# PAMRec/PAMRec

Measured on NVIDIA B200. Metric: train samples/sec, higher is better.
Workload: dtype f32

## Files before the change

pamrec_b200/csrc/api.cu:

```cuda
#include <cmath>
#include <cstdarg>
#include <cstdio>
#include <cstdlib>
#include <string>
#include <vector>

#include "comm.h"
#include "head2.h"
#include "kernels.h"
#include "layout.h"

using namespace pamrec;

struct Xchg {
  std::vector<int64_t> soff, scnt, roff, rcnt;
  int64_t n_send = 0, n_recv = 0;
};

struct PamrecHandle_ {
  PamrecConfig cfg;
  Layout L;
  PamrecBuffers buf;
  bool bound = false;
  int debug = 0;
// ... 301 lines not shown
  size_t have = (size_t)h->L.ws[h->L.ws_index["cub_temp"]].numel;
  if (need > have) return fail(h, "cub temp storage: need %zu have %zu", need, have);
  cudaMemsetAsync(h->buf.workspace, 0, h->L.ws_bytes, st);
  if (h->sharded() || h->sibling()) {
    cudaMemsetAsync(h->wi("sp.item.slot"), 0xFF, (size_t)h->L.rows_of(h->cfg.n_items) * 4, st);
    cudaMemsetAsync(h->wi("sp.cate.slot"), 0xFF, (size_t)h->L.rows_of(h->cfg.n_cates) * 4, st);
    if (h->cfg.model_kind != PAMREC_MODEL_SASREC)
      cudaMemsetAsync(h->wi("sp.user.slot"), 0xFF, (size_t)h->L.rows_of(h->cfg.n_users) * 4, st);
  } else {
    cudaMemsetAsync(h->wi("sp2.slot"), 0xFF, ((size_t)h->cfg.n_items + h->cfg.n_cates + h->cfg.n_users) * 4, st);
  }
  if (h->sharded() && !h->h_counts &&
      cudaMallocHost(&h->h_counts, sizeof(int) * (8 * (size_t)h->cfg.world_size + 4)) != cudaSuccess)
    return fail(h, "cudaMallocHost for the exchange counts failed");
  cudaMemcpyAsync(h->wi("seg_id"), h->h_seg_id.data(), h->h_seg_id.size() * 4, cudaMemcpyHostToDevice, st);
  cudaMemcpyAsync(h->wi("seg_tab"), h->h_seg_tab.data(), h->h_seg_tab.size() * 4, cudaMemcpyHostToDevice, st);
  if (h->sibling()) h->head2_grid = 0;
  else if (int rc = build_head(h, st)) return rc;
  cudaStreamSynchronize(st);
  h->bound = true;
  return check_cuda(h, "bind");
}

static int check_batch(PamrecHandle h, const PamrecBatch* b, bool training) {
  if (!h) return -1;
  if (!h->bound) return fail(h, "pamrec_bind has not been called");
  if (!b) return fail(h, "null batch");
  if (b->batch == 0 && (h->sharded() || h->cfg.world_size > 1)) return 0;
  if (b->batch < 1 || b->batch > h->cfg.max_batch) return fail(h, "batch %d outside [1, %d]", b->batch, h->cfg.max_batch);
  if (h->sibling()) {
    if (!b->satisfied_item_history || !b->satisfied_cate_history || !b->satisfied_mask || !b->item_history || !b->item_cate_history ||
        !b->mask || !b->items || !b->cates)
      return fail(h, "null batch field (the sibling models also read satisfied_item_history / satisfied_cate_history / satisfied_mask)");
    const bool sas = h->cfg.model_kind == PAMREC_MODEL_SASREC;
    if (training && (!b->labels_satisfied || (!sas && (!b->users || !b->labels_play)))) return fail(h, "null label field");
    return 0;
  }
  if (training && b->batch % PAMREC_GROUP != 0)
    return fail(h, "training batch %d is not a multiple of %d (pamrec.py:73-75)", b->batch, PAMREC_GROUP);
  if (training && h->cfg.loss_kind == PAMREC_LOSS_SOFTMAX && b->batch % h->cfg.softmax_group != 0)
    return fail(h, "training batch %d is not a multiple of the softmax group %d (base_model.py:224-225)", b->batch, h->cfg.softmax_group);
  if (!b->item_history || !b->item_cate_history || !b->item_loop_times_history || !b->mask || !b->items || !b->cates)
    return fail(h, "null batch field");
  if (training && (!b->users || !b->labels_satisfied || !b->labels_play || !b->plays)) return fail(h, "null label field");
  return 0;
}

static Sp2 make_sp2(PamrecHandle h, const PamrecBatch* b) {
  Sp2 s;
  memset(&s, 0, sizeof s);
  const PamrecConfig& c = h->cfg;
  s.item_hist = b->item_history; s.cate_hist = b->item_cate_history; s.items = b->items; s.cates = b->cates; s.users = b->users;
  s.B = b->batch; s.N = (int64_t)b->batch * c.max_seq_len;
  s.n_items = c.n_items; s.n_cates = c.n_cates; s.n_users = c.n_users;
  s.keys = h->wi("sp2.keys"); s.idx = h->wi("sp2.idx"); s.skeys = h->wi("sp2.skeys"); s.sidx = h->wi("sp2.sidx"); s.uidx = h->wi("sp2.uidx");
  s.ukeys[0] = h->wi("sp.item.ukeys"); s.ukeys[1] = h->wi("sp.cate.ukeys"); s.ukeys[2] = h->wi("sp.user.ukeys");
  s.nuniq = h->wi("sp.nuniq"); s.meta = h->wi("sp2.meta");
  s.accum[0] = h->wf("sp.item.accum"); s.accum[1] = h->wf("sp.cate.accum");
  s.dflag[0] = h->wi("sp2.dflag"); s.dflag[1] = s.dflag[0] + h->L.cub_keys_table;
  s.l2sq = h->wd("sp2.l2sq"); s.undedup = h->wd("sp_normsq");
  s.w[0] = h->buf.item_w; s.m[0] = h->buf.item_m; s.v[0] = h->buf.item_v;
  s.w[1] = h->buf.cate_w; s.m[1] = h->buf.cate_m; s.v[1] = h->buf.cate_v;
  s.w[2] = h->buf.ulong_w; s.m[2] = h->buf.ulong_m; s.v[2] = h->buf.ulong_v;
  s.w[3] = h->buf.ushort_w; s.m[3] = h->buf.ushort_m; s.v[3] = h->buf.ushort_v;
  s.dX0 = h->wf("g_a"); s.dT = h->wf("d_tgt_total");
  if (h->replicated()) { s.mode = SP2_DENSE; s.rep_grad = h->rep_grad_in(); }
  else if (c.sparse_adam_mode == PAMREC_ADAM_LAZY) s.mode = SP2_FUSED;
  else { s.mode = SP2_COMPACT; s.slot = h->wi("sp2.slot"); }
  return s;
}
static AdamP make_adam(PamrecHandle h, float lr_t) {
  const PamrecConfig& c = h->cfg;
  AdamP a;
  a.lr = lr_t; a.b1 = c.beta1; a.b2 = c.beta2; a.eps = c.epsilon; a.l2 = c.embed_l2; a.clip = c.max_grad_norm; a.is_clip = c.is_clip_norm;
  a.lr_dev = nullptr;
  return a;
}

static const char* const kShardName[3] = {"item", "cate", "user"};
static const ShardDim& shard_dim(PamrecHandle h, int t) { return t == 0 ? h->L.sh_item : (t == 1 ? h->L.sh_cate : h->L.sh_user); }

static SparseTable req_table(PamrecHandle h, int t) {
  SparseTable s;
  memset(&s, 0, sizeof s);
  const ShardDim& d = shard_dim(h, t);
  std::string p = std::string("sp.") + kShardName[t] + ".";
  s.keys = h->wi(p + "keys"); s.idx = h->wi(p + "idx"); s.skeys = h->wi(p + "skeys"); s.sidx = h->wi(p + "sidx");
  s.uidx = h->wi(p + "uidx"); s.ukeys = h->wi(p + "ukeys");
  s.width = d.width; s.n_rows = d.rps * h->cfg.world_size;
  s.accum = d.width ? h->wf(p + "accum") : nullptr;
  s.nuniq = h->wi("sp.nuniq") + t;
  s.normsq = h->wd("sp_normsq") + t;
  return s;
}
static SparseTable own_table(PamrecHandle h, int t, bool user_short = false) {
  SparseTable s;
  memset(&s, 0, sizeof s);
  const ShardDim& d = shard_dim(h, t);
  std::string q = std::string("so.") + kShardName[t] + ".";
  s.keys = h->wi(q + "keys"); s.idx = h->wi(q + "idx"); s.skeys = h->wi(q + "skeys"); s.sidx = h->wi(q + "sidx");
  s.uidx = h->wi(q + "uidx"); s.ukeys = h->wi(q + "ukeys");
  s.slot = h->wi(std::string("sp.") + kShardName[t] + ".slot");
  s.n_rows = d.rps;
  s.nuniq = h->wi("sp.nuniq") + 4 + t;
  double* ns = h->wd("sp_normsq");
  if (t == 0) { s.width = kI; s.w = h->buf.item_w; s.m = h->buf.item_m; s.v = h->buf.item_v; s.accum = h->wf(q + "accum"); s.normsq = ns; }
  else if (t == 1) { s.width = kC; s.w = h->buf.cate_w; s.m = h->buf.cate_m; s.v = h->buf.cate_v; s.accum = h->wf(q + "accum"); s.normsq = ns + 1; }
  else if (!user_short) { s.width = PAMREC_USER_DIM; s.w = h->buf.ulong_w; s.m = h->buf.ulong_m; s.v = h->buf.ulong_v; s.normsq = ns + 2; }
  else { s.width = PAMREC_USER_DIM; s.w = h->buf.ushort_w; s.m = h->buf.ushort_m; s.v = h->buf.ushort_v; s.normsq = ns + 3; }
  return s;
}

static int shard_exchange_fwd(PamrecHandle h, const PamrecBatch* b, bool training, cudaStream_t st) {
  const int W = h->cfg.world_size, B = b->batch, T = h->cfg.max_seq_len;
  const int64_t N = (int64_t)B * T;
  void* tmp = h->ws<char>("cub_temp");
  const size_t tmp_bytes = (size_t)h->L.ws[h->L.ws_index.at("cub_temp")].numel;
  int* cs = h->wi("sh.counts_send");
  int* cr = h->wi("sh.counts_recv");
  cudaMemsetAsync(cs, 0, sizeof(int) * 4 * W, st);
  const int nt = training ? 3 : 2;
  h->xc_users = training;
  for (int t = 0; t < nt; ++t) {
    const ShardDim& d = shard_dim(h, t);
    SparseTable req = req_table(h, t);
    const int* hist = t == 0 ? b->item_history : (t == 1 ? b->item_cate_history : b->users);
    const int* tgt = t == 0 ? b->items : (t == 1 ? b->cates : nullptr);
    const int64_t n_hist = t < 2 ? N : B, n_tgt = t < 2 ? B : 0;
    if (launch_sparse_plan(req, hist, tgt, n_hist, n_tgt, W, d.rps, d.rps * W, false, tmp, tmp_bytes, st))
      return fail(h, "cub sort failed");
    std::string p = std::string("sh.") + kShardName[t] + ".";
    launch_shard_route(req, n_hist + n_tgt, W, d.rps, h->wi(p + "off"), cs, t, h->wi(p + "send_ids"), h->wi(p + "inv"), st);
  }
  {
    PAMREC_PROF("xchg_counts", 1, st);
    if (h->comm.all_to_all(cs, cr, 4, COMM_I32, st)) return fail(h, "nccl: %s", h->comm.err.c_str());
    cudaMemcpyAsync(h->h_counts, cs, sizeof(int) * 4 * W, cudaMemcpyDeviceToHost, st);
    cudaMemcpyAsync(h->h_counts + 4 * W, cr, sizeof(int) * 4 * W, cudaMemcpyDeviceToHost, st);
    h->h_counts[8 * W] = 0;
    if (h->mbox_open) cudaMemcpyAsync(h->h_counts + 8 * W, h->mbox_err(), sizeof(int), cudaMemcpyDeviceToHost, st);
    if (cudaStreamSynchronize(st) != cudaSuccess) return check_cuda(h, "exchange counts");
    if (h->h_counts[8 * W]) return fail(h, "peer mailbox all-reduce timed out at sync point %d (a rank left the step?)", h->h_counts[8 * W] - 1);
  }
  for (int t = 0; t < 3; ++t) {
    Xchg& x = h->xc[t];
    x.soff.assign(W, 0); x.scnt.assign(W, 0); x.roff.assign(W, 0); x.rcnt.assign(W, 0);
    int64_t so = 0, ro = 0;
    for (int p = 0; p < W; ++p) {
      x.scnt[p] = t < nt ? h->h_counts[4 * p + t] : 0;
      x.rcnt[p] = t < nt ? h->h_counts[4 * W + 4 * p + t] : 0;
      x.soff[p] = so; so += x.scnt[p];
      x.roff[p] = ro; ro += x.rcnt[p];
    }
    x.n_send = so; x.n_recv = ro;
    if (ro > shard_dim(h, t).cap_recv) return fail(h, "exchange overflow on table %s: %lld rows", kShardName[t], (long long)ro);
  }
  {
    PAMREC_PROF("xchg_ids", 1, st);
    int xrc = h->comm.group_start();
    for (int t = 0; t < nt && !xrc; ++t) {
      const Xchg& x = h->xc[t];
      std::string p = std::string("sh.") + kShardName[t] + ".";
      xrc |= h->comm.all_to_all_v(h->wi(p + "send_ids"), x.soff.data(), x.scnt.data(), h->wi(p + "recv_ids"), x.roff.data(),
                                  x.rcnt.data(), 1, COMM_I32, st);
    }
    xrc |= h->comm.group_end();
    if (xrc) return fail(h, "nccl: %s", h->comm.err.c_str());
  }
  if (training) {
    int prc = 0;
    h->fork(st, [&](cudaStream_t s2) {
      for (int t = 0; t < 3; ++t) {
        SparseTable own = own_table(h, t);
        std::string p = std::string("sh.") + kShardName[t] + ".";
        prc |= launch_sparse_plan(own, h->wi(p + "recv_ids"), nullptr, h->xc[t].n_recv, 0, 1, 0, own.n_rows, true, tmp, tmp_bytes, s2);
      }
      cudaEventRecord(h->ev_plan, s2);
    });
    if (prc) return fail(h, "cub sort failed");
  }
  launch_serve_rows(h->buf.item_w, h->wi("sh.item.recv_ids"), h->xc[0].n_recv, kI, h->wf("sh.item.xrows"), st);
  launch_serve_rows(h->buf.cate_w, h->wi("sh.cate.recv_ids"), h->xc[1].n_recv, kC, h->wf("sh.cate.xrows"), st);
  {
    PAMREC_PROF("xchg_rows", 1, st);
    int xrc = h->comm.group_start();
    for (int t = 0; t < 2 && !xrc; ++t) {
      const Xchg& x = h->xc[t];
      std::string p = std::string("sh.") + kShardName[t] + ".";
      xrc |= h->comm.all_to_all_v(h->wf(p + "xrows"), x.roff.data(), x.rcnt.data(), h->wf(p + "rows"), x.soff.data(),
                                  x.scnt.data(), shard_dim(h, t).width, COMM_F32, st);
    }
    xrc |= h->comm.group_end();
    if (xrc) return fail(h, "nccl: %s", h->comm.err.c_str());
  }
  return 0;
}

static int embed_forward(PamrecHandle h, const PamrecBatch* b, bool training, float* x0, cudaStream_t st) {
  const int B = b->batch, T = h->cfg.max_seq_len;
  if (!h->sharded()) {
    launch_embed_fwd(b->item_history, b->item_cate_history, b->items, b->cates, h->buf.item_w, h->buf.cate_w, h->P(h->L.pos), x0,
                     h->wf("tgt"), B, T, st);
    return 0;
  }
  if (int rc = shard_exchange_fwd(h, b, training, st)) return rc;
  const int64_t N = (int64_t)B * T;
  const int* ii = h->wi("sh.item.inv");
  const int* ci = h->wi("sh.cate.inv");
  launch_embed_fwd(ii, ci, ii + N, ci + N, h->wf("sh.item.rows"), h->wf("sh.cate.rows"), h->P(h->L.pos), x0, h->wf("tgt"), B, T, st);
  return 0;
}

int pamrec_gather_fwd(PamrecHandle h, const PamrecBatch* b, float* x0_out, void* stream) {
  if (int rc = check_batch(h, b, false)) return rc;
  if (h->sibling()) return fail(h, "pamrec_gather_fwd is PAMRec's fused gather; the sibling models gather inside pamrec_forward");
  ProfBind _pb(h);
  cudaStream_t st = (cudaStream_t)stream;
  if (int rc = embed_forward(h, b, false, x0_out ? x0_out : h->wf("x0"), st)) return rc;
  return check_cuda(h, "gather_fwd");
}

static DenseP dense_p(const float* X, int ldx, int M, int groups, int K, int N, const float* W, int ws, const float* bias,
                      int bs, float* Z, int ldz) {
  DenseP p;
  memset(&p, 0, sizeof p);
  p.X = X; p.ldx = ldx; p.M = M; p.n_groups = groups; p.K = K; p.N = N;
  p.W = W; p.w_stride = ws; p.bias = bias; p.b_stride = bs; p.Z = Z; p.ldz = ldz;
  return p;
}
static void set_in_bn(DenseP& p, const BnSet& s) { p.in_stat = s.stat; p.in_gamma = s.gamma; p.in_beta = s.beta; }
static void set_in_bn_dw(DenseDwP& p, const BnSet& s) { p.in_stat = s.stat; p.in_gamma = s.gamma; p.in_beta = s.beta; }

static int sib_forward(PamrecHandle h, const PamrecBatch* b, int training, float* pred_out, cudaStream_t st);
static int sib_backward(PamrecHandle h, const PamrecBatch* b, cudaStream_t st);
static int sib_apply(PamrecHandle h, const PamrecBatch* b, int64_t step, cudaStream_t st);
static int sas_forward(PamrecHandle h, const PamrecBatch* b, int training, float* pred_out, cudaStream_t st);
static int sas_backward(PamrecHandle h, const PamrecBatch* b, cudaStream_t st);

int pamrec_forward(PamrecHandle h, const PamrecBatch* b, int training, float* pred_out, void* stream) {
  if (int rc = check_batch(h, b, training != 0)) return rc;
  ProfBind _pb(h);
  cudaStream_t st = (cudaStream_t)stream;
  if (h->cfg.model_kind == PAMREC_MODEL_SASREC) return sas_forward(h, b, training, pred_out, st);
  if (h->sibling()) return sib_forward(h, b, training, pred_out, st);
  const Layout& L = h->L;
  const int B = b->batch, T = h->cfg.max_seq_len, N = B * T;
  const int W = h->cfg.world_size;
  const int Bg = b->global_batch > 0 ? b->global_batch : B * W;
  const double cntN = (double)Bg * T, cntB = (double)Bg;
  int64_t nl = 0;
  int crc = 0;
  int p2p_slot = 0;
  auto sync_finalize = [&](std::initializer_list<int> ids, double cnt, bool with_scalars) {
    if (!training) return;
    if (W > 1 && h->mbox_open) {
      P2PArgs a;
      memset(&a, 0, sizeof a);
      for (int id : ids) { a.buf[a.nbuf] = h->bn[id].sums; a.n[a.nbuf++] = 2 * h->bn[id].C; a.bn[a.nbn] = h->bn[id]; a.count[a.nbn++] = cnt; }
      if (with_scalars) { a.buf[a.nbuf] = h->wd("dp.scalars"); a.n[a.nbuf++] = 8; }
      for (int p = 0; p < W; ++p) { a.peer_slots[p] = h->mbox_slots(p); a.peer_flags[p] = h->mbox_flags(p); }
      a.world = W; a.rank = h->cfg.rank; a.slot = p2p_slot; a.epoch = ++h->mbox_epoch[p2p_slot]; a.err = h->mbox_err();
      ++p2p_slot;
      launch_p2p_allreduce(a, st); nl += 1;
      return;
    }
    if (W > 1 && !crc) {
      PAMREC_PROF("allreduce_bn_fwd", 1, st);
      crc |= h->comm.group_start();
      for (int id : ids) crc |= h->comm.all_reduce(h->bn[id].sums, 2 * (int64_t)h->bn[id].C, COMM_F64, st);
      if (with_scalars) crc |= h->comm.all_reduce(h->wd("dp.scalars"), 8, COMM_F64, st);
      crc |= h->comm.group_end();
    }
    for (int id : ids) { launch_bn_finalize(h->bn[id], cnt, st); nl += 1; }
  };
  float* x0 = h->wf("x0");
  int* ctl = h->wi("bucket_ctl");
  const bool bucket_aside = !h->sharded() && getenv("PAMREC_NO_SIDE_STREAM") == nullptr;
  if (bucket_aside) {
    h->fork(st, [&](cudaStream_t s2) {
      launch_bucket_plan(b->item_loop_times_history, N, h->wi("bucket"), h->wi("perm"), ctl, h->wi("tile_bucket"), h->wi("tile_begin"),
                         h->wi("tile_count"), s2);
      cudaEventRecord(h->ev_bucket, s2);
    });
  }
  if (int rc = embed_forward(h, b, training != 0, x0, st)) return rc;
  nl += 1;
  if (training && !h->sharded() && B > 0) {
    int prc = 0;
    h->fork(st, [&](cudaStream_t s2) {
      prc |= launch_sp2_plan(make_sp2(h, b), h->ws<char>("cub_temp"), (size_t)L.ws[L.ws_index.at("cub_temp")].numel, s2);
      cudaEventRecord(h->ev_plan, s2);
    });
    if (prc) return fail(h, "cub sort failed");
    h->plan_for = b->item_history; h->plan_rows = B;
  }
  if (training && W > 1 && !h->use_head2()) {
    cudaMemsetAsync(h->wd("dp.scalars"), 0, 8 * sizeof(double), st);
    launch_count_valid_groups(b->plays, B, h->wd("dp.scalars"), st);
  }
  if (bucket_aside) cudaStreamWaitEvent(st, h->ev_bucket, 0);
  else launch_bucket_plan(b->item_loop_times_history, N, h->wi("bucket"), h->wi("perm"), ctl, h->wi("tile_bucket"),
                          h->wi("tile_begin"), h->wi("tile_count"), st);
  nl += 3;
  const int max_tiles = N / kTokTile + kNB + 1;
  const float* xin = x0;
  for (int k = 0; k < 2; ++k) {
    const BlockOff& o = L.blk[k];
    std::string p = "blk" + std::to_string(k) + ".";
    launch_proj_fwd(xin, h->wi("perm"), ctl, h->wi("tile_bucket"), h->wi("tile_begin"), h->wi("tile_count"), max_tiles,
                    h->P(o.wq), h->P(o.wk), h->P(o.wv), h->P(o.ln_a_beta), h->P(o.ln_a_gamma), h->wf(p + "qin"), h->wf(p + "Q"),
                    h->wf(p + "K"), h->wf(p + "V"), st);
    if (h->attn_mma)
      launch_attn_fwd_mma(h->wf(p + "Q"), h->wf(p + "K"), h->wf(p + "V"), h->wf(p + "qin"), b->mask, h->wf(p + "y"), h->wf(p + "ml"), B, T, st);
    else if (h->attn_tc && attn_tc_supported(T))
      launch_attn_fwd_tc(h->wf(p + "Q"), h->wf(p + "K"), h->wf(p + "V"), h->wf(p + "qin"), b->mask, h->wf(p + "y"), h->wf(p + "ml"), B, T,
                         h->n_sm, reinterpret_cast<int*>(h->head_bar + 3), st);
    else
      launch_attn_fwd(h->wf(p + "Q"), h->wf(p + "K"), h->wf(p + "V"), h->wf(p + "qin"), b->mask, h->wf(p + "y"), h->wf(p + "ml"), B, T, st);
    float* hdbg = (training && (h->debug & PAMREC_DEBUG_SAVE_FFN_HIDDEN)) ? h->wf(k == 0 ? "d_Q" : "d_K") : nullptr;
    launch_ffn_fwd(h->wf(p + "y"), h->P(o.w1), h->P(o.b1), h->P(o.w2), h->P(o.b2), h->P(o.ln_b_beta), h->P(o.ln_b_gamma),
                   h->wf(p + "out"), hdbg, N, st);
    nl += 3;
    xin = h->wf(p + "out");
  }
  const float* H = xin;
  BnSet* bn = h->bn;
  if (h->use_head2()) {
    HeadDyn d = head_dyn(h, b, training != 0, 0);
    d.pred = pred_out;
    if (launch_head2_fwd(h->head2, d, h->head2_grid, training ? "head_fwd" : "head_score", st)) return check_cuda(h, "cooperative head launch");
    return check_cuda(h, "forward");
  }
  if (!training) {
    for (int i = 0; i < BN_COUNT; ++i) launch_bn_eval_stat(bn[i], st);
    nl += BN_COUNT;
  }
  {
    DenseP p = dense_p(H, kD, N, 1, kD, 20, h->P(L.score.w0), 0, h->P(L.score.b0), 0, h->wf("z1"), 20);
    p.out_sums = training ? bn[BN_S0].sums : nullptr;
    launch_dense_fwd(p, st); nl += 1;
    sync_finalize({BN_S0}, cntN, true);
    DenseP q = dense_p(h->wf("z1"), 20, N, 1, 20, 1, h->P(L.score.w1), 0, h->P(L.score.b1), 0, h->wf("z2"), 1);
    set_in_bn(q, bn[BN_S0]);
    q.out_sums = training ? bn[BN_S1].sums : nullptr;
    launch_dense_fwd(q, st); nl += 1;
    sync_finalize({BN_S1}, cntN, false);
  }
  launch_pool_fwd(H, h->wf("z2"), bn[BN_S1], b->mask, h->wf("new_long"), B, T, st); nl += 1;
  {
    DenseP e0 = dense_p(h->wf("new_long"), kD, B, 5, kD, 100, h->P(L.expert.w0), 4000, h->P(L.expert.b0), 100, h->wf("ze0"), 500);
    for (int g = 0; g < 5; ++g) { e0.x_off[g] = 0; e0.z_off[g] = g * 100; }
    e0.out_sums = training ? bn[BN_E0].sums : nullptr;
    launch_dense_fwd(e0, st);
    DenseP g0 = dense_p(h->wf("new_long"), kD, B, 2, kD, 64, h->P(L.gate.w0), 2560, h->P(L.gate.b0), 64, h->wf("zg0"), 128);
    for (int g = 0; g < 2; ++g) { g0.x_off[g] = 0; g0.z_off[g] = g * 64; }
    g0.out_sums = training ? bn[BN_G0].sums : nullptr;
    launch_dense_fwd(g0, st);
    nl += 2;
    sync_finalize({BN_E0, BN_G0}, cntB, false);
    DenseP e1 = dense_p(h->wf("ze0"), 500, B, 5, 100, 64, h->P(L.expert.w1), 6400, h->P(L.expert.b1), 64, h->wf("ze1"), 320);
    for (int g = 0; g < 5; ++g) { e1.x_off[g] = g * 100; e1.z_off[g] = g * 64; }
    set_in_bn(e1, bn[BN_E0]);
    e1.out_sums = training ? bn[BN_E1].sums : nullptr;
    launch_dense_fwd(e1, st);
    DenseP g1 = dense_p(h->wf("zg0"), 128, B, 2, 64, 5, h->P(L.gate.w1), 320, h->P(L.gate.b1), 5, h->wf("zg1"), 10);
    for (int g = 0; g < 2; ++g) { g1.x_off[g] = g * 64; g1.z_off[g] = g * 5; }
    set_in_bn(g1, bn[BN_G0]);
    g1.out_sums = training ? bn[BN_G1].sums : nullptr;
    launch_dense_fwd(g1, st);
    nl += 2;
    sync_finalize({BN_E1, BN_G1}, cntB, false);
  }
  launch_combine_fwd(h->wf("ze1"), h->wf("zg1"), bn[BN_E1], bn[BN_G1], h->wf("tgt"), h->wf("u"), B, st); nl += 1;
  {
    DenseP t0 = dense_p(h->wf("u"), 168, B, 3, 84, 100, h->P(L.tower.w0), 8400, h->P(L.tower.b0), 100, h->wf("zt0"), 300);
    t0.x_off[0] = 0; t0.x_off[1] = 84; t0.x_off[2] = 0;
    for (int g = 0; g < 3; ++g) t0.z_off[g] = g * 100;
    t0.out_sums = training ? bn[BN_T0].sums : nullptr;
    launch_dense_fwd(t0, st); nl += 1;
    sync_finalize({BN_T0}, cntB, false);
    DenseP t1 = dense_p(h->wf("zt0"), 300, B, 3, 100, 64, h->P(L.tower.w1), 6400, h->P(L.tower.b1), 64, h->wf("zt1"), 192);
    for (int g = 0; g < 3; ++g) { t1.x_off[g] = g * 100; t1.z_off[g] = g * 64; }
    set_in_bn(t1, bn[BN_T0]);
    t1.out_sums = training ? bn[BN_T1].sums : nullptr;
    launch_dense_fwd(t1, st); nl += 1;
    sync_finalize({BN_T1}, cntB, false);
    DenseP to = dense_p(h->wf("zt1"), 192, B, 3, 64, 1, h->P(L.tower.wout), 64, h->P(L.tower.bout), 1, h->wf("logits"), 3);
    for (int g = 0; g < 3; ++g) { to.x_off[g] = g * 64; to.z_off[g] = g; }
    set_in_bn(to, bn[BN_T1]);
    launch_dense_fwd(to, st); nl += 1;
  }
  if (pred_out) { launch_sigmoid_col0(h->wf("logits"), pred_out, B, st); nl += 1; }
  if (crc) return fail(h, "nccl: %s", h->comm.err.c_str());
  return check_cuda(h, "forward");
}

static DenseDwP dw_p(const float* X, int ldx, int M, int groups, int K, int N, const float* dZ, int lddz, float* dW, int ws,
                     float* db, int bs) {
  DenseDwP p;
  memset(&p, 0, sizeof p);
  p.X = X; p.ldx = ldx; p.M = M; p.n_groups = groups; p.K = K; p.N = N; p.dZ = dZ; p.lddz = lddz;
  p.dW = dW; p.w_stride = ws; p.db = db; p.b_stride = bs;
  return p;
}
static DenseDxP dx_p(const float* dZ, int lddz, int M, int K, const float* Wbase, float* dX, int lddx, int accumulate) {
  DenseDxP p;
  memset(&p, 0, sizeof p);
  p.dZ = dZ; p.lddz = lddz; p.M = M; p.K = K; p.Wbase = Wbase; p.dX = dX; p.lddx = lddx; p.accumulate = accumulate;
  return p;
}
static void dx_add(DenseDxP& p, int slice, int out_off, int dz_off, int64_t w_off, int N) {
  if (slice >= p.n_slices) { p.n_slices = slice + 1; p.out_off[slice] = out_off; p.n_contrib[slice] = 0; }
  int c = p.n_contrib[slice]++;
  p.dz_off[slice][c] = dz_off; p.w_off[slice][c] = w_off; p.Ncon[slice][c] = N;
}

static HeadDyn head_dyn(PamrecHandle h, const PamrecBatch* b, bool training, int slot0) {
  HeadDyn d;
  memset(&d, 0, sizeof d);
  const int W = h->cfg.world_size;
  d.B = b->batch; d.T = h->cfg.max_seq_len; d.training = training ? 1 : 0; d.world = W; d.rank = h->cfg.rank;
  d.Bg = b->global_batch > 0 ? b->global_batch : b->batch * W;
  d.cntN = (double)d.Bg * d.T; d.cntB = (double)d.Bg;
  d.mask = b->mask; d.y_sat = b->labels_satisfied; d.y_play = b->labels_play; d.plays = b->plays;
  d.fuzhu_w = h->cfg.fuzhu_weight; d.order_w = h->cfg.order_weight;
  d.sm_group = h->cfg.loss_kind == PAMREC_LOSS_SOFTMAX ? h->cfg.softmax_group : 0;
  d.bar = h->head_bar;
  d.trace = h->head_trace ? reinterpret_cast<unsigned long long*>(h->head_bar + 64) + (slot0 ? 32 : 0) : nullptr;
  d.trace_cta = (h->head_trace && h->head_trace_cta) ? h->head_trace_cta + (slot0 ? 16 * 256 : 0) : nullptr;
  if (W > 1) {
    for (int p = 0; p < W; ++p) {
      d.peer_slots[p] = h->mbox_slots(p); d.peer_flags[p] = h->mbox_flags(p);
      d.peer_ll[p] = reinterpret_cast<uint4*>(static_cast<char*>(h->mbox_peer[p]) + p2p_ll_offset(W));
    }
    d.p2p_epoch = ++h->coop_epoch; d.p2p_slot0 = slot0; d.p2p_err = h->mbox_err();
  }
  return d;
}

static int build_head(PamrecHandle h, cudaStream_t st) {
  h->head2_grid = 0;
  if (getenv("PAMREC_HEAD_LEGACY") != nullptr) return 0;
  if (h->cfg.world_size > kP2PMaxWorld) return 0;
  const Layout& L = h->L;
  Head2& H = h->head2;
  memset(&H, 0, sizeof H);
  H.H = h->wf("blk1.out"); H.tgt = h->wf("tgt");
  H.s_w0 = h->P(L.score.w0); H.s_b0 = h->P(L.score.b0); H.s_w1 = h->P(L.score.w1); H.s_b1 = h->P(L.score.b1);
  H.e_w0 = h->P(L.expert.w0); H.e_b0 = h->P(L.expert.b0); H.e_w1 = h->P(L.expert.w1); H.e_b1 = h->P(L.expert.b1);
  H.g_w0 = h->P(L.gate.w0); H.g_b0 = h->P(L.gate.b0); H.g_w1 = h->P(L.gate.w1); H.g_b1 = h->P(L.gate.b1);
  H.t_w0 = h->P(L.tower.w0); H.t_b0 = h->P(L.tower.b0); H.t_w1 = h->P(L.tower.w1); H.t_b1 = h->P(L.tower.b1);
  H.t_wo = h->P(L.tower.wout); H.t_bo = h->P(L.tower.bout);
  H.ds_w0 = h->G(L.score.w0); H.ds_b0 = h->G(L.score.b0); H.ds_w1 = h->G(L.score.w1); H.ds_b1 = h->G(L.score.b1);
  H.de_w0 = h->G(L.expert.w0); H.de_b0 = h->G(L.expert.b0); H.de_w1 = h->G(L.expert.w1); H.de_b1 = h->G(L.expert.b1);
  H.dg_w0 = h->G(L.gate.w0); H.dg_b0 = h->G(L.gate.b0); H.dg_w1 = h->G(L.gate.w1); H.dg_b1 = h->G(L.gate.b1);
  H.dt_w0 = h->G(L.tower.w0); H.dt_b0 = h->G(L.tower.b0); H.dt_w1 = h->G(L.tower.w1); H.dt_b1 = h->G(L.tower.b1);
  H.dt_wo = h->G(L.tower.wout); H.dt_bo = h->G(L.tower.bout);
  H.wT = h->wf("head.wT");
  static_assert(kHead2Groups == 8, "layout.h: bn.gsums / bn.gbsums hold 8 copies");
  for (int i = 0; i < BN_COUNT; ++i) {
    H.bn[i] = h->bn[i];
    H.gsums[i] = h->wd("bn.gsums") + (size_t)kHead2Groups * L.bn_bsums_off[i];
    H.gbsums[i] = h->wd("bn.gbsums") + (size_t)kHead2Groups * L.bn_bsums_off[i];
  }
  H.z1 = h->wf("z1"); H.z2 = h->wf("z2"); H.aw = h->wf("pool.aw"); H.new_long = h->wf("new_long");
  H.ze0 = h->wf("ze0"); H.zg0 = h->wf("zg0"); H.ze1 = h->wf("ze1"); H.zg1 = h->wf("zg1"); H.u = h->wf("u");
  H.zt0 = h->wf("zt0"); H.zt1 = h->wf("zt1"); H.logits = h->wf("logits");
  H.d_logits = h->wf("d_logits"); H.d_t1 = h->wf("d_t1"); H.d_t0 = h->wf("d_t0"); H.d_e1 = h->wf("d_e1"); H.d_g1 = h->wf("d_g1");
  H.d_e0 = h->wf("d_e0"); H.d_g0 = h->wf("d_g0"); H.d_new_long = h->wf("d_new_long"); H.d_tgt = h->wf("d_tgt");
  H.d_z2 = h->wf("d_z2"); H.g_a = h->wf("g_a");
  H.loss_acc = h->wd("loss_acc"); H.dp_scalars = h->wd("dp.scalars");
  const int g2 = head2_grid();
  if (g2 <= 0) { cudaGetLastError(); return 0; }
  if (!h->head_bar) {
    if (cudaMalloc(&h->head_bar, 256 + 2 * 32 * 8) != cudaSuccess) return check_cuda(h, "head barrier alloc");
    cudaMemsetAsync(h->head_bar, 0, 256 + 2 * 32 * 8, st);
  }
  h->head2_grid = g2;
  return check_cuda(h, "head2");
}

int pamrec_backward(PamrecHandle h, const PamrecBatch* b, void* stream) {
  if (int rc = check_batch(h, b, true)) return rc;
  ProfBind _pb(h);
  cudaStream_t st = (cudaStream_t)stream;
  if (h->cfg.model_kind == PAMREC_MODEL_SASREC) return sas_backward(h, b, st);
  if (h->sibling()) return sib_backward(h, b, st);
  const Layout& L = h->L;
  const int B = b->batch, T = h->cfg.max_seq_len, N = B * T;
  const int W = h->cfg.world_size;
  const int Bg = b->global_batch > 0 ? b->global_batch : B * W;
  const double cntN = (double)Bg * T, cntB = (double)Bg;
  const float gs = 1.0f / (float)W;
  BnSet* bn = h->bn;
  int64_t nl = 0;
  int crc = 0;
  const float* Pb = h->buf.dense_param;
  cudaMemsetAsync(h->buf.dense_grad, 0, (size_t)L.dense_numel * 4, st);
  cudaMemsetAsync(h->wd("loss_acc"), 0, 8 * sizeof(double), st);
  cudaMemsetAsync(h->wd("sp_normsq"), 0, 8 * sizeof(double), st);
  const bool rows = h->use_head2();
  const bool coop = rows;
  if (!coop) {
  launch_loss(h->wf("logits"), b->labels_satisfied, b->labels_play, b->plays, h->wf("d_logits"), h->wd("loss_acc"), B, Bg,
              W > 1 ? h->wd("dp.scalars") : nullptr, h->cfg.fuzhu_weight, h->cfg.order_weight,
              h->cfg.loss_kind == PAMREC_LOSS_SOFTMAX ? h->cfg.softmax_group : 0, st); nl += 1;
  }
  cudaMemsetAsync(h->wd("bn.bsums"), 0, (size_t)L.ws[L.ws_index.at("bn.bsums")].numel * sizeof(double), st);
  if (rows) {
    HeadDyn d = head_dyn(h, b, true, 12);
    if (launch_head2_bwd(h->head2, d, h->head2_grid, st)) return check_cuda(h, "cooperative head launch");
    h->fork(st, [&](cudaStream_t s2) { launch_head2_dw(h->head2, B, s2); });
  }
  int p2p_slot = 6;
  auto sync_bsums = [&](std::initializer_list<int> ids) {
    if (W == 1 || crc) return;
    if (h->mbox_open) {
      P2PArgs a;
      memset(&a, 0, sizeof a);
      for (int id : ids) { a.buf[a.nbuf] = bn[id].bsums; a.n[a.nbuf++] = 2 * bn[id].C; }
      for (int p = 0; p < W; ++p) { a.peer_slots[p] = h->mbox_slots(p); a.peer_flags[p] = h->mbox_flags(p); }
      a.world = W; a.rank = h->cfg.rank; a.slot = p2p_slot; a.epoch = ++h->mbox_epoch[p2p_slot]; a.err = h->mbox_err();
      ++p2p_slot;
      launch_p2p_allreduce(a, st);
      return;
    }
    PAMREC_PROF("allreduce_bn_bwd", 1, st);
    crc |= h->comm.group_start();
    for (int id : ids) crc |= h->comm.all_reduce(bn[id].bsums, 2 * (int64_t)bn[id].C, COMM_F64, st);
    crc |= h->comm.group_end();
  };
  auto grad_of = [&](int id, const float* Z, double cnt) {
    BnGrad g; g.Z = Z; g.stat = bn[id].stat; g.gamma = bn[id].gamma; g.beta = bn[id].beta; g.bsums = bn[id].bsums; g.count = cnt;
    return g;
  };
  auto out_of = [&](int id, const float* Z) {
    BnGradOut o; o.Z = Z; o.stat = bn[id].stat; o.gamma = bn[id].gamma; o.beta = bn[id].beta; o.bsums = bn[id].bsums;
    return o;
  };
  auto dw_bn = [&](DenseDwP& w, int id, const float* Z, double cnt) {
    w.g = grad_of(id, Z, cnt); w.g_dgamma = bn[id].dgamma; w.g_dbeta = bn[id].dbeta; w.g_C = bn[id].C; w.g_scale = gs;
  };
  if (!coop) {
  {
    DenseDwP w = dw_p(h->wf("zt1"), 192, B, 3, 64, 1, h->wf("d_logits"), 3, h->G(L.tower.wout), 64, h->G(L.tower.bout), 1);
    for (int g = 0; g < 3; ++g) { w.x_off[g] = g * 64; w.z_off[g] = g; }
    set_in_bn_dw(w, bn[BN_T1]);
    h->fork(st, [&](cudaStream_t s2) { launch_dense_dw(w, s2); });
    DenseDxP x = dx_p(h->wf("d_logits"), 3, B, 64, Pb, h->wf("d_t1"), 192, 0);
    for (int g = 0; g < 3; ++g) dx_add(x, g, g * 64, g, L.tower.wout + g * 64, 1);
    x.o = out_of(BN_T1, h->wf("zt1"));
    launch_dense_dx(x, st);
    nl += 2;
    sync_bsums({BN_T1});
    DenseDwP w1 = dw_p(h->wf("zt0"), 300, B, 3, 100, 64, h->wf("d_t1"), 192, h->G(L.tower.w1), 6400, h->G(L.tower.b1), 64);
    for (int g = 0; g < 3; ++g) { w1.x_off[g] = g * 100; w1.z_off[g] = g * 64; }
    set_in_bn_dw(w1, bn[BN_T0]);
    dw_bn(w1, BN_T1, h->wf("zt1"), cntB);
    h->fork(st, [&](cudaStream_t s2) { launch_dense_dw(w1, s2); });
    DenseDxP x1 = dx_p(h->wf("d_t1"), 192, B, 100, Pb, h->wf("d_t0"), 300, 0);
    for (int g = 0; g < 3; ++g) dx_add(x1, g, g * 100, g * 64, L.tower.w1 + (int64_t)g * 6400, 64);
    x1.g = grad_of(BN_T1, h->wf("zt1"), cntB);
    x1.o = out_of(BN_T0, h->wf("zt0"));
    launch_dense_dx(x1, st);
    nl += 2;
    sync_bsums({BN_T0});
    DenseDwP w0 = dw_p(h->wf("u"), 168, B, 3, 84, 100, h->wf("d_t0"), 300, h->G(L.tower.w0), 8400, h->G(L.tower.b0), 100);
    w0.x_off[0] = 0; w0.x_off[1] = 84; w0.x_off[2] = 0;
    for (int g = 0; g < 3; ++g) w0.z_off[g] = g * 100;
    dw_bn(w0, BN_T0, h->wf("zt0"), cntB);
    h->fork(st, [&](cudaStream_t s2) { launch_dense_dw(w0, s2); });
    DenseDxP x0 = dx_p(h->wf("d_t0"), 300, B, 84, Pb, h->wf("d_u"), 168, 0);
    dx_add(x0, 0, 0, 0, L.tower.w0, 100);
    dx_add(x0, 0, 0, 200, L.tower.w0 + 2 * 8400, 100);
    dx_add(x0, 1, 84, 100, L.tower.w0 + 8400, 100);
    x0.g = grad_of(BN_T0, h->wf("zt0"), cntB);
    launch_dense_dx(x0, st);
    nl += 2;
  }
  launch_combine_bwd(h->wf("ze1"), h->wf("zg1"), bn[BN_E1], bn[BN_G1], h->wf("d_u"), h->wf("d_e1"), h->wf("d_g1"),
                     h->wf("d_tgt"), B, st); nl += 1;
  {
    launch_bn_bwd_stats(bn[BN_E1], h->wf("d_e1"), h->wf("ze1"), B, st);
    launch_bn_bwd_stats(bn[BN_G1], h->wf("d_g1"), h->wf("zg1"), B, st);
    nl += 2;
    sync_bsums({BN_E1, BN_G1});
    DenseDwP we = dw_p(h->wf("ze0"), 500, B, 5, 100, 64, h->wf("d_e1"), 320, h->G(L.expert.w1), 6400, h->G(L.expert.b1), 64);
    for (int g = 0; g < 5; ++g) { we.x_off[g] = g * 100; we.z_off[g] = g * 64; }
    set_in_bn_dw(we, bn[BN_E0]);
    dw_bn(we, BN_E1, h->wf("ze1"), cntB);
    h->fork(st, [&](cudaStream_t s2) { launch_dense_dw(we, s2); });
    DenseDxP xe = dx_p(h->wf("d_e1"), 320, B, 100, Pb, h->wf("d_e0"), 500, 0);
    for (int g = 0; g < 5; ++g) dx_add(xe, g, g * 100, g * 64, L.expert.w1 + (int64_t)g * 6400, 64);
    xe.g = grad_of(BN_E1, h->wf("ze1"), cntB);
    xe.o = out_of(BN_E0, h->wf("ze0"));
    launch_dense_dx(xe, st);
    DenseDwP wg = dw_p(h->wf("zg0"), 128, B, 2, 64, 5, h->wf("d_g1"), 10, h->G(L.gate.w1), 320, h->G(L.gate.b1), 5);
    for (int g = 0; g < 2; ++g) { wg.x_off[g] = g * 64; wg.z_off[g] = g * 5; }
    set_in_bn_dw(wg, bn[BN_G0]);
    dw_bn(wg, BN_G1, h->wf("zg1"), cntB);
    h->fork(st, [&](cudaStream_t s2) { launch_dense_dw(wg, s2); });
    DenseDxP xg = dx_p(h->wf("d_g1"), 10, B, 64, Pb, h->wf("d_g0"), 128, 0);
    for (int g = 0; g < 2; ++g) dx_add(xg, g, g * 64, g * 5, L.gate.w1 + (int64_t)g * 320, 5);
    xg.g = grad_of(BN_G1, h->wf("zg1"), cntB);
    xg.o = out_of(BN_G0, h->wf("zg0"));
    launch_dense_dx(xg, st);
    nl += 4;
    sync_bsums({BN_E0, BN_G0});
    DenseDwP we0 = dw_p(h->wf("new_long"), kD, B, 5, kD, 100, h->wf("d_e0"), 500, h->G(L.expert.w0), 4000, h->G(L.expert.b0), 100);
    for (int g = 0; g < 5; ++g) { we0.x_off[g] = 0; we0.z_off[g] = g * 100; }
    dw_bn(we0, BN_E0, h->wf("ze0"), cntB);
    h->fork(st, [&](cudaStream_t s2) { launch_dense_dw(we0, s2); });
    DenseDwP wg0 = dw_p(h->wf("new_long"), kD, B, 2, kD, 64, h->wf("d_g0"), 128, h->G(L.gate.w0), 2560, h->G(L.gate.b0), 64);
    for (int g = 0; g < 2; ++g) { wg0.x_off[g] = 0; wg0.z_off[g] = g * 64; }
    dw_bn(wg0, BN_G0, h->wf("zg0"), cntB);
    h->fork(st, [&](cudaStream_t s2) { launch_dense_dw(wg0, s2); });
    DenseDxP xe0 = dx_p(h->wf("d_e0"), 500, B, kD, Pb, h->wf("d_new_long"), kD, 0);
    for (int g = 0; g < 5; ++g) dx_add(xe0, 0, 0, g * 100, L.expert.w0 + (int64_t)g * 4000, 100);
    xe0.g = grad_of(BN_E0, h->wf("ze0"), cntB);
    launch_dense_dx(xe0, st);
    DenseDxP xg0 = dx_p(h->wf("d_g0"), 128, B, kD, Pb, h->wf("d_new_long"), kD, 1);
    for (int g = 0; g < 2; ++g) dx_add(xg0, 0, 0, g * 64, L.gate.w0 + (int64_t)g * 2560, 64);
    xg0.g = grad_of(BN_G0, h->wf("zg0"), cntB);
    launch_dense_dx(xg0, st);
    nl += 4;
  }
  }
  const float* H = h->wf("blk1.out");
  float* g_a = h->wf("g_a");
  float* g_b = h->wf("g_b");
  if (!coop) {
    launch_pool_bwd(H, h->wf("z2"), bn[BN_S1], b->mask, h->wf("d_new_long"), h->wf("d_z2"), g_a, B, T, st); nl += 1;
    launch_bn_bwd_stats(bn[BN_S1], h->wf("d_z2"), h->wf("z2"), N, st); nl += 1;
    sync_bsums({BN_S1});
    DenseDwP w1 = dw_p(h->wf("z1"), 20, N, 1, 20, 1, h->wf("d_z2"), 1, h->G(L.score.w1), 0, h->G(L.score.b1), 0);
    set_in_bn_dw(w1, bn[BN_S0]);
    dw_bn(w1, BN_S1, h->wf("z2"), cntN);
    h->fork(st, [&](cudaStream_t s2) { launch_dense_dw(w1, s2); });
    DenseDxP x1 = dx_p(h->wf("d_z2"), 1, N, 20, Pb, h->wf("d_a1"), 20, 0);
    dx_add(x1, 0, 0, 0, L.score.w1, 1);
    x1.g = grad_of(BN_S1, h->wf("z2"), cntN);
    x1.o = out_of(BN_S0, h->wf("z1"));
    launch_dense_dx(x1, st);
    nl += 2;
    sync_bsums({BN_S0});
    DenseDwP w0 = dw_p(H, kD, N, 1, kD, 20, h->wf("d_a1"), 20, h->G(L.score.w0), 0, h->G(L.score.b0), 0);
    dw_bn(w0, BN_S0, h->wf("z1"), cntN);
    h->fork(st, [&](cudaStream_t s2) { launch_dense_dw(w0, s2); });
    DenseDxP x0 = dx_p(h->wf("d_a1"), 20, N, kD, Pb, g_a, kD, 1);
    dx_add(x0, 0, 0, 0, L.score.w0, 20);
    x0.g = grad_of(BN_S0, h->wf("z1"), cntN);
    launch_dense_dx(x0, st);
    nl += 2;
  }
  const int max_tiles = N / kTokTile + kNB + 1;
  int* ctl = h->wi("bucket_ctl");
  for (int k = 1; k >= 0; --k) {
    const BlockOff& o = L.blk[k];
    std::string p = "blk" + std::to_string(k) + ".";
    const float* xin = k == 0 ? h->wf("x0") : h->wf("blk0.out");
    float* gout = k == 1 ? g_a : g_b;
    float* gin = k == 1 ? g_b : g_a;
    launch_ffn_bwd(h->wf(p + "y"), gout, h->P(o.w1), h->P(o.b1), h->P(o.w2), h->P(o.ln_b_beta), h->P(o.ln_b_gamma), h->wf("d_y"),
                   h->G(o.w1), h->G(o.b1), h->G(o.w2), h->G(o.b2), h->G(o.ln_b_beta), h->G(o.ln_b_gamma), N, st);
    if (h->attn_mma && (T <= 128 || getenv("PAMREC_ATTN_BWD_MMA") != nullptr) && getenv("PAMREC_ATTN_BWD_FFMA") == nullptr)
      launch_attn_bwd_mma(h->wf(p + "Q"), h->wf(p + "K"), h->wf(p + "V"), h->wf("d_y"), h->wf(p + "y"), h->wf(p + "qin"), h->wf(p + "ml"),
                          b->mask, h->wf("d_Q"), h->wf("d_K"), h->wf("d_V"), B, T, st);
    else
      launch_attn_bwd(h->wf(p + "Q"), h->wf(p + "K"), h->wf(p + "V"), h->wf("d_y"), h->wf(p + "y"), h->wf(p + "qin"), h->wf(p + "ml"),
                      b->mask, h->wf("d_Q"), h->wf("d_K"), h->wf("d_V"), B, T, st);
    launch_proj_bwd(xin, h->wf("d_y"), h->wf("d_Q"), h->wf("d_K"), h->wf("d_V"), h->wi("perm"), ctl, h->wi("tile_bucket"),
                    h->wi("tile_begin"), h->wi("tile_count"), max_tiles, h->P(o.wq), h->P(o.wk), h->P(o.wv), h->P(o.ln_a_beta),
                    h->P(o.ln_a_gamma), gin, h->G(o.wq), h->G(o.wk), h->G(o.wv), h->G(o.ln_a_beta), h->G(o.ln_a_gamma), st);
    nl += 3;
  }
  launch_embed_bwd_reduce(g_a, h->wf("d_tgt"), h->wf("d_tgt_total"), h->G(L.pos), h->wd("sp_normsq") + 4,
                          h->sharded() ? nullptr : h->wd("sp_normsq"), B, T, st); nl += 2;
  h->join(st);
  if (crc) return fail(h, "nccl: %s", h->comm.err.c_str());
  return check_cuda(h, "backward");
}

static void peer_allreduce_grads(PamrecHandle h, cudaStream_t st) {
  XrArgs a;
  memset(&a, 0, sizeof a);
  const int W = h->cfg.world_size;
  for (int p = 0; p < W; ++p) a.peer[p] = h->xr_region(p);
  a.world = W; a.rank = h->cfg.rank; a.epoch = ++h->xr_epoch;
  a.cap = p2p_xr_cap(W, h->xr_floats());
  a.dense_grad = h->buf.dense_grad; a.n_dense = h->L.dense_numel;
  a.scalars[0] = h->wd("sp_normsq"); a.n_scalars[0] = 8;
  a.scalars[1] = h->wd("loss_acc"); a.n_scalars[1] = 4;
  a.counter = reinterpret_cast<unsigned*>(h->xr_region(h->cfg.rank) + 128);
  a.err = h->mbox_err();
  launch_xr_allreduce(a, h->buf.dense_grad, st);
}

int pamrec_apply_gradients(PamrecHandle h, const PamrecBatch* b, int64_t step, void* stream) {
  if (int rc = check_batch(h, b, true)) return rc;
  ProfBind _pb(h);
  if (h->sibling()) return sib_apply(h, b, step, (cudaStream_t)stream);
  if (step < 0) return fail(h, "step must be >= 1 (or 0: advance the device step counter)");
  if (step == 0 && (h->sharded() || h->cfg.world_size > 1)) return fail(h, "the device step counter (step = 0) needs one GPU with whole tables");
  cudaStream_t st = (cudaStream_t)stream;
  const Layout& L = h->L;
  const PamrecConfig& c = h->cfg;
  const int B = b->batch, T = c.max_seq_len;
  const int64_t N = (int64_t)B * T;
  const double b1 = c.beta1, b2 = c.beta2;
  const double tstep = step > 0 ? (double)step : 1.0;
  const float lr_t = (float)((double)c.learning_rate * std::sqrt(1.0 - std::pow(b2, tstep)) / (1.0 - std::pow(b1, tstep)));
  const float* lr_dev = nullptr;
  if (!h->sharded()) {
    launch_adam_step(step, h->wd("adam.step"), c.learning_rate, c.beta1, c.beta2, h->wf("adam.lr"), st);
    lr_dev = h->wf("adam.lr");
  }
  double* reg = h->wd("loss_acc") + 3;
  void* tmp = h->ws<char>("cub_temp");
  size_t tmp_bytes = (size_t)L.ws[L.ws_index.at("cub_temp")].numel;
  int64_t nl = 0;
  bool dense_aside = false;
  const float* dX0 = h->wf("g_a");
  const float* dT = h->wf("d_tgt_total");
  if (h->sharded()) {
    Comm& cm = h->comm;
    int crc = 0;
    if (!h->xc_users) return fail(h, "apply_gradients needs pamrec_forward(training=1) on the same batch");
    for (int t = 0; t < 2; ++t) {
      SparseTable req = req_table(h, t);
      const int col = t == 0 ? 0 : kI;
      launch_sparse_segreduce(req, N + B, N, dX0, kD, col, dT, kE, col, req.normsq, st);
    }
    {
      PAMREC_PROF("xchg_grads", 1, st);
      crc |= cm.group_start();
      for (int t = 0; t < 2; ++t) {
        const Xchg& x = h->xc[t];
        std::string p = std::string("sh.") + kShardName[t] + ".";
        crc |= cm.all_to_all_v(req_table(h, t).accum, x.soff.data(), x.scnt.data(), h->wf(p + "xrows"), x.roff.data(), x.rcnt.data(),
                               shard_dim(h, t).width, COMM_F32, st);
      }
      crc |= cm.group_end();
    }
    cudaStreamWaitEvent(st, h->ev_plan, 0);
    for (int t = 0; t < 3; ++t) {
      SparseTable own = own_table(h, t);
      const int64_t nr = h->xc[t].n_recv;
      std::string p = std::string("sh.") + kShardName[t] + ".";
      if (t < 2) launch_sparse_segreduce(own, nr, nr, h->wf(p + "xrows"), own.width, 0, nullptr, 0, 0, h->wd("sh.scratch"), st);
      launch_sparse_l2norm(own, nr, c.embed_l2, reg, st);
      if (t == 2) launch_sparse_l2norm(own_table(h, 2, true), nr, c.embed_l2, reg, st);
    }
    if (h->use_xr()) {
      peer_allreduce_grads(h, st);
    } else {
      PAMREC_PROF("allreduce_grads", 1, st);
      crc |= cm.group_start();
      crc |= cm.all_reduce(h->buf.dense_grad, L.dense_numel, COMM_F32, st);
      crc |= cm.all_reduce(h->wd("sp_normsq"), 8, COMM_F64, st);
      crc |= cm.all_reduce(h->wd("loss_acc"), 4, COMM_F64, st);
      crc |= cm.group_end();
    }
    if (crc) return fail(h, "nccl: %s", cm.err.c_str());
    for (int t = 0; t < 3; ++t) {
      SparseTable own = own_table(h, t);
      const int64_t nr = h->xc[t].n_recv;
      launch_sparse_adam(own, nr, c.sparse_adam_mode, c.embed_l2, lr_t, c.beta1, c.beta2, c.epsilon, c.max_grad_norm, c.is_clip_norm, st);
      if (t == 2)
        launch_sparse_adam(own_table(h, 2, true), nr, c.sparse_adam_mode, c.embed_l2, lr_t, c.beta1, c.beta2, c.epsilon,
                           c.max_grad_norm, c.is_clip_norm, st);
      launch_slot_reset(own, nr, st);
    }
  } else {
    if (c.world_size == 1 && getenv("PAMREC_NO_SIDE_STREAM") == nullptr) {
      dense_aside = true;
      h->fork(st, [&](cudaStream_t s2) {
        launch_dense_norm(h->buf.dense_param, h->buf.dense_grad, h->wi("seg_tab"), (int)L.dense.size(), c.layer_l2, h->wd("seg_normsq"),
                          h->wd("sp_normsq") + 4, reg, s2);
        launch_dense_adam(h->buf.dense_param, h->buf.dense_grad, h->buf.dense_m, h->buf.dense_v, h->wi("seg_id"), h->wi("seg_tab"),
                          h->wd("seg_normsq"), L.dense_numel, c.layer_l2, lr_t, lr_dev, c.beta1, c.beta2, c.epsilon, c.max_grad_norm,
                          c.is_clip_norm, s2);
      });
    }
    const bool planned = h->plan_for == b->item_history && h->plan_rows == B;
    h->plan_for = nullptr;
    const Sp2 s2 = make_sp2(h, b);
    AdamP ap = make_adam(h, lr_t);
    ap.lr_dev = lr_dev;
    if (planned) cudaStreamWaitEvent(st, h->ev_plan, 0);
    else if (launch_sp2_plan(s2, tmp, tmp_bytes, st)) return fail(h, "cub sort failed");
    launch_sp2_walk(s2, ap, st);
    nl += 10;
    if (h->replicated()) {
      Sp2 s3 = s2;
      if (h->use_xr()) {
        peer_allreduce_grads(h, st);
        s3.rep_grad = h->rep_grad_out();
      } else {
        Comm& cm = h->comm;
        int crc = 0;
        {
          PAMREC_PROF("allreduce_grads", 1, st);
          crc |= cm.group_start();
          crc |= cm.all_reduce(h->buf.dense_grad, L.dense_numel, COMM_F32, st);
          crc |= cm.all_reduce(s2.rep_grad, sp2_rep_floats(c.n_items, c.n_cates, c.n_users), COMM_F32, st);
          crc |= cm.all_reduce(h->wd("sp_normsq"), 8, COMM_F64, st);
          crc |= cm.all_reduce(h->wd("loss_acc"), 4, COMM_F64, st);
          crc |= cm.group_end();
        }
        if (crc) return fail(h, "nccl: %s", cm.err.c_str());
      }
      launch_sp2_rep_l2(s3, st);
      launch_sp2_adam_sweep(s3, ap, c.sparse_adam_mode == PAMREC_ADAM_LAZY ? 1 : 0, st);
      nl += 3;
    } else if (s2.mode == SP2_FUSED) {
      launch_sp2_lazy_finish(s2, ap, st); nl += 1;
    } else {
      launch_sp2_adam_sweep(s2, ap, 0, st); nl += 1;
    }
  }
  const int n_seg = (int)L.dense.size();
  if (dense_aside) {
    h->join(st);
  } else {
    launch_dense_norm(h->buf.dense_param, h->buf.dense_grad, h->wi("seg_tab"), n_seg, c.layer_l2, h->wd("seg_normsq"),
                      h->wd("sp_normsq") + 4, reg, st);
    launch_dense_adam(h->buf.dense_param, h->buf.dense_grad, h->buf.dense_m, h->buf.dense_v, h->wi("seg_id"), h->wi("seg_tab"),
                      h->wd("seg_normsq"), L.dense_numel, c.layer_l2, lr_t, lr_dev, c.beta1, c.beta2, c.epsilon, c.max_grad_norm,
                      c.is_clip_norm, st);
  }
  launch_finish_losses(h->wd("loss_acc"), h->wf("losses"), h->sharded() ? nullptr : h->wd("sp2.l2sq"), c.embed_l2, h->wd("sp_normsq"), st);
  nl += 3;
  return check_cuda(h, "apply_gradients");
}

#include "api_sibling.inl"

int pamrec_train_step(PamrecHandle h, const PamrecBatch* b, int64_t step, float* losses_out, void* stream) {
  if (!h) return -1;
  const int64_t l0 = h->prof.launches;
  if (int rc = pamrec_forward(h, b, 1, nullptr, stream)) return rc;
  if (int rc = pamrec_backward(h, b, stream)) return rc;
  if (int rc = pamrec_apply_gradients(h, b, step, stream)) return rc;
  if (losses_out)
    cudaMemcpyAsync(losses_out, h->wf("losses"), 5 * sizeof(float), cudaMemcpyDeviceToDevice, (cudaStream_t)stream);
  h->launches = h->prof.launches - l0;
  return check_cuda(h, "train_step");
}

int pamrec_comm_all_reduce(PamrecHandle h, void* dptr, int64_t count, int dtype, void* stream) {
  if (!h) return -1;
  CommType t = dtype == PAMREC_F64 ? COMM_F64 : (dtype == PAMREC_I32 ? COMM_I32 : COMM_F32);
  if (h->comm.all_reduce(dptr, count, t, (cudaStream_t)stream)) return fail(h, "nccl: %s", h->comm.err.c_str());
  return 0;
}

int pamrec_bench_gather(PamrecHandle h, const int32_t* item_ids, const int32_t* cate_ids, const int32_t* tgt_items,
                        const int32_t* tgt_cates, int64_t n_rows, int32_t T, float* out, void* stream) {
  if (!h || !h->bound) return fail(h, "not bound");
  if (h->sibling()) return fail(h, "bench_gather measures PAMRec's fused gather");
  if (T < 1 || T > h->cfg.max_seq_len) return fail(h, "T outside the position table");
  ProfBind _pb(h);
  launch_embed_fwd(item_ids, cate_ids, tgt_items, tgt_cates, h->buf.item_w, h->buf.cate_w, h->P(h->L.pos), out, nullptr, n_rows,
                   T, (cudaStream_t)stream);
  return check_cuda(h, "bench_gather");
}

int pamrec_bench_table_adam(PamrecHandle h, int64_t step, void* stream) {
  if (!h || !h->bound) return fail(h, "not bound");
  ProfBind _pb(h);
  const PamrecConfig& c = h->cfg;
  const double b1 = c.beta1, b2 = c.beta2;
  const float lr_t = (float)((double)c.learning_rate * std::sqrt(1.0 - std::pow(b2, (double)step)) / (1.0 - std::pow(b1, (double)step)));
  if (h->sharded() || h->sibling()) return fail(h, "bench_table_adam runs on PAMRec's whole tables");
  PamrecBatch nb;
  memset(&nb, 0, sizeof nb);
  Sp2 s2 = make_sp2(h, &nb);
  s2.mode = SP2_COMPACT; s2.slot = h->wi("sp2.slot");
  launch_sp2_adam_sweep(s2, make_adam(h, lr_t), 0, (cudaStream_t)stream);
  return check_cuda(h, "bench_table_adam");
}

int pamrec_set_debug(PamrecHandle h, int flags) {
  if (!h) return -1;
  h->debug = flags;
  h->head_trace = (flags & PAMREC_DEBUG_HEAD_TRACE) != 0;
  if (h->head_trace && !h->head_trace_cta && cudaMalloc(&h->head_trace_cta, 2 * 16 * 256 * 8) == cudaSuccess)
    cudaMemset(h->head_trace_cta, 0, 2 * 16 * 256 * 8);
  return 0;
}
int pamrec_head_trace_ctas(PamrecHandle h, int backward, uint64_t* out ) {
  if (!h || !out || !h->head_trace_cta) return -1;
  cudaDeviceSynchronize();
  if (cudaMemcpy(out, h->head_trace_cta + (backward ? 16 * 256 : 0), 16 * 256 * 8, cudaMemcpyDeviceToHost) != cudaSuccess) return check_cuda(h, "head trace");
  return 0;
}
int pamrec_head_trace(PamrecHandle h, int backward, uint64_t out[32]) {
  if (!h || !out || !h->head_bar) return -1;
  cudaDeviceSynchronize();
  if (cudaMemcpy(out, reinterpret_cast<unsigned long long*>(h->head_bar + 64) + (backward ? 32 : 0), 32 * 8, cudaMemcpyDeviceToHost) != cudaSuccess)
    return check_cuda(h, "head trace");
  return 0;
}
int pamrec_profile_enable(PamrecHandle h, int on) {
  if (!h) return -1;
  h->prof.on = on != 0;
  return 0;
}
int pamrec_profile_reset(PamrecHandle h) {
  if (!h) return -1;
  h->prof.reset();
  return 0;
}
int pamrec_profile_count(PamrecHandle h) {
  if (!h) return -1;
  h->prof.resolve();
  return (int)h->prof.names.size();
}
int pamrec_profile_get(PamrecHandle h, int index, char name[64], double* total_ms, int64_t* launches) {
  if (!h || index < 0 || index >= (int)h->prof.names.size()) return -1;
  snprintf(name, 64, "%s", h->prof.names[index].c_str());
  if (total_ms) *total_ms = h->prof.ms[index];
  if (launches) *launches = h->prof.cnt[index];
  return 0;
}

}
```

pamrec_b200/csrc/common.cuh:

```cuda
#pragma once
#include <cuda_runtime.h>
#include <stdint.h>

#include "../../include/pamrec_b200.h"

namespace pamrec {

constexpr int kI = PAMREC_ITEM_DIM;
constexpr int kC = PAMREC_CATE_DIM;
constexpr int kE = PAMREC_EMB_DIM;
constexpr int kD = PAMREC_D;
constexpr int kNB = PAMREC_NBUCKET;
constexpr int kDD = kD * kD;
constexpr int kMT = 1;
constexpr int kWarpRows = 16 * kMT;
constexpr int kTokThreads = 128;
constexpr int kTokTile = 4 * kWarpRows;
constexpr int kRowPad = 41;
constexpr int kAttnStride = 44;
constexpr float kMaskNeg = -4294967295.0f;
constexpr float kLnEps = 1e-8f;
constexpr float kBnEps = 1e-4f;
constexpr float kBnDecay = 0.05f;

__device__ __forceinline__ float warp_sum(float v) {
#pragma unroll
  for (int o = 16; o > 0; o >>= 1) v += __shfl_xor_sync(0xffffffffu, v, o);
  return v;
}
__device__ __forceinline__ float warp_max(float v) {
#pragma unroll
  for (int o = 16; o > 0; o >>= 1) v = fmaxf(v, __shfl_xor_sync(0xffffffffu, v, o));
  return v;
}
__device__ __forceinline__ double warp_sum_d(double v) {
#pragma unroll
  for (int o = 16; o > 0; o >>= 1) v += __shfl_xor_sync(0xffffffffu, v, o);
  return v;
}
__device__ __forceinline__ float4 ld4(const float* p) { return *reinterpret_cast<const float4*>(p); }
__device__ __forceinline__ void st4(float* p, const float4& v) { *reinterpret_cast<float4*>(p) = v; }
__device__ __forceinline__ float4 f4_zero() { return make_float4(0.f, 0.f, 0.f, 0.f); }
__device__ __forceinline__ void f4_fma(float4& a, float s, const float4& b) {
  a.x = fmaf(s, b.x, a.x); a.y = fmaf(s, b.y, a.y); a.z = fmaf(s, b.z, a.z); a.w = fmaf(s, b.w, a.w);
}
__device__ __forceinline__ float f4_dot(const float4& a, const float4& b) {
  return fmaf(a.x, b.x, fmaf(a.y, b.y, fmaf(a.z, b.z, a.w * b.w)));
}
__device__ __forceinline__ float4 f4_shfl_down(const float4& v, int d) {
  float4 r;
  r.x = __shfl_down_sync(0xffffffffu, v.x, d); r.y = __shfl_down_sync(0xffffffffu, v.y, d);
  r.z = __shfl_down_sync(0xffffffffu, v.z, d); r.w = __shfl_down_sync(0xffffffffu, v.w, d);
  return r;
}

struct BnSet {
  int C;
  const float* gamma; const float* beta;
  float* dgamma; float* dbeta;
  float* mmean; float* mvar;
  double* sums;
  float* stat;
  double* bsums;
};

struct DenseP {
  const float* X; int ldx; int M;
  int n_groups, K, N;
  int x_off[8], z_off[8];
  const float* W; int w_stride;
  const float* bias; int b_stride;
  float* Z; int ldz;
  const float* in_stat; const float* in_gamma; const float* in_beta;
  double* out_sums;
};

struct BnGrad {
  const float* Z;
  const float* stat; const float* gamma; const float* beta;
  const double* bsums; double count;
};
struct BnGradOut {
  const float* Z; const float* stat; const float* gamma; const float* beta;
  double* bsums;
};
struct DenseDxP {
  const float* dZ; int lddz; int M;
  int n_slices; int K;
  int out_off[8]; int n_contrib[8];
  int dz_off[8][8]; int64_t w_off[8][8]; int Ncon[8][8];
  const float* Wbase;
  float* dX; int lddx; int accumulate;
  BnGrad g;
  BnGradOut o;
};

struct DenseDwP {
  const float* X; int ldx; int M;
  int n_groups, K, N;
  int x_off[8], z_off[8];
  const float* dZ; int lddz;
  const float* in_stat; const float* in_gamma; const float* in_beta;
  float* dW; int w_stride; float* db; int b_stride;
  BnGrad g;
  float* g_dgamma; float* g_dbeta; int g_C; float g_scale;
};

}
```

pamrec_b200/csrc/kernels.h:

```cpp
#pragma once
#include <string>
#include <vector>

#include "common.cuh"

namespace pamrec {

struct Prof {
  bool on = false;
  int64_t launches = 0;
  std::vector<std::string> names;
  std::vector<double> ms;
  std::vector<int64_t> cnt;
  struct Pair { cudaEvent_t a, b; int id; };
  std::vector<Pair> pending;
  std::vector<cudaEvent_t> free_ev;
  int id_of(const char* name);
  cudaEvent_t get_event();
  void resolve();
  void reset();
  ~Prof();
};
extern thread_local Prof* g_prof;
struct ProfScope {
  Prof* p; cudaStream_t st; cudaEvent_t b; bool timed;
  ProfScope(const char* name, int n_kernels, cudaStream_t st);
  ~ProfScope();
};
#define PAMREC_PROF(name, n, st) ProfScope _prof_scope(name, n, st)

int init_encoder_kernels(int max_T);
void launch_embed_fwd(const int* ih, const int* ch, const int* items, const int* cates, const float* item_w,
                      const float* cate_w, const float* pos, float* x0, float* tgt, int64_t n_rows, int T, cudaStream_t st);
void launch_bucket_plan(const float* lt, int n, int* bucket, int* perm, int* ctl, int* tile_bucket, int* tile_begin,
                        int* tile_count, cudaStream_t st);
void launch_proj_fwd(const float* X, const int* perm, const int* ctl, const int* tile_bucket, const int* tile_begin,
                     const int* tile_count, int max_tiles, const float* Wq, const float* Wk, const float* Wv,
                     const float* ln_beta, const float* ln_gamma, float* QIN, float* Q, float* K, float* V, cudaStream_t st);
void launch_attn_fwd(const float* Q, const float* K, const float* V, const float* QIN, const int* mask, float* Y, float* ML,
                     int B, int T, cudaStream_t st);
void launch_ffn_fwd(const float* Y, const float* W1, const float* b1, const float* W2, const float* b2,
                    const float* ln_beta, const float* ln_gamma, float* OUT, float* Hdbg, int n_tok, cudaStream_t st);
void launch_ffn_bwd(const float* Y, const float* dOUT, const float* W1, const float* b1, const float* W2,
                    const float* ln_beta, const float* ln_gamma, float* dY, float* dW1, float* db1, float* dW2,
                    float* db2, float* dbeta, float* dgamma, int n_tok, cudaStream_t st);
void launch_attn_bwd(const float* Q, const float* K, const float* V, const float* dY, const float* Y, const float* QIN,
                     const float* ML, const int* mask, float* dQ, float* dK, float* dV, int B, int T, cudaStream_t st);
void launch_proj_bwd(const float* X, const float* dY, const float* dQ, const float* dK, const float* dV, const int* perm,
                     const int* ctl, const int* tile_bucket, const int* tile_begin, const int* tile_count, int max_tiles,
                     const float* Wq, const float* Wk, const float* Wv, const float* ln_beta, const float* ln_gamma,
                     float* dX, float* dWq, float* dWk, float* dWv, float* dbeta, float* dgamma, cudaStream_t st);

bool attn_tc_supported(int T);
int init_attn_tc_kernels(int max_T);
void launch_attn_fwd_tc(const float* Q, const float* K, const float* V, const float* QIN, const int* mask, float* Y, float* ML, int B, int T,
                        int n_sm, int* err, cudaStream_t st);

int init_attn_mma_kernels(int max_T);
void launch_attn_fwd_mma(const float* Q, const float* K, const float* V, const float* QIN, const int* mask, float* Y, float* ML, int B, int T,
                         cudaStream_t st);
void launch_attn_bwd_mma(const float* Q, const float* K, const float* V, const float* dY, const float* Y, const float* QIN, const float* ML,
                         const int* mask, float* dQ, float* dK, float* dV, int B, int T, cudaStream_t st);

void launch_dense_fwd(const DenseP& p, cudaStream_t st);
void launch_dense_dx(const DenseDxP& p, cudaStream_t st);
void launch_dense_dw(const DenseDwP& p, cudaStream_t st);
void launch_bn_finalize(const BnSet& s, double count, cudaStream_t st);
void launch_bn_eval_stat(const BnSet& s, cudaStream_t st);
void launch_bn_bwd_stats(const BnSet& s, const float* dA, const float* Z, int M, cudaStream_t st);
void launch_pool_fwd(const float* H, const float* Z2, const BnSet& s1, const int* mask, float* new_long, int B, int T,
                     cudaStream_t st);
void launch_pool_bwd(const float* H, const float* Z2, const BnSet& s1, const int* mask, const float* d_new_long, float* dA2,
                     float* dH, int B, int T, cudaStream_t st);
void launch_combine_fwd(const float* ZE1, const float* ZG1, const BnSet& e1, const BnSet& g1, const float* tgt, float* U,
                        int B, cudaStream_t st);
void launch_combine_bwd(const float* ZE1, const float* ZG1, const BnSet& e1, const BnSet& g1, const float* dU, float* dE1,
                        float* dG1, float* dTgt, int B, cudaStream_t st);
void launch_loss(const float* logits, const float* y_sat, const float* y_play, const float* plays, float* d_logits,
                 double* loss_acc, int B, int B_global, const double* n_valid_global, float fuzhu_w, float order_w,
                 int softmax_group, cudaStream_t st);
void launch_sigmoid_col0(const float* logits, float* pred, int B, cudaStream_t st);

struct SparseTable {
  int width;
  int64_t n_rows;
  float* w; float* m; float* v;
  int* keys; int* idx; int* skeys; int* sidx; int* uidx; int* ukeys; int* slot;
  float* accum;
  int* nuniq;
  double* normsq;
  const int* l2_has0;
};
void launch_embed_bwd_reduce(const float* dX0, const float* dTgtHead, float* dTgtTotal, float* dPos, double* pos_normsq,
                             double* undedup, int B, int T, cudaStream_t st);
size_t sparse_temp_bytes(int64_t n_keys);
int launch_sparse_reduce(const SparseTable& t, const int* hist_ids, const int* tgt_ids, int64_t n_hist, int64_t n_tgt,
                         const float* hist_grad, int hist_ld, int hist_col, const float* tgt_grad, int tgt_ld, int tgt_col,
                         void* cub_temp, size_t cub_bytes, cudaStream_t st);
int launch_sparse_plan(const SparseTable& t, const int* hist_ids, const int* tgt_ids, int64_t n_hist, int64_t n_tgt,
                       int world, int64_t rps, int64_t key_range, bool fill_slot, void* cub_temp, size_t cub_bytes,
                       cudaStream_t st);
int launch_sparse_segreduce(const SparseTable& t, int64_t n, int64_t n_hist, const float* hist_grad, int hist_ld, int hist_col,
                            const float* tgt_grad, int tgt_ld, int tgt_col, double* normsq, cudaStream_t st);
void launch_slot_reset(const SparseTable& t, int64_t n_keys, cudaStream_t st);
int launch_sparse_l2norm(const SparseTable& t, int64_t n_keys, float l2, double* reg_acc, cudaStream_t st);
int launch_sparse_adam(const SparseTable& t, int64_t n_keys, int mode, float l2, float lr_t, float b1, float b2, float eps,
                        float clip, int is_clip, cudaStream_t st);
void launch_dense_norm(const float* P, const float* G, const int* seg_tab, int n_seg, float layer_l2, double* seg_normsq,
                       const double* pos_normsq, double* reg_acc, cudaStream_t st);
void launch_dense_adam(float* P, const float* G, float* M, float* V, const int* seg_id, const int* seg_tab,
                       const double* seg_normsq, int64_t n, float layer_l2, float lr_t, const float* lr_dev, float b1, float b2, float eps,
                       float clip, int is_clip, cudaStream_t st);
void launch_adam_step(int64_t step, double* step_dev, float lr, float b1, float b2, float* lr_out, cudaStream_t st);
void launch_finish_losses(const double* loss_acc, float* losses, const double* l2sq, float embed_l2, double* sp_normsq, cudaStream_t st);

enum { SP2_COMPACT = 0,
       SP2_FUSED = 1,
       SP2_DENSE = 2 };
struct AdamP { float lr, b1, b2, eps, l2, clip; int is_clip; const float* lr_dev; };
struct Sp2 {
  const int* item_hist; const int* cate_hist; const int* items; const int* cates; const int* users;
  int64_t N; int B;
  int n_items, n_cates, n_users;
  int* keys; int* idx; int* skeys; int* sidx; int* uidx;
  int* ukeys[3]; int* nuniq;
  int* meta;
  int* slot;
  float* accum[2]; int* dflag[2];
  double* l2sq;
  const double* undedup;
  float* w[4]; float* m[4]; float* v[4];
  const float* dX0; const float* dT;
  float* rep_grad;
  int mode;
};
inline int64_t sp2_rep_floats(int64_t n_items, int64_t n_cates, int64_t n_users) { return n_items * 17 + n_cates * 5 + n_users; }
size_t sp2_temp_bytes(int64_t n_keys);
int launch_sp2_plan(const Sp2& s, void* cub_temp, size_t cub_bytes, cudaStream_t st);
void launch_sp2_walk(const Sp2& s, const AdamP& a, cudaStream_t st);
void launch_sp2_lazy_finish(const Sp2& s, const AdamP& a, cudaStream_t st);
void launch_sp2_adam_sweep(const Sp2& s, const AdamP& a, int lazy, cudaStream_t st);
void launch_sp2_rep_l2(const Sp2& s, cudaStream_t st);

void launch_sib_gather(const int* sat_item, const int* sat_cate, const int* hist_item, const int* hist_cate, const int* items,
                       const int* cates, const float* item_w, const float* cate_w, float* h, float* tgt, int* ids_item,
                       int* ids_cate, int B, int T, int item_dim, cudaStream_t st);
void launch_sib_has0(const int* hist_item, const int* hist_cate, const int* items, const int* cates, int B, int T, int* has0,
                     cudaStream_t st);
void launch_sib_feat_fwd(float* feat, const float* tgt, int B, int T, int item_dim, cudaStream_t st);
void launch_sib_feat_bwd(const float* d_feat, const float* feat, const float* tgt, float* d_att, float* dq, int B, int T, int item_dim,
                         cudaStream_t st);
void launch_sib_pool_fwd(const float* h, const float* score, const int* sat_mask, const int* mask, const float* tgt, float* aw,
                         float* x, int B, int T, int item_dim, cudaStream_t st);
void launch_sib_pool_bwd(const float* h, const float* aw, const int* sat_mask, const int* mask, const float* d_x, float* d_score,
                         float* dh, int B, int T, int item_dim, cudaStream_t st);
void launch_sib_tgt_total(const float* d_tgt, const float* d_x, const float* dq, float* out, int B, int item_dim, cudaStream_t st);
void launch_sib_mix_fwd(const float* ZE1, const float* ZG1, const BnSet& e1, const BnSet& g1, const float* tgt, float* U, int n_expert,
                        const int sel[2][5], int B, int item_dim, cudaStream_t st);
void launch_sib_mix_bwd(const float* ZE1, const float* ZG1, const BnSet& e1, const BnSet& g1, const float* dU, float* dE1, float* dG1,
                        float* dTgt, int n_expert, const int sel[2][5], int B, int item_dim, cudaStream_t st);
void launch_sib_loss(const float* logits, const float* y_sat, const float* y_play, float* d_logits, double* loss_acc, int B, float aux_w,
                     int heads, cudaStream_t st);
void launch_sib_pred(const float* logits, float* pred, int B, int heads, cudaStream_t st);

int init_sas_kernels(int max_T);
void launch_sas_embed(const float* h, const float* pos, float* x0, int B, int T, int S, cudaStream_t st);
void launch_sas_proj_fwd(const float* X, const float* W, const float* bias, const float* ln_beta, const float* ln_gamma, float* XQ,
                         float* QKV, int64_t N, int S, cudaStream_t st);
void launch_sas_proj_bwd(const float* XQ, const float* dQKV, const float* dY, const float* W, const float* ln_gamma, float* dX,
                         float* g_gamma, float* g_beta, int64_t N, int S, cudaStream_t st);
void launch_sas_attn_fwd(const float* QKV, const float* XQ, const int* mask, float* Y, float* ML, int B, int T, int S, cudaStream_t st);
void launch_sas_attn_bwd(const float* QKV, const float* XQ, const float* Y, const float* dY, const float* ML, const int* mask, float* dQKV,
                         float* Dq, int B, int T, int S, cudaStream_t st);
void launch_sas_ffn_fwd(const float* Y, const float* W1, const float* b1, const float* W2, const float* b2, const float* ln_beta,
                        const float* ln_gamma, float* F, float* HPRE, float* OUT, int64_t N, int S, cudaStream_t st);
void launch_sas_ffn_bwd(const float* Y, const float* HPRE, const float* dOUT, const float* W1, const float* W2, const float* ln_gamma,
                        float* HID, float* DHPRE, float* dY, float* g_gamma, float* g_beta, int64_t N, int S, cudaStream_t st);
void launch_sas_final_fwd(const float* SEQ, const int* mask, const float* tgt, float* U, int B, int T, int S, cudaStream_t st);
void launch_sas_final_bwd(const float* dU, const int* mask, float* dSEQ, float* dTgt, int B, int T, int S, cudaStream_t st);
void launch_sas_pos_bwd(const float* dX0, float* dPos, double* normsq, int B, int T, int S, cudaStream_t st);

constexpr int kP2PMaxDoubles = 2048;
constexpr int kP2PSlots = 24;
constexpr int kP2PMaxWorld = 8;
struct P2PArgs {
  double* buf[3]; int n[3]; int nbuf;
  double* peer_slots[kP2PMaxWorld];
  uint32_t* peer_flags[kP2PMaxWorld];
  int world, rank, slot; uint32_t epoch;
  uint32_t* err;
  BnSet bn[2]; double count[2]; int nbn;
};
void launch_p2p_allreduce(const P2PArgs& a, cudaStream_t st);
inline size_t p2p_ll_offset(int world) {
  const size_t b = (size_t)kP2PSlots * world * kP2PMaxDoubles * sizeof(double) + (size_t)kP2PSlots * world * sizeof(uint32_t) + 256;
  return (b + 255) / 256 * 256;
}
constexpr int kXrScalars = 16;
inline size_t p2p_xr_offset(int world) { return (p2p_ll_offset(world) + (size_t)kP2PSlots * world * kP2PMaxDoubles * 16 + 255) / 256 * 256; }
inline int64_t p2p_xr_cap(int world, int64_t n_floats) { const int64_t q = 64 * (int64_t)world; return (n_floats + q - 1) / q * q; }
inline size_t p2p_xr_header_bytes() { return 512 + (size_t)kP2PMaxWorld * kXrScalars * sizeof(double); }
inline size_t p2p_mailbox_bytes(int world, int64_t xr_floats) {
  return p2p_xr_offset(world) + p2p_xr_header_bytes() + 2 * (size_t)p2p_xr_cap(world, xr_floats) * sizeof(float);
}
struct XrArgs {
  char* peer[kP2PMaxWorld];
  int world, rank; uint32_t epoch;
  int64_t cap;
  const float* dense_grad; int64_t n_dense;
  double* scalars[2]; int n_scalars[2];
  unsigned* counter;
  uint32_t* err;
};
inline float* xr_xbuf(char* region) { return reinterpret_cast<float*>(region + p2p_xr_header_bytes()); }
void launch_xr_allreduce(const XrArgs& a, float* dense_grad_out, cudaStream_t st);

void launch_shard_route(const SparseTable& req, int64_t n, int world, int64_t rps, int* off, int* counts, int slot, int* send_ids,
                        int* inv, cudaStream_t st);
void launch_serve_rows(const float* shard, const int* ids, int64_t n, int width, float* out, cudaStream_t st);
void launch_count_valid_groups(const float* plays, int B, double* out, cudaStream_t st);

}
```

pamrec_b200/csrc/kernels_attn_tc.cu:

```cuda
#include "kernels.h"
#include "mma.cuh"

namespace pamrec {

namespace tc {

constexpr int kThreads = 128;
constexpr int kRows = 128;
constexpr int kChunks = kD / 4;
constexpr int kNV = 48;
constexpr int kMaxNK = 208;
constexpr uint32_t kColPlo = 256, kColO = 464, kTmemCols = 512;

__device__ __forceinline__ uint32_t smem_u32(const void* p) { return (uint32_t)__cvta_generic_to_shared(p); }
__device__ __forceinline__ void mbar_init(uint64_t* bar, uint32_t count) {
  asm volatile("mbarrier.init.shared::cta.b64 [%0], %1;" ::"r"(smem_u32(bar)), "r"(count) : "memory");
}
__device__ __forceinline__ bool mbar_try_wait(uint64_t* bar, uint32_t parity) {
  uint32_t ok;
  asm volatile("{\n\t.reg .pred p;\n\tmbarrier.try_wait.parity.shared::cta.b64 p, [%1], %2;\n\tselp.u32 %0, 1, 0, p;\n\t}"
               : "=r"(ok) : "r"(smem_u32(bar)), "r"(parity) : "memory");
  return ok != 0;
}
__device__ __forceinline__ void mbar_wait(uint64_t* bar, uint32_t parity, int* err) {
  uint32_t spins = 0;
  while (!mbar_try_wait(bar, parity)) {
    if (++spins > (1u << 22)) { if (err) atomicExch(err, 1); break; }
  }
}
__device__ __forceinline__ void fence_proxy_async_smem() { asm volatile("fence.proxy.async.shared::cta;" ::: "memory"); }
__device__ __forceinline__ void tc_fence_before() { asm volatile("tcgen05.fence::before_thread_sync;" ::: "memory"); }
__device__ __forceinline__ void tc_fence_after() { asm volatile("tcgen05.fence::after_thread_sync;" ::: "memory"); }
__device__ __forceinline__ void tc_commit(uint64_t* bar) {
  asm volatile("tcgen05.commit.cta_group::1.mbarrier::arrive::one.shared::cluster.b64 [%0];" ::"r"(smem_u32(bar)) : "memory");
}
__device__ __forceinline__ void umma_ss(uint32_t tmem_d, uint64_t da, uint64_t db, uint32_t idesc, uint32_t accumulate) {
  asm volatile("{\n\t.reg .pred p;\n\tsetp.ne.b32 p, %4, 0;\n\ttcgen05.mma.cta_group::1.kind::tf32 [%0], %1, %2, %3, p;\n\t}"
               ::"r"(tmem_d), "l"(da), "l"(db), "r"(idesc), "r"(accumulate) : "memory");
}
__device__ __forceinline__ void umma_ts(uint32_t tmem_d, uint32_t tmem_a, uint64_t db, uint32_t idesc, uint32_t accumulate) {
  asm volatile("{\n\t.reg .pred p;\n\tsetp.ne.b32 p, %4, 0;\n\ttcgen05.mma.cta_group::1.kind::tf32 [%0], [%1], %2, %3, p;\n\t}"
               ::"r"(tmem_d), "r"(tmem_a), "l"(db), "r"(idesc), "r"(accumulate) : "memory");
}
__device__ __forceinline__ uint64_t make_desc(uint32_t smem_addr, uint32_t lbo_bytes, uint32_t sbo_bytes) {
  uint64_t d = 0;
  d |= (uint64_t)((smem_addr >> 4) & 0x3FFF);
  d |= (uint64_t)((lbo_bytes >> 4) & 0x3FFF) << 16;
  d |= (uint64_t)((sbo_bytes >> 4) & 0x3FFF) << 32;
  d |= (uint64_t)1 << 46;
  return d;
}
__device__ __forceinline__ uint32_t make_idesc(int M, int N) {
  return (1u << 4) | (2u << 7) | (2u << 10) | ((uint32_t)(N >> 3) << 17) | ((uint32_t)(M >> 4) << 24);
}
__device__ __forceinline__ void tmem_ld16(uint32_t addr, float (&v)[16]) {
  uint32_t r[16];
  asm volatile("tcgen05.ld.sync.aligned.32x32b.x16.b32 {%0, %1, %2, %3, %4, %5, %6, %7, %8, %9, %10, %11, %12, %13, %14, %15}, [%16];"
               : "=r"(r[0]), "=r"(r[1]), "=r"(r[2]), "=r"(r[3]), "=r"(r[4]), "=r"(r[5]), "=r"(r[6]), "=r"(r[7]), "=r"(r[8]), "=r"(r[9]),
                 "=r"(r[10]), "=r"(r[11]), "=r"(r[12]), "=r"(r[13]), "=r"(r[14]), "=r"(r[15])
               : "r"(addr) : "memory");
  asm volatile("tcgen05.wait::ld.sync.aligned;" ::: "memory");
#pragma unroll
  for (int i = 0; i < 16; ++i) v[i] = __uint_as_float(r[i]);
}
__device__ __forceinline__ void tmem_st16(uint32_t addr, const uint32_t (&r)[16]) {
  asm volatile("tcgen05.st.sync.aligned.32x32b.x16.b32 [%0], {%1, %2, %3, %4, %5, %6, %7, %8, %9, %10, %11, %12, %13, %14, %15, %16};"
               ::"r"(addr), "r"(r[0]), "r"(r[1]), "r"(r[2]), "r"(r[3]), "r"(r[4]), "r"(r[5]), "r"(r[6]), "r"(r[7]), "r"(r[8]), "r"(r[9]),
                 "r"(r[10]), "r"(r[11]), "r"(r[12]), "r"(r[13]), "r"(r[14]), "r"(r[15]) : "memory");
}

struct Geometry {
  int spt;
  int qtiles;
  int nk;
};
__host__ __device__ inline Geometry geometry(int T) {
  Geometry g;
  if (T <= 64) { g.spt = 2; g.qtiles = 1; g.nk = 128; }
  else { g.spt = 1; g.qtiles = (T + kRows - 1) / kRows; g.nk = (T + 15) / 16 * 16; }
  return g;
}
inline size_t smem_bytes(int T) {
  const Geometry g = geometry(T);
  return (size_t)(2 * kChunks * kRows * 4 + 2 * kChunks * g.nk * 4 + 2 * (g.nk / 4) * kNV * 4) * 4 + (size_t)g.nk * 4 + 64 + 1024;
}

}

__global__ void __launch_bounds__(tc::kThreads, 1)
k_attn_fwd_tc(const float* __restrict__ Q, const float* __restrict__ K, const float* __restrict__ V, const float* __restrict__ QIN,
              const int* __restrict__ mask, float* __restrict__ Y, float* __restrict__ ML, int B, int T, int n_units, int* __restrict__ err) {
  using namespace tc;
  extern __shared__ unsigned char smem_raw[];
  unsigned char* base = reinterpret_cast<unsigned char*>((reinterpret_cast<uintptr_t>(smem_raw) + 1023) & ~(uintptr_t)1023);
  const Geometry g = geometry(T);
  const int NK = g.nk;
  float* Qh = reinterpret_cast<float*>(base);
  float* Ql = Qh + kChunks * kRows * 4;
  float* Kh = Ql + kChunks * kRows * 4;
  float* Kl = Kh + kChunks * NK * 4;
  float* Vh = Kl + kChunks * NK * 4;
  float* Vl = Vh + (NK / 4) * kNV * 4;
  int* kmask = reinterpret_cast<int*>(Vl + (NK / 4) * kNV * 4);
  uint32_t* tmem_slot = reinterpret_cast<uint32_t*>(kmask + NK);
  uint64_t* bar = reinterpret_cast<uint64_t*>(tmem_slot + 2);
  const int tid = threadIdx.x, warp = tid >> 5;
  if (tid == 0) {
    mbar_init(bar, 1);
    asm volatile("fence.mbarrier_init.release.cluster;" ::: "memory");
  }
  if (warp == 0) {
    asm volatile("tcgen05.alloc.cta_group::1.sync.aligned.shared::cta.b32 [%0], %1;" ::"r"(smem_u32(tmem_slot)), "r"(kTmemCols) : "memory");
    asm volatile("tcgen05.relinquish_alloc_permit.cta_group::1.sync.aligned;" ::: "memory");
  }
  tc_fence_before();
  __syncthreads();
  tc_fence_after();
  const uint32_t tmem = *tmem_slot;
  const uint32_t lane_base = tmem + ((uint32_t)(warp * 32) << 16);
  const uint32_t idesc_s = make_idesc(kRows, NK), idesc_o = make_idesc(kRows, kNV);
  const float rscale = 1.0f / sqrtf((float)kD);
  uint32_t phase = 0;

  for (int unit = blockIdx.x; unit < n_units; unit += gridDim.x) {
    const int b0 = unit * g.spt;
    for (int i = tid; i < NK * kChunks; i += kThreads) {
      const int kk = i % NK, c = i / NK;
      const int sl = g.spt == 2 ? kk >> 6 : 0, t = g.spt == 2 ? (kk & 63) : kk;
      const bool ok = t < T && b0 + sl < B;
      float4 kv = f4_zero(), vv = f4_zero();
      if (ok) {
        const int64_t gofs = ((int64_t)(b0 + sl) * T + t) * kD + 4 * c;
        kv = ld4(K + gofs);
        vv = ld4(V + gofs);
      }
      uint4 h, l;
      split_tf32(kv.x, h.x, l.x); split_tf32(kv.y, h.y, l.y); split_tf32(kv.z, h.z, l.z); split_tf32(kv.w, h.w, l.w);
      *reinterpret_cast<uint4*>(Kh + (c * NK + kk) * 4) = h;
      *reinterpret_cast<uint4*>(Kl + (c * NK + kk) * 4) = l;
      const float ve[4] = {vv.x, vv.y, vv.z, vv.w};
#pragma unroll
      for (int e = 0; e < 4; ++e) {
        uint32_t vh, vl;
        split_tf32(ve[e], vh, vl);
        const int o = ((kk >> 2) * kNV + 4 * c + e) * 4 + (kk & 3);
        reinterpret_cast<uint32_t*>(Vh)[o] = vh;
        reinterpret_cast<uint32_t*>(Vl)[o] = vl;
      }
    }
    for (int i = tid; i < (NK / 4) * (kNV - kD) * 4; i += kThreads) {
      const int ch = i / ((kNV - kD) * 4), rem = i % ((kNV - kD) * 4);
      const int o = (ch * kNV + kD) * 4 + rem;
      Vh[o] = 0.f; Vl[o] = 0.f;
    }
    for (int kk = tid; kk < NK; kk += kThreads) {
      const int sl = g.spt == 2 ? kk >> 6 : 0, t = g.spt == 2 ? (kk & 63) : kk;
      kmask[kk] = (t < T && b0 + sl < B) ? (mask[(int64_t)(b0 + sl) * T + t] != 0 ? 1 : 0) : -1;
    }
    for (int qt = 0; qt < g.qtiles; ++qt) {
      for (int i = tid; i < kRows * kChunks; i += kThreads) {
        const int r = i % kRows, c = i / kRows;
        const int sl = g.spt == 2 ? r >> 6 : 0, t = g.spt == 2 ? (r & 63) : qt * kRows + r;
        float4 qv = f4_zero();
        if (t < T && b0 + sl < B) qv = ld4(Q + ((int64_t)(b0 + sl) * T + t) * kD + 4 * c);
        uint4 h, l;
        split_tf32(qv.x, h.x, l.x); split_tf32(qv.y, h.y, l.y); split_tf32(qv.z, h.z, l.z); split_tf32(qv.w, h.w, l.w);
        *reinterpret_cast<uint4*>(Qh + (c * kRows + r) * 4) = h;
        *reinterpret_cast<uint4*>(Ql + (c * kRows + r) * 4) = l;
      }
      fence_proxy_async_smem();
      tc_fence_before();
      __syncthreads();
      tc_fence_after();
      if (tid == 0) {
        const uint32_t lbo_q = kRows * 16, lbo_k = (uint32_t)NK * 16, sbo = 128;
        uint32_t acc = 0;
#pragma unroll
        for (int ks = 0; ks < kD / 8; ++ks) {
          const uint64_t dqh = make_desc(smem_u32(Qh) + 2 * ks * lbo_q, lbo_q, sbo), dql = make_desc(smem_u32(Ql) + 2 * ks * lbo_q, lbo_q, sbo);
          const uint64_t dkh = make_desc(smem_u32(Kh) + 2 * ks * lbo_k, lbo_k, sbo), dkl = make_desc(smem_u32(Kl) + 2 * ks * lbo_k, lbo_k, sbo);
          umma_ss(tmem, dql, dkh, idesc_s, acc); acc = 1;
          umma_ss(tmem, dqh, dkl, idesc_s, 1);
          umma_ss(tmem, dqh, dkh, idesc_s, 1);
        }
        tc_commit(bar);
      }
      mbar_wait(bar, phase, err); phase ^= 1;
      tc_fence_after();
      const int r = tid;
      const int sl = g.spt == 2 ? r >> 6 : 0, tq = g.spt == 2 ? (r & 63) : qt * kRows + r;
      const bool row_ok = tq < T && b0 + sl < B;
      const int c_lo = g.spt == 2 ? 64 * sl : 0, c_hi = g.spt == 2 ? 64 * sl + 64 : NK;
      float m = -INFINITY;
      for (int c0 = c_lo; c0 < c_hi; c0 += 16) {
        float s[16];
        tmem_ld16(lane_base + (uint32_t)c0, s);
#pragma unroll
        for (int j = 0; j < 16; ++j) {
          const int km = kmask[c0 + j];
          if (km >= 0) m = fmaxf(m, km ? s[j] * rscale : kMaskNeg);
        }
      }
      float lsum = 0.f;
      for (int c0 = 0; c0 < NK; c0 += 16) {
        uint32_t ph[16], pl[16];
        if (c0 >= c_lo && c0 < c_hi) {
          float s[16];
          tmem_ld16(lane_base + (uint32_t)c0, s);
#pragma unroll
          for (int j = 0; j < 16; ++j) {
            const int km = kmask[c0 + j];
            float p = 0.f;
            if (km >= 0) p = expf((km ? s[j] * rscale : kMaskNeg) - m);
            lsum += p;
            split_tf32(p, ph[j], pl[j]);
          }
        } else {
#pragma unroll
          for (int j = 0; j < 16; ++j) { ph[j] = 0u; pl[j] = 0u; }
        }
        tmem_st16(lane_base + (uint32_t)c0, ph);
        tmem_st16(lane_base + kColPlo + (uint32_t)c0, pl);
      }
      asm volatile("tcgen05.wait::st.sync.aligned;" ::: "memory");
      tc_fence_before();
      __syncthreads();
      tc_fence_after();
      if (tid == 0) {
        const uint32_t lbo_v = kNV * 16, sbo = 128;
        uint32_t acc = 0;
        for (int ks = 0; ks < NK / 8; ++ks) {
          const uint64_t dvh = make_desc(smem_u32(Vh) + 2 * ks * lbo_v, lbo_v, sbo), dvl = make_desc(smem_u32(Vl) + 2 * ks * lbo_v, lbo_v, sbo);
          umma_ts(tmem + kColO, tmem + kColPlo + 8 * ks, dvh, idesc_o, acc); acc = 1;
          umma_ts(tmem + kColO, tmem + 8 * ks, dvl, idesc_o, 1);
          umma_ts(tmem + kColO, tmem + 8 * ks, dvh, idesc_o, 1);
        }
        tc_commit(bar);
      }
      mbar_wait(bar, phase, err); phase ^= 1;
      tc_fence_after();
      {
        float o[48];
#pragma unroll
        for (int c0 = 0; c0 < kNV; c0 += 16) {
          float v[16];
          tmem_ld16(lane_base + kColO + (uint32_t)c0, v);
#pragma unroll
          for (int j = 0; j < 16; ++j) o[c0 + j] = v[j];
        }
        if (row_ok) {
          const int64_t tok = (int64_t)(b0 + sl) * T + tq;
          const float inv = 1.0f / lsum;
#pragma unroll
          for (int i = 0; i < kChunks; ++i) {
            const float4 q = ld4(QIN + tok * kD + 4 * i);
            st4(Y + tok * kD + 4 * i, make_float4(fmaf(o[4 * i], inv, q.x), fmaf(o[4 * i + 1], inv, q.y), fmaf(o[4 * i + 2], inv, q.z),
                                                  fmaf(o[4 * i + 3], inv, q.w)));
          }
          ML[2 * tok] = m;
          ML[2 * tok + 1] = lsum;
        }
      }
      tc_fence_before();
      __syncthreads();
      tc_fence_after();
    }
  }
  if (warp == 0) asm volatile("tcgen05.dealloc.cta_group::1.sync.aligned.b32 %0, %1;" ::"r"(tmem), "r"(kTmemCols) : "memory");
}

bool attn_tc_supported(int T) { return T >= 1 && tc::geometry(T).nk <= tc::kMaxNK; }

int init_attn_tc_kernels(int max_T) {
  size_t need = 0;
  for (int T = 1; T <= max_T; ++T)
    if (attn_tc_supported(T)) need = need > tc::smem_bytes(T) ? need : tc::smem_bytes(T);
  if (need == 0) return 0;
  return cudaFuncSetAttribute((const void*)k_attn_fwd_tc, cudaFuncAttributeMaxDynamicSharedMemorySize, (int)need) == cudaSuccess ? 0 : -1;
}

void launch_attn_fwd_tc(const float* Q, const float* K, const float* V, const float* QIN, const int* mask, float* Y, float* ML, int B, int T,
                        int n_sm, int* err, cudaStream_t st) {
  PAMREC_PROF("attn_fwd", 1, st);
  if (B == 0) return;
  const tc::Geometry g = tc::geometry(T);
  const int n_units = (B + g.spt - 1) / g.spt;
  const int grid = n_units < n_sm ? n_units : n_sm;
  k_attn_fwd_tc<<<grid, tc::kThreads, tc::smem_bytes(T), st>>>(Q, K, V, QIN, mask, Y, ML, B, T, n_units, err);
}

}
```

pamrec_b200/csrc/kernels_encoder.cu:

```cuda
#include "kernels.h"
#include "mma.cuh"

namespace pamrec {

constexpr int kEmbU = 8;
constexpr int kEmbTok = 32;
__global__ void __launch_bounds__(kEmbTok * 10, 3)
k_embed_fwd(const int* __restrict__ ih, const int* __restrict__ ch, const int* __restrict__ items,
            const int* __restrict__ cates, const float* __restrict__ item_w, const float* __restrict__ cate_w,
            const float* __restrict__ pos, float* __restrict__ x0, float* __restrict__ tgt, int64_t n_tok, int T) {
  constexpr int TOK = kEmbTok * kEmbU;
  __shared__ int s_id[4][TOK];
  __shared__ int s_t[TOK];
  const int tid = threadIdx.x;
  const int64_t tok0 = (int64_t)blockIdx.x * TOK;
  for (int i = tid; i < TOK; i += kEmbTok * 10) {
    const int64_t tok = tok0 + i;
    if (tok < n_tok) {
      const int64_t b = tok / T;
      s_t[i] = (int)(tok - b * T);
      s_id[0][i] = __ldg(ih + tok);
      s_id[1][i] = __ldg(ch + tok);
      s_id[2][i] = __ldg(items + b);
      s_id[3][i] = __ldg(cates + b);
    }
  }
  __syncthreads();
  const int c = tid % 10, tl = tid / 10;
  const int which = c < 4 ? 0 : (c == 4 ? 1 : (c < 9 ? 2 : 3));
  const bool is_item = (which & 1) == 0;
  const int sub = c < 4 ? c : (c < 9 && c > 4 ? c - 5 : 0);
  const float* table = is_item ? item_w : cate_w;
  const int width = is_item ? kI : kC;
  float4 v[kEmbU];
#pragma unroll
  for (int j = 0; j < kEmbU; ++j) {
    const int i = j * kEmbTok + tl;
    if (tok0 + i < n_tok) v[j] = __ldg(reinterpret_cast<const float4*>(table + (int64_t)s_id[which][i] * width) + sub);
  }
#pragma unroll
  for (int j = 0; j < kEmbU; ++j) {
    const int i = j * kEmbTok + tl;
    const int64_t tok = tok0 + i;
    if (tok < n_tok) {
      const int t = s_t[i];
      if (tgt != nullptr && t == 0 && c >= 5) st4(tgt + (tok / T) * kE + 4 * (c - 5), v[j]);
      const float4 p = __ldg(reinterpret_cast<const float4*>(pos + t * kD) + c);
      float4 o = v[j];
      o.x += p.x; o.y += p.y; o.z += p.z; o.w += p.w;
      st4(x0 + tok * kD + 4 * c, o);
    }
  }
}

void launch_embed_fwd(const int* ih, const int* ch, const int* items, const int* cates, const float* item_w,
                      const float* cate_w, const float* pos, float* x0, float* tgt, int64_t n_rows, int T,
                      cudaStream_t st) {
  PAMREC_PROF("embed_fwd", 1, st);
  const int64_t n_tok = n_rows * T;
  if (n_tok == 0) return;
  const int64_t per_cta = (int64_t)kEmbU * kEmbTok;
  k_embed_fwd<<<(unsigned)((n_tok + per_cta - 1) / per_cta), kEmbTok * 10, 0, st>>>(ih, ch, items, cates, item_w, cate_w, pos, x0,
                                                                                  tgt, n_tok, T);
}

__global__ void k_bucket_hist(const float* __restrict__ lt, int n, int* __restrict__ bucket, int* __restrict__ ctl) {
  __shared__ int h[16];
  if (threadIdx.x < 16) h[threadIdx.x] = 0;
  __syncthreads();
  int i = blockIdx.x * blockDim.x + threadIdx.x;
  if (i < n) {
    int k = (int)lt[i];
    k = min(max(k, 0), kNB - 1);
    bucket[i] = k;
    atomicAdd(&h[k], 1);
  }
  __syncthreads();
  if (threadIdx.x < kNB && h[threadIdx.x]) atomicAdd(&ctl[threadIdx.x], h[threadIdx.x]);
}

__global__ void k_bucket_plan(int* __restrict__ ctl, int* __restrict__ tile_bucket, int* __restrict__ tile_begin,
                              int* __restrict__ tile_count) {
  if (threadIdx.x != 0 || blockIdx.x != 0) return;
  int start = 0, nt = 0;
  for (int k = 0; k < kNB; ++k) {
    int cnt = ctl[k];
    ctl[16 + k] = start;
    for (int o = 0; o < cnt; o += kTokTile) {
      tile_bucket[nt] = k;
      tile_begin[nt] = start + o;
      tile_count[nt] = min(kTokTile, cnt - o);
      ++nt;
    }
    start += cnt;
  }
  ctl[32] = nt;
}

__global__ void k_bucket_scatter(const int* __restrict__ bucket, int n, int* __restrict__ ctl, int* __restrict__ perm) {
  __shared__ int h[16], base[16];
  if (threadIdx.x < 16) h[threadIdx.x] = 0;
  __syncthreads();
  int i = blockIdx.x * blockDim.x + threadIdx.x;
  int k = -1, r = 0;
  if (i < n) { k = bucket[i]; r = atomicAdd(&h[k], 1); }
  __syncthreads();
  if (threadIdx.x < kNB) base[threadIdx.x] = h[threadIdx.x] ? atomicAdd(&ctl[16 + threadIdx.x], h[threadIdx.x]) : 0;
  __syncthreads();
  if (i < n) perm[base[k] + r] = i;
}

void launch_bucket_plan(const float* lt, int n, int* bucket, int* perm, int* ctl, int* tile_bucket, int* tile_begin,
                        int* tile_count, cudaStream_t st) {
  PAMREC_PROF("bucket_plan", 3, st);
  cudaMemsetAsync(ctl, 0, 64 * sizeof(int), st);
  if (n == 0) return;
  int g = (n + 255) / 256;
  k_bucket_hist<<<g, 256, 0, st>>>(lt, n, bucket, ctl);
  k_bucket_plan<<<1, 32, 0, st>>>(ctl, tile_bucket, tile_begin, tile_count);
  k_bucket_scatter<<<g, 256, 0, st>>>(bucket, n, ctl, perm);
}

constexpr int kTileIt = (kTokTile * 10 + kTokThreads - 1) / kTokThreads;

constexpr int kTS = 44;
__device__ __forceinline__ void load_split_mat(uint32_t* __restrict__ hi, uint32_t* __restrict__ lo, const float* __restrict__ W, int tid);
__device__ __forceinline__ void load_tile44(float* __restrict__ dst, const float* __restrict__ src, const int* toks, int cnt, int tid);
constexpr int kLnWriteF = 1, kLnWriteXhat = 2;
__device__ __forceinline__ void ln_row44(float* __restrict__ row, const float* __restrict__ beta, const float* __restrict__ gamma,
                                         float& mean, float& rstd, int write);
__device__ __forceinline__ void store_frag_rows(float* __restrict__ dst, const float (&c)[kMT][5][4], int64_t tok0, const int* toks,
                                                int row_base, int cnt, int lane);

constexpr int kProjFwdSmem = (6 * kDD + 2 * kTokTile * kTS + 2 * kD) * 4;
__global__ void __launch_bounds__(kTokThreads)
k_proj_fwd(const float* __restrict__ X, const int* __restrict__ perm, const int* __restrict__ ctl,
           const int* __restrict__ tile_bucket, const int* __restrict__ tile_begin, const int* __restrict__ tile_count,
           const float* __restrict__ Wq, const float* __restrict__ Wk, const float* __restrict__ Wv,
           const float* __restrict__ ln_beta, const float* __restrict__ ln_gamma, float* __restrict__ QIN,
           float* __restrict__ Q, float* __restrict__ K, float* __restrict__ V) {
  int tile = blockIdx.x;
  if (tile >= ctl[32]) return;
  extern __shared__ __align__(16) float sm[];
  uint32_t* Whi = reinterpret_cast<uint32_t*>(sm);
  uint32_t* Wlo = Whi + 3 * kDD;
  float* xs = sm + 6 * kDD;
  float* qs = xs + kTokTile * kTS;
  float* lnp = qs + kTokTile * kTS;
  __shared__ int toks[kTokTile];
  const int tid = threadIdx.x, lane = tid & 31, w = tid >> 5;
  const int k = tile_bucket[tile], begin = tile_begin[tile], cnt = tile_count[tile];
  load_split_mat(Whi, Wlo, Wq + (int64_t)k * kDD, tid);
  load_split_mat(Whi + kDD, Wlo + kDD, Wk + (int64_t)k * kDD, tid);
  load_split_mat(Whi + 2 * kDD, Wlo + 2 * kDD, Wv + (int64_t)k * kDD, tid);
  if (tid < kD) { lnp[tid] = ln_beta[tid]; lnp[kD + tid] = ln_gamma[tid]; }
  if (tid < cnt) toks[tid] = perm[begin + tid];
  __syncthreads();
  load_tile44(xs, X, toks, cnt, tid);
  __syncthreads();
  if (tid < kTokTile) {
    float* xr = xs + tid * kTS;
    float* qr = qs + tid * kTS;
#pragma unroll
    for (int i = 0; i < 10; ++i) st4(qr + 4 * i, ld4(xr + 4 * i));
    float mean, rstd;
    ln_row44(qr, lnp, lnp + kD, mean, rstd, kLnWriteF);
    if (tid < cnt) {
      float* o = QIN + (int64_t)toks[tid] * kD;
#pragma unroll
      for (int i = 0; i < 10; ++i) st4(o + 4 * i, ld4(qr + 4 * i));
    }
  }
  __syncthreads();
  const float* xw = xs + kWarpRows * w * kTS;
  const float* qw = qs + kWarpRows * w * kTS;
#pragma unroll 1
  for (int m = 0; m < 3; ++m) {
    float c[kMT][5][4];
#pragma unroll
    for (int mt = 0; mt < kMT; ++mt)
#pragma unroll
      for (int nt = 0; nt < 5; ++nt)
#pragma unroll
        for (int q = 0; q < 4; ++q) c[mt][nt][q] = 0.f;
    const float* aw = m == 0 ? qw : xw;
    warp_gemm_rows_x40x40<kMT, false>(c, [&](int r, int kk) { return aw[r * kTS + kk]; }, Whi + m * kDD, Wlo + m * kDD, lane);
    store_frag_rows(m == 0 ? Q : (m == 1 ? K : V), c, 0, toks, kWarpRows * w, cnt, lane);
  }
}

void launch_proj_fwd(const float* X, const int* perm, const int* ctl, const int* tile_bucket, const int* tile_begin,
                     const int* tile_count, int max_tiles, const float* Wq, const float* Wk, const float* Wv,
                     const float* ln_beta, const float* ln_gamma, float* QIN, float* Q, float* K, float* V,
                     cudaStream_t st) {
  PAMREC_PROF("proj_fwd", 1, st);
  k_proj_fwd<<<max_tiles, kTokThreads, kProjFwdSmem, st>>>(X, perm, ctl, tile_bucket, tile_begin, tile_count, Wq, Wk, Wv,
                                                        ln_beta, ln_gamma, QIN, Q, K, V);
}

constexpr int kAttnCh = 8;
__host__ __device__ inline int attn_nw(int T) { return (T + 31) / 32; }
__host__ __device__ inline int attn_spb(int T) { int nw = attn_nw(T); return nw >= 4 ? 1 : 4 / nw; }
__host__ __device__ inline int attn_fwd_per(int T) { return 2 * T * kAttnStride + 2 * ((T + 3) & ~3) + 4; }
__device__ __forceinline__ void attn_live_list(const int* __restrict__ mk, int T, int lane, int* __restrict__ lv, int* __restrict__ nl) {
  int base = 0;
  for (int c = 0; c < T; c += 32) {
    const int j = c + lane;
    const bool live = j < T && mk[j] != 0;
    const unsigned bal = __ballot_sync(0xffffffffu, live);
    if (live) lv[base + __popc(bal & ((1u << lane) - 1u))] = j;
    base += __popc(bal);
  }
  if (lane == 0) *nl = base;
}
inline size_t attn_fwd_smem(int T) { return (size_t)attn_spb(T) * attn_fwd_per(T) * 4; }

__device__ __forceinline__ float dot40(const float4 (&q)[10], const float* __restrict__ row) {
  float4 r = ld4(row);
  float4 a = make_float4(q[0].x * r.x, q[0].y * r.y, q[0].z * r.z, q[0].w * r.w);
#pragma unroll
  for (int i = 1; i < 10; ++i) {
    r = ld4(row + 4 * i);
    a.x = fmaf(q[i].x, r.x, a.x); a.y = fmaf(q[i].y, r.y, a.y); a.z = fmaf(q[i].z, r.z, a.z); a.w = fmaf(q[i].w, r.w, a.w);
  }
  return (a.x + a.y) + (a.z + a.w);
}

__global__ void __launch_bounds__(256)
k_attn_fwd(const float* __restrict__ Q, const float* __restrict__ K, const float* __restrict__ V,
           const float* __restrict__ QIN, const int* __restrict__ mask, float* __restrict__ Y, float* __restrict__ ML,
           int B, int T) {
  extern __shared__ __align__(16) float sm[];
  const int nw = attn_nw(T), spb = attn_spb(T), tps = nw * 32;
  const int per = attn_fwd_per(T);
  const int tid = threadIdx.x;
  const int b0 = blockIdx.x * spb;
  const int ns = min(spb, B - b0);
  for (int i = tid; i < ns * T * 10; i += blockDim.x) {
    const int sl = i / (T * 10), rc = i % (T * 10), r = rc / 10, c = rc % 10;
    const int64_t g = ((int64_t)(b0 + sl) * T + r) * kD + 4 * c;
    float* base = sm + sl * per;
    st4(base + r * kAttnStride + 4 * c, ld4(K + g));
    st4(base + T * kAttnStride + r * kAttnStride + 4 * c, ld4(V + g));
  }
  for (int i = tid; i < ns * T; i += blockDim.x) {
    const int sl = i / T, r = i % T;
    reinterpret_cast<int*>(sm + sl * per + 2 * T * kAttnStride)[r] = mask[(int64_t)(b0 + sl) * T + r];
  }
  __syncthreads();
  const int sl = tid / tps, t = tid % tps;
  const int T4 = (T + 3) & ~3;
  if (sl < ns && t < 32) {
    int* mki = reinterpret_cast<int*>(sm + sl * per + 2 * T * kAttnStride);
    attn_live_list(mki, T, t, mki + T4, mki + 2 * T4);
  }
  __syncthreads();
  if (sl >= ns || t >= T) return;
  const float* Ks = sm + sl * per;
  const float* Vs = Ks + T * kAttnStride;
  const int* lv = reinterpret_cast<const int*>(Vs + T * kAttnStride) + T4;
  const int nl = lv[T4];
  const int64_t row = ((int64_t)(b0 + sl) * T + t) * kD;
  float4 q[10], o[10];
#pragma unroll
  for (int i = 0; i < 10; ++i) { q[i] = ld4(Q + row + 4 * i); o[i] = f4_zero(); }
  const float rscale = 1.0f / sqrtf((float)kD);
  float m = -INFINITY, l = 0.f;
  for (int k0 = 0; k0 < nl; k0 += kAttnCh) {
    float sc[kAttnCh];
    float cm = -INFINITY;
#pragma unroll
    for (int jj = 0; jj < kAttnCh; ++jj) {
      const int k = k0 + jj;
      float val = -INFINITY;
      if (k < nl) val = dot40(q, Ks + lv[k] * kAttnStride) * rscale;
      sc[jj] = val;
      cm = fmaxf(cm, val);
    }
    const float mn = fmaxf(m, cm);
    const float corr = expf(m - mn);
    l *= corr;
#pragma unroll
    for (int i = 0; i < 10; ++i) { o[i].x *= corr; o[i].y *= corr; o[i].z *= corr; o[i].w *= corr; }
#pragma unroll
    for (int jj = 0; jj < kAttnCh; ++jj) {
      const int k = k0 + jj;
      if (k < nl) {
        const float pj = expf(sc[jj] - mn);
        l += pj;
        const float* vr = Vs + lv[k] * kAttnStride;
#pragma unroll
        for (int i = 0; i < 10; ++i) f4_fma(o[i], pj, ld4(vr + 4 * i));
      }
    }
    m = mn;
  }
  if (nl == 0) {
    m = kMaskNeg; l = (float)T;
    for (int j = 0; j < T; ++j) {
#pragma unroll
      for (int i = 0; i < 10; ++i) f4_fma(o[i], 1.0f, ld4(Vs + j * kAttnStride + 4 * i));
    }
  }
  const float inv = 1.0f / l;
#pragma unroll
  for (int i = 0; i < 10; ++i) {
    const float4 r = ld4(QIN + row + 4 * i);
    st4(Y + row + 4 * i, make_float4(fmaf(o[i].x, inv, r.x), fmaf(o[i].y, inv, r.y), fmaf(o[i].z, inv, r.z), fmaf(o[i].w, inv, r.w)));
  }
  ML[2 * ((int64_t)(b0 + sl) * T + t)] = m;
  ML[2 * ((int64_t)(b0 + sl) * T + t) + 1] = l;
}

void launch_attn_fwd(const float* Q, const float* K, const float* V, const float* QIN, const int* mask, float* Y, float* ML,
                     int B, int T, cudaStream_t st) {
  PAMREC_PROF("attn_fwd", 1, st);
  if (B == 0) return;
  const size_t smem = attn_fwd_smem(T);
  const int spb = attn_spb(T), threads = spb * attn_nw(T) * 32;
  k_attn_fwd<<<(B + spb - 1) / spb, threads, smem, st>>>(Q, K, V, QIN, mask, Y, ML, B, T);
}

__device__ __forceinline__ void load_split_mat(uint32_t* __restrict__ hi, uint32_t* __restrict__ lo, const float* __restrict__ W,
                                               int tid) {
  constexpr int IT = (kDD / 4 + kTokThreads - 1) / kTokThreads;
  float4 v[IT];
#pragma unroll
  for (int it = 0; it < IT; ++it) {
    const int i = tid + it * kTokThreads;
    if (i < kDD / 4) v[it] = ld4(W + 4 * i);
  }
#pragma unroll
  for (int it = 0; it < IT; ++it) {
    const int i = tid + it * kTokThreads;
    if (i < kDD / 4) {
      uint4 h, l;
      split_tf32(v[it].x, h.x, l.x); split_tf32(v[it].y, h.y, l.y); split_tf32(v[it].z, h.z, l.z); split_tf32(v[it].w, h.w, l.w);
      *reinterpret_cast<uint4*>(hi + 4 * i) = h;
      *reinterpret_cast<uint4*>(lo + 4 * i) = l;
    }
  }
}
__device__ __forceinline__ void load_tile44(float* __restrict__ dst, const float* __restrict__ src, const int* toks, int cnt, int tid) {
  float4 v[kTileIt];
#pragma unroll
  for (int it = 0; it < kTileIt; ++it) {
    const int i = tid + it * kTokThreads;
    const int r = i / 10, c = i % 10;
    v[it] = f4_zero();
    if (r < cnt) v[it] = toks ? ld4(src + (int64_t)toks[r] * kD + 4 * c) : ld4(src + 4 * (int64_t)i);
  }
#pragma unroll
  for (int it = 0; it < kTileIt; ++it) {
    const int i = tid + it * kTokThreads;
    st4(dst + (i / 10) * kTS + 4 * (i % 10), v[it]);
  }
}
__device__ __forceinline__ void ln_row44(float* __restrict__ row, const float* __restrict__ beta, const float* __restrict__ gamma,
                                         float& mean, float& rstd, int write) {
  float4 x[10];
  float sacc = 0.f;
#pragma unroll
  for (int i = 0; i < 10; ++i) { x[i] = ld4(row + 4 * i); sacc += (x[i].x + x[i].y) + (x[i].z + x[i].w); }
  mean = sacc * (1.0f / kD);
  float v = 0.f;
#pragma unroll
  for (int i = 0; i < 10; ++i) {
    float a = x[i].x - mean, b = x[i].y - mean, c = x[i].z - mean, d = x[i].w - mean;
    v = fmaf(a, a, v); v = fmaf(b, b, v); v = fmaf(c, c, v); v = fmaf(d, d, v);
  }
  rstd = 1.0f / sqrtf(v * (1.0f / kD) + kLnEps);
  if (write == kLnWriteXhat) {
#pragma unroll
    for (int i = 0; i < 10; ++i)
      st4(row + 4 * i, make_float4((x[i].x - mean) * rstd, (x[i].y - mean) * rstd, (x[i].z - mean) * rstd, (x[i].w - mean) * rstd));
  } else if (write == kLnWriteF) {
#pragma unroll
    for (int i = 0; i < 10; ++i) {
      const float4 g = ld4(gamma + 4 * i), b = ld4(beta + 4 * i);
      st4(row + 4 * i, make_float4(fmaf(g.x, (x[i].x - mean) * rstd, b.x), fmaf(g.y, (x[i].y - mean) * rstd, b.y),
                                   fmaf(g.z, (x[i].z - mean) * rstd, b.z), fmaf(g.w, (x[i].w - mean) * rstd, b.w)));
    }
  }
}

constexpr int kFfnFwdSmem = (4 * kDD + 2 * kTokTile * kTS + 4 * kD) * 4;
__global__ void __launch_bounds__(kTokThreads)
k_ffn_fwd(const float* __restrict__ Y, const float* __restrict__ W1, const float* __restrict__ b1,
          const float* __restrict__ W2, const float* __restrict__ b2, const float* __restrict__ ln_beta,
          const float* __restrict__ ln_gamma, float* __restrict__ OUT, float* __restrict__ Hdbg, int n_tok) {
  extern __shared__ __align__(16) float sm[];
  uint32_t* W1hi = reinterpret_cast<uint32_t*>(sm);
  uint32_t* W1lo = W1hi + kDD;
  uint32_t* W2hi = W1lo + kDD;
  uint32_t* W2lo = W2hi + kDD;
  float* fs = sm + 4 * kDD;
  float* hs = fs + kTokTile * kTS;
  float* pr = hs + kTokTile * kTS;
  const int tid = threadIdx.x, lane = tid & 31, w = tid >> 5;
  const int64_t tok0 = (int64_t)blockIdx.x * kTokTile;
  const int cnt = (int)min((int64_t)kTokTile, (int64_t)n_tok - tok0);
  load_split_mat(W1hi, W1lo, W1, tid);
  load_split_mat(W2hi, W2lo, W2, tid);
  if (tid < kD) { pr[tid] = b1[tid]; pr[kD + tid] = b2[tid]; pr[2 * kD + tid] = ln_beta[tid]; pr[3 * kD + tid] = ln_gamma[tid]; }
  load_tile44(fs, Y + tok0 * kD, nullptr, cnt, tid);
  __syncthreads();
  if (tid < kTokTile) {
    float mean, rstd;
    ln_row44(fs + tid * kTS, pr + 2 * kD, pr + 3 * kD, mean, rstd, kLnWriteF);
  }
  __syncthreads();
  const int g = lane >> 2, t = lane & 3;
  const float* fw = fs + kWarpRows * w * kTS;
  float* hw = hs + kWarpRows * w * kTS;
  float c[kMT][5][4];
#pragma unroll
  for (int mt = 0; mt < kMT; ++mt)
#pragma unroll
    for (int nt = 0; nt < 5; ++nt) {
      const float b0 = pr[8 * nt + 2 * t], bb1 = pr[8 * nt + 2 * t + 1];
      c[mt][nt][0] = b0; c[mt][nt][1] = bb1; c[mt][nt][2] = b0; c[mt][nt][3] = bb1;
    }
  warp_gemm_rows_x40x40<kMT, false>(c, [&](int r, int k) { return fw[r * kTS + k]; }, W1hi, W1lo, lane);
#pragma unroll
  for (int mt = 0; mt < kMT; ++mt)
#pragma unroll
    for (int nt = 0; nt < 5; ++nt) {
      const int r = 16 * mt + g, col = 8 * nt + 2 * t;
      *reinterpret_cast<float2*>(hw + r * kTS + col) = make_float2(fmaxf(c[mt][nt][0], 0.f), fmaxf(c[mt][nt][1], 0.f));
      *reinterpret_cast<float2*>(hw + (r + 8) * kTS + col) = make_float2(fmaxf(c[mt][nt][2], 0.f), fmaxf(c[mt][nt][3], 0.f));
    }
  __syncwarp();
  if (Hdbg != nullptr) {
    for (int i = lane; i < kWarpRows * kD; i += 32) {
      const int r = i / kD, col = i % kD;
      if (kWarpRows * w + r < cnt) Hdbg[(tok0 + kWarpRows * w + r) * kD + col] = hw[r * kTS + col];
    }
  }
#pragma unroll
  for (int mt = 0; mt < kMT; ++mt)
#pragma unroll
    for (int nt = 0; nt < 5; ++nt) {
      const int r = 16 * mt + g, col = 8 * nt + 2 * t;
      const float2 f0 = *reinterpret_cast<const float2*>(fw + r * kTS + col);
      const float2 f1 = *reinterpret_cast<const float2*>(fw + (r + 8) * kTS + col);
      const float b0 = pr[kD + col], bb1 = pr[kD + col + 1];
      c[mt][nt][0] = b0 + f0.x; c[mt][nt][1] = bb1 + f0.y; c[mt][nt][2] = b0 + f1.x; c[mt][nt][3] = bb1 + f1.y;
    }
  warp_gemm_rows_x40x40<kMT, false>(c, [&](int r, int k) { return hw[r * kTS + k]; }, W2hi, W2lo, lane);
#pragma unroll
  for (int mt = 0; mt < kMT; ++mt)
#pragma unroll
    for (int nt = 0; nt < 5; ++nt) {
      const int r = kWarpRows * w + 16 * mt + g, col = 8 * nt + 2 * t;
      if (r < cnt) *reinterpret_cast<float2*>(OUT + (tok0 + r) * kD + col) = make_float2(c[mt][nt][0], c[mt][nt][1]);
      if (r + 8 < cnt) *reinterpret_cast<float2*>(OUT + (tok0 + r + 8) * kD + col) = make_float2(c[mt][nt][2], c[mt][nt][3]);
    }
}

void launch_ffn_fwd(const float* Y, const float* W1, const float* b1, const float* W2, const float* b2,
                    const float* ln_beta, const float* ln_gamma, float* OUT, float* Hdbg, int n_tok, cudaStream_t st) {
  PAMREC_PROF("ffn_fwd", 1, st);
  if (n_tok == 0) return;
  k_ffn_fwd<<<(n_tok + kTokTile - 1) / kTokTile, kTokThreads, kFfnFwdSmem, st>>>(Y, W1, b1, W2, b2, ln_beta, ln_gamma, OUT, Hdbg, n_tok);
}

template <typename XF>
__device__ __forceinline__ void ln_bwd_frag(float (&d)[kMT][5][4], XF xhat2, const float* __restrict__ rstd_w,
                                            const float* __restrict__ gamma, float* __restrict__ red, int lane) {
  const int g = lane >> 2, t = lane & 3;
  float sb[5][2], sg[5][2];
#pragma unroll
  for (int nt = 0; nt < 5; ++nt) { sb[nt][0] = sb[nt][1] = sg[nt][0] = sg[nt][1] = 0.f; }
#pragma unroll
  for (int mt = 0; mt < kMT; ++mt) {
#pragma unroll
    for (int h = 0; h < 2; ++h) {
      const int r = 16 * mt + g + 8 * h;
      float m1 = 0.f, m2 = 0.f;
      float xh[5][2];
#pragma unroll
      for (int nt = 0; nt < 5; ++nt) {
        const int col = 8 * nt + 2 * t;
        const float2 x = xhat2(r, col);
        xh[nt][0] = x.x; xh[nt][1] = x.y;
        const float d0 = d[mt][nt][2 * h], d1 = d[mt][nt][2 * h + 1];
        sb[nt][0] += d0; sb[nt][1] += d1;
        sg[nt][0] = fmaf(d0, x.x, sg[nt][0]); sg[nt][1] = fmaf(d1, x.y, sg[nt][1]);
        const float e0 = d0 * gamma[col], e1 = d1 * gamma[col + 1];
        m1 += e0 + e1;
        m2 = fmaf(e0, x.x, m2); m2 = fmaf(e1, x.y, m2);
      }
      m1 += __shfl_xor_sync(0xffffffffu, m1, 1); m1 += __shfl_xor_sync(0xffffffffu, m1, 2);
      m2 += __shfl_xor_sync(0xffffffffu, m2, 1); m2 += __shfl_xor_sync(0xffffffffu, m2, 2);
      m1 *= (1.0f / kD); m2 *= (1.0f / kD);
      const float rs = rstd_w[r];
#pragma unroll
      for (int nt = 0; nt < 5; ++nt) {
        const int col = 8 * nt + 2 * t;
        d[mt][nt][2 * h] = rs * (d[mt][nt][2 * h] * gamma[col] - m1 - xh[nt][0] * m2);
        d[mt][nt][2 * h + 1] = rs * (d[mt][nt][2 * h + 1] * gamma[col + 1] - m1 - xh[nt][1] * m2);
      }
    }
  }
#pragma unroll
  for (int nt = 0; nt < 5; ++nt)
#pragma unroll
    for (int j = 0; j < 2; ++j) {
      float a = sb[nt][j], b = sg[nt][j];
#pragma unroll
      for (int o = 4; o < 32; o <<= 1) { a += __shfl_xor_sync(0xffffffffu, a, o); b += __shfl_xor_sync(0xffffffffu, b, o); }
      if (g == 0) { atomicAdd(red + 8 * nt + 2 * t + j, a); atomicAdd(red + kD + 8 * nt + 2 * t + j, b); }
    }
}
__device__ __forceinline__ void store_frag_rows(float* __restrict__ dst, const float (&c)[kMT][5][4], int64_t tok0, const int* toks,
                                                int row_base, int cnt, int lane) {
  const int g = lane >> 2, t = lane & 3;
#pragma unroll
  for (int mt = 0; mt < kMT; ++mt)
#pragma unroll
    for (int h = 0; h < 2; ++h) {
      const int r = row_base + 16 * mt + g + 8 * h;
      if (r < cnt) {
        float* o = dst + (toks ? (int64_t)toks[r] : tok0 + r) * kD + 2 * t;
#pragma unroll
        for (int nt = 0; nt < 5; ++nt) *reinterpret_cast<float2*>(o + 8 * nt) = make_float2(c[mt][nt][2 * h], c[mt][nt][2 * h + 1]);
      }
    }
}

constexpr int kFfnBwdSmem = (4 * kDD + 3 * kTokTile * kTS + 2 * 41 * kD + 4 * kD + 2 * kD + kTokTile) * 4;
__global__ void __launch_bounds__(kTokThreads)
k_ffn_bwd(const float* __restrict__ Y, const float* __restrict__ dOUT, const float* __restrict__ W1,
          const float* __restrict__ b1, const float* __restrict__ W2, const float* __restrict__ ln_beta,
          const float* __restrict__ ln_gamma, float* __restrict__ dY, float* __restrict__ dW1, float* __restrict__ db1,
          float* __restrict__ dW2, float* __restrict__ db2, float* __restrict__ dbeta, float* __restrict__ dgamma,
          int n_tok) {
  extern __shared__ __align__(16) float sm[];
  uint32_t* W1hi = reinterpret_cast<uint32_t*>(sm);
  uint32_t* W1lo = W1hi + kDD;
  uint32_t* W2hi = W1lo + kDD;
  uint32_t* W2lo = W2hi + kDD;
  float* xs = sm + 4 * kDD;
  float* hs = xs + kTokTile * kTS;
  float* gs = hs + kTokTile * kTS;
  float* acc2 = gs + kTokTile * kTS;
  float* acc1 = acc2 + 41 * kD;
  float* pr = acc1 + 41 * kD;
  float* red = pr + 4 * kD;
  float* rstd_s = red + 2 * kD;
  const int tid = threadIdx.x, lane = tid & 31, w = tid >> 5;
  const int g = lane >> 2, t = lane & 3;
  const int64_t tok0 = (int64_t)blockIdx.x * kTokTile;
  const int cnt = (int)min((int64_t)kTokTile, (int64_t)n_tok - tok0);
  load_split_mat(W1hi, W1lo, W1, tid);
  load_split_mat(W2hi, W2lo, W2, tid);
  if (tid < kD) { pr[tid] = b1[tid]; pr[2 * kD + tid] = ln_beta[tid]; pr[3 * kD + tid] = ln_gamma[tid]; }
  if (tid < 2 * kD) red[tid] = 0.f;
  for (int i = tid; i < 2 * 41 * kD; i += kTokThreads) acc2[i] = 0.f;
  load_tile44(xs, Y + tok0 * kD, nullptr, cnt, tid);
  load_tile44(gs, dOUT + tok0 * kD, nullptr, cnt, tid);
  __syncthreads();
  if (tid < kTokTile) {
    float mean, rstd;
    ln_row44(xs + tid * kTS, pr + 2 * kD, pr + 3 * kD, mean, rstd, kLnWriteXhat);
    rstd_s[tid] = rstd;
  }
  __syncthreads();
  const float* xw = xs + kWarpRows * w * kTS;
  float* hw = hs + kWarpRows * w * kTS;
  const float* gw = gs + kWarpRows * w * kTS;
  const float* beta = pr + 2 * kD;
  const float* gamma = pr + 3 * kD;
  auto f_elem = [&](int r, int k) { return fmaf(gamma[k], xw[r * kTS + k], beta[k]); };
  float c[kMT][5][4];
#pragma unroll
  for (int mt = 0; mt < kMT; ++mt)
#pragma unroll
    for (int nt = 0; nt < 5; ++nt) {
      const float b0 = pr[8 * nt + 2 * t], bb1 = pr[8 * nt + 2 * t + 1];
      c[mt][nt][0] = b0; c[mt][nt][1] = bb1; c[mt][nt][2] = b0; c[mt][nt][3] = bb1;
    }
  warp_gemm_rows_x40x40<kMT, false>(c, f_elem, W1hi, W1lo, lane);
#pragma unroll
  for (int mt = 0; mt < kMT; ++mt)
#pragma unroll
    for (int nt = 0; nt < 5; ++nt) {
      const int r = 16 * mt + g, col = 8 * nt + 2 * t;
      *reinterpret_cast<float2*>(hw + r * kTS + col) = make_float2(fmaxf(c[mt][nt][0], 0.f), fmaxf(c[mt][nt][1], 0.f));
      *reinterpret_cast<float2*>(hw + (r + 8) * kTS + col) = make_float2(fmaxf(c[mt][nt][2], 0.f), fmaxf(c[mt][nt][3], 0.f));
    }
  __syncwarp();
#pragma unroll
  for (int mt = 0; mt < kMT; ++mt)
#pragma unroll
    for (int nt = 0; nt < 5; ++nt)
#pragma unroll
      for (int q = 0; q < 4; ++q) c[mt][nt][q] = 0.f;
  warp_gemm_rows_x40x40<kMT, true>(c, [&](int r, int k) { return gw[r * kTS + k]; }, W2hi, W2lo, lane);
#pragma unroll
  for (int mt = 0; mt < kMT; ++mt)
#pragma unroll
    for (int nt = 0; nt < 5; ++nt) {
      const int r = 16 * mt + g, col = 8 * nt + 2 * t;
      const float2 h0 = *reinterpret_cast<const float2*>(hw + r * kTS + col);
      const float2 h1 = *reinterpret_cast<const float2*>(hw + (r + 8) * kTS + col);
      if (!(h0.x > 0.f)) c[mt][nt][0] = 0.f;
      if (!(h0.y > 0.f)) c[mt][nt][1] = 0.f;
      if (!(h1.x > 0.f)) c[mt][nt][2] = 0.f;
      if (!(h1.y > 0.f)) c[mt][nt][3] = 0.f;
    }
  {
    float cw[3][5][4];
#pragma unroll
    for (int mt = 0; mt < 3; ++mt)
#pragma unroll
      for (int nt = 0; nt < 5; ++nt)
#pragma unroll
        for (int q = 0; q < 4; ++q) cw[mt][nt][q] = 0.f;
    warp_gemm_tn_48x40(cw, kWarpRows, [&](int r, int i) { return i < kD ? hw[r * kTS + i] : (i == kD ? 1.f : 0.f); },
                       [&](int r, int n) { return gw[r * kTS + n]; }, lane);
    tn_flush_smem(cw, acc2, lane);
  }
  __syncwarp();
#pragma unroll
  for (int mt = 0; mt < kMT; ++mt)
#pragma unroll
    for (int nt = 0; nt < 5; ++nt) {
      const int r = 16 * mt + g, col = 8 * nt + 2 * t;
      *reinterpret_cast<float2*>(hw + r * kTS + col) = make_float2(c[mt][nt][0], c[mt][nt][1]);
      *reinterpret_cast<float2*>(hw + (r + 8) * kTS + col) = make_float2(c[mt][nt][2], c[mt][nt][3]);
    }
  __syncwarp();
#pragma unroll
  for (int mt = 0; mt < kMT; ++mt)
#pragma unroll
    for (int nt = 0; nt < 5; ++nt) {
      const int r = 16 * mt + g, col = 8 * nt + 2 * t;
      const float2 g0 = *reinterpret_cast<const float2*>(gw + r * kTS + col);
      const float2 g1 = *reinterpret_cast<const float2*>(gw + (r + 8) * kTS + col);
      c[mt][nt][0] = g0.x; c[mt][nt][1] = g0.y; c[mt][nt][2] = g1.x; c[mt][nt][3] = g1.y;
    }
  warp_gemm_rows_x40x40<kMT, true>(c, [&](int r, int k) { return hw[r * kTS + k]; }, W1hi, W1lo, lane);
  {
    float cw[3][5][4];
#pragma unroll
    for (int mt = 0; mt < 3; ++mt)
#pragma unroll
      for (int nt = 0; nt < 5; ++nt)
#pragma unroll
        for (int q = 0; q < 4; ++q) cw[mt][nt][q] = 0.f;
    warp_gemm_tn_48x40(cw, kWarpRows, [&](int r, int i) { return i < kD ? f_elem(r, i) : (i == kD ? 1.f : 0.f); },
                       [&](int r, int n) { return hw[r * kTS + n]; }, lane);
    tn_flush_smem(cw, acc1, lane);
  }
  ln_bwd_frag(c, [&](int r, int col) { return *reinterpret_cast<const float2*>(xw + r * kTS + col); }, rstd_s + kWarpRows * w, gamma, red, lane);
  store_frag_rows(dY, c, tok0, nullptr, kWarpRows * w, cnt, lane);
  __syncthreads();
  for (int i = tid; i < kDD; i += kTokThreads) { atomicAdd(dW2 + i, acc2[i]); atomicAdd(dW1 + i, acc1[i]); }
  if (tid < kD) {
    atomicAdd(db2 + tid, acc2[kDD + tid]); atomicAdd(db1 + tid, acc1[kDD + tid]);
    atomicAdd(dbeta + tid, red[tid]); atomicAdd(dgamma + tid, red[kD + tid]);
  }
}

void launch_ffn_bwd(const float* Y, const float* dOUT, const float* W1, const float* b1, const float* W2,
                    const float* ln_beta, const float* ln_gamma, float* dY, float* dW1, float* db1, float* dW2,
                    float* db2, float* dbeta, float* dgamma, int n_tok, cudaStream_t st) {
  PAMREC_PROF("ffn_bwd", 1, st);
  if (n_tok == 0) return;
  k_ffn_bwd<<<(n_tok + kTokTile - 1) / kTokTile, kTokThreads, kFfnBwdSmem, st>>>(Y, dOUT, W1, b1, W2, ln_beta, ln_gamma, dY, dW1,
                                                                             db1, dW2, db2, dbeta, dgamma, n_tok);
}

__host__ __device__ inline int attn_bwd_per(int T) { return 4 * T * kAttnStride + ((5 * T + 4 + 3) & ~3); }
inline size_t attn_bwd_smem(int T) { return (size_t)attn_spb(T) * attn_bwd_per(T) * 4; }

__global__ void __launch_bounds__(256)
k_attn_bwd(const float* __restrict__ Q, const float* __restrict__ K, const float* __restrict__ V,
           const float* __restrict__ dY, const float* __restrict__ Y, const float* __restrict__ QIN,
           const float* __restrict__ ML, const int* __restrict__ mask, float* __restrict__ dQ, float* __restrict__ dK,
           float* __restrict__ dV, int B, int T) {
  extern __shared__ __align__(16) float sm[];
  const int nw = attn_nw(T), spb = attn_spb(T), tps = nw * 32;
  const int TS = T * kAttnStride;
  const int per = attn_bwd_per(T);
  const int tid = threadIdx.x;
  const int b0 = blockIdx.x * spb;
  const int ns = min(spb, B - b0);
  for (int i = tid; i < ns * T * 10; i += blockDim.x) {
    const int sl = i / (T * 10), rc = i % (T * 10), r = rc / 10, c = rc % 10;
    const int64_t g = ((int64_t)(b0 + sl) * T + r) * kD + 4 * c;
    float* base = sm + sl * per + r * kAttnStride + 4 * c;
    st4(base, ld4(K + g));
    st4(base + TS, ld4(V + g));
    st4(base + 2 * TS, ld4(Q + g));
    st4(base + 3 * TS, ld4(dY + g));
  }
  const int sl = tid / tps, t = tid % tps;
  const bool active = sl < ns && t < T;
  float* S = sm + sl * per;
  if (active) {
    const int64_t tok = (int64_t)(b0 + sl) * T + t;
    float d = 0.f;
#pragma unroll
    for (int i = 0; i < 10; ++i) {
      const float4 g = ld4(dY + tok * kD + 4 * i), y = ld4(Y + tok * kD + 4 * i), r = ld4(QIN + tok * kD + 4 * i);
      d = fmaf(g.x, y.x - r.x, d); d = fmaf(g.y, y.y - r.y, d); d = fmaf(g.z, y.z - r.z, d); d = fmaf(g.w, y.w - r.w, d);
    }
    S[4 * TS + t] = ML[2 * tok];
    S[4 * TS + T + t] = 1.0f / ML[2 * tok + 1];
    S[4 * TS + 2 * T + t] = d;
    reinterpret_cast<int*>(S + 4 * TS + 3 * T)[t] = mask[tok];
  }
  __syncthreads();
  if (sl < ns && t < 32) {
    int* mki = reinterpret_cast<int*>(S + 4 * TS + 3 * T);
    attn_live_list(mki, T, t, mki + T, mki + 2 * T);
  }
  __syncthreads();
  if (!active) return;
  const float* Ks = S;
  const float* Vs = S + TS;
  const float* Qs = S + 2 * TS;
  const float* Gs = S + 3 * TS;
  const float* rm = S + 4 * TS;
  const float* ril = rm + T;
  const float* rD = ril + T;
  const int* mk = reinterpret_cast<const int*>(rD + T);
  const int* lv = mk + T;
  const int nl = lv[T];
  const float rscale = 1.0f / sqrtf((float)kD);
  const int64_t row = ((int64_t)(b0 + sl) * T + t) * kD;
  {
    float4 q[10], g[10], acc[10];
#pragma unroll
    for (int i = 0; i < 10; ++i) { q[i] = ld4(Qs + t * kAttnStride + 4 * i); g[i] = ld4(Gs + t * kAttnStride + 4 * i); acc[i] = f4_zero(); }
    const float mt = rm[t], il = ril[t], Dt = rD[t];
#pragma unroll 2
    for (int k = 0; k < nl; ++k) {
      const int j = lv[k];
      const float* kr = Ks + j * kAttnStride;
      const float sv = dot40(q, kr) * rscale;
      const float p = expf(sv - mt) * il;
      const float dp = dot40(g, Vs + j * kAttnStride);
      const float ds = p * (dp - Dt) * rscale;
#pragma unroll
      for (int i = 0; i < 10; ++i) f4_fma(acc[i], ds, ld4(kr + 4 * i));
    }
#pragma unroll
    for (int i = 0; i < 10; ++i) st4(dQ + row + 4 * i, acc[i]);
  }
  {
    const int j = t;
    float4 kj[10], vj[10], ak[10], av[10];
#pragma unroll
    for (int i = 0; i < 10; ++i) { kj[i] = ld4(Ks + j * kAttnStride + 4 * i); vj[i] = ld4(Vs + j * kAttnStride + 4 * i); ak[i] = f4_zero(); av[i] = f4_zero(); }
    const int mkj = mk[j];
    const int tq_end = (mkj || nl == 0) ? T : 0;
    for (int tt = 0; tt < tq_end; ++tt) {
      const float* qr = Qs + tt * kAttnStride;
      const float* gr = Gs + tt * kAttnStride;
      const float sv = mkj ? dot40(kj, qr) * rscale : kMaskNeg;
      const float p = expf(sv - rm[tt]) * ril[tt];
      const float dp = dot40(vj, gr);
      const float ds = mkj ? p * (dp - rD[tt]) * rscale : 0.f;
#pragma unroll
      for (int i = 0; i < 10; ++i) { f4_fma(ak[i], ds, ld4(qr + 4 * i)); f4_fma(av[i], p, ld4(gr + 4 * i)); }
    }
#pragma unroll
    for (int i = 0; i < 10; ++i) { st4(dK + row + 4 * i, ak[i]); st4(dV + row + 4 * i, av[i]); }
  }
}

void launch_attn_bwd(const float* Q, const float* K, const float* V, const float* dY, const float* Y, const float* QIN,
                     const float* ML, const int* mask, float* dQ, float* dK, float* dV, int B, int T, cudaStream_t st) {
  PAMREC_PROF("attn_bwd", 1, st);
  if (B == 0) return;
  const size_t smem = attn_bwd_smem(T);
  const int spb = attn_spb(T), threads = spb * attn_nw(T) * 32;
  k_attn_bwd<<<(B + spb - 1) / spb, threads, smem, st>>>(Q, K, V, dY, Y, QIN, ML, mask, dQ, dK, dV, B, T);
}

constexpr int kProjBwdSmem = (6 * kDD + 2 * kTokTile * kTS + kDD + 2 * kD + 2 * kD + 2 * kTokTile) * 4;
__global__ void __launch_bounds__(kTokThreads)
k_proj_bwd(const float* __restrict__ X, const float* __restrict__ dY, const float* __restrict__ dQ,
           const float* __restrict__ dK, const float* __restrict__ dV, const int* __restrict__ perm,
           const int* __restrict__ ctl, const int* __restrict__ tile_bucket, const int* __restrict__ tile_begin,
           const int* __restrict__ tile_count, const float* __restrict__ Wq, const float* __restrict__ Wk,
           const float* __restrict__ Wv, const float* __restrict__ ln_beta, const float* __restrict__ ln_gamma,
           float* __restrict__ dX, float* __restrict__ dWq, float* __restrict__ dWk, float* __restrict__ dWv,
           float* __restrict__ dbeta, float* __restrict__ dgamma) {
  int tile = blockIdx.x;
  if (tile >= ctl[32]) return;
  extern __shared__ __align__(16) float sm[];
  uint32_t* Whi = reinterpret_cast<uint32_t*>(sm);
  uint32_t* Wlo = Whi + 3 * kDD;
  float* xs = sm + 6 * kDD;
  float* gs = xs + kTokTile * kTS;
  float* acc = gs + kTokTile * kTS;
  float* lnp = acc + kDD;
  float* red = lnp + 2 * kD;
  float* mean_s = red + 2 * kD;
  float* rstd_s = mean_s + kTokTile;
  __shared__ int toks[kTokTile];
  const int tid = threadIdx.x, lane = tid & 31, w = tid >> 5;
  const int g = lane >> 2, t = lane & 3;
  const int k = tile_bucket[tile], begin = tile_begin[tile], cnt = tile_count[tile];
  load_split_mat(Whi, Wlo, Wq + (int64_t)k * kDD, tid);
  load_split_mat(Whi + kDD, Wlo + kDD, Wk + (int64_t)k * kDD, tid);
  load_split_mat(Whi + 2 * kDD, Wlo + 2 * kDD, Wv + (int64_t)k * kDD, tid);
  if (tid < kD) { lnp[tid] = ln_beta[tid]; lnp[kD + tid] = ln_gamma[tid]; }
  if (tid < 2 * kD) red[tid] = 0.f;
  for (int i = tid; i < kDD; i += kTokThreads) acc[i] = 0.f;
  if (tid < cnt) toks[tid] = perm[begin + tid];
  __syncthreads();
  load_tile44(xs, X, toks, cnt, tid);
  load_tile44(gs, dQ, toks, cnt, tid);
  __syncthreads();
  if (tid < kTokTile) {
    float mean, rstd;
    ln_row44(xs + tid * kTS, lnp, lnp + kD, mean, rstd, 0);
    mean_s[tid] = mean; rstd_s[tid] = rstd;
  }
  __syncthreads();
  const float* xw = xs + kWarpRows * w * kTS;
  const float* gw = gs + kWarpRows * w * kTS;
  const float* mw = mean_s + kWarpRows * w;
  const float* rw = rstd_s + kWarpRows * w;
  const float* beta = lnp;
  const float* gamma = lnp + kD;
  auto xhat = [&](int r, int i) { return (xw[r * kTS + i] - mw[r]) * rw[r]; };
  auto g_elem = [&](int r, int kk) { return gw[r * kTS + kk]; };
  float dqin[kMT][5][4], dx[kMT][5][4];
#pragma unroll
  for (int mt = 0; mt < kMT; ++mt)
#pragma unroll
    for (int h = 0; h < 2; ++h) {
      const int r = kWarpRows * w + 16 * mt + g + 8 * h;
      const float* src = dY + (int64_t)toks[r < cnt ? r : 0] * kD + 2 * t;
#pragma unroll
      for (int nt = 0; nt < 5; ++nt) {
        const float2 v = r < cnt ? *reinterpret_cast<const float2*>(src + 8 * nt) : make_float2(0.f, 0.f);
        dqin[mt][nt][2 * h] = v.x; dqin[mt][nt][2 * h + 1] = v.y;
      }
    }
  warp_gemm_rows_x40x40<kMT, true>(dqin, g_elem, Whi, Wlo, lane);
  {
    float cw[3][5][4];
#pragma unroll
    for (int mt = 0; mt < 3; ++mt)
#pragma unroll
      for (int nt = 0; nt < 5; ++nt)
#pragma unroll
        for (int q = 0; q < 4; ++q) cw[mt][nt][q] = 0.f;
    warp_gemm_tn_48x40(cw, kWarpRows, [&](int r, int i) { return i < kD ? fmaf(gamma[i], xhat(r, i), beta[i]) : 0.f; }, g_elem, lane);
    tn_flush_smem(cw, acc, lane, kD - 1);
  }
  float* dWs[3] = {dWq + (int64_t)k * kDD, dWk + (int64_t)k * kDD, dWv + (int64_t)k * kDD};
  auto flush_acc = [&](float* dW) {
    __syncthreads();
    for (int i = tid; i < kDD; i += kTokThreads) { atomicAdd(dW + i, acc[i]); acc[i] = 0.f; }
  };
  flush_acc(dWs[0]);
#pragma unroll
  for (int mt = 0; mt < kMT; ++mt)
#pragma unroll
    for (int nt = 0; nt < 5; ++nt)
#pragma unroll
      for (int q = 0; q < 4; ++q) dx[mt][nt][q] = 0.f;
#pragma unroll 1
  for (int m = 1; m < 3; ++m) {
    __syncthreads();
    load_tile44(gs, m == 1 ? dK : dV, toks, cnt, tid);
    __syncthreads();
    warp_gemm_rows_x40x40<kMT, true>(dx, g_elem, Whi + m * kDD, Wlo + m * kDD, lane);
    float cw[3][5][4];
#pragma unroll
    for (int mt = 0; mt < 3; ++mt)
#pragma unroll
      for (int nt = 0; nt < 5; ++nt)
#pragma unroll
        for (int q = 0; q < 4; ++q) cw[mt][nt][q] = 0.f;
    warp_gemm_tn_48x40(cw, kWarpRows, [&](int r, int i) { return i < kD ? xw[r * kTS + i] : 0.f; }, g_elem, lane);
    tn_flush_smem(cw, acc, lane, kD - 1);
    flush_acc(dWs[m]);
  }
  ln_bwd_frag(dqin, [&](int r, int col) { return make_float2(xhat(r, col), xhat(r, col + 1)); }, rw, gamma, red, lane);
#pragma unroll
  for (int mt = 0; mt < kMT; ++mt)
#pragma unroll
    for (int nt = 0; nt < 5; ++nt)
#pragma unroll
      for (int q = 0; q < 4; ++q) dx[mt][nt][q] += dqin[mt][nt][q];
  store_frag_rows(dX, dx, 0, toks, kWarpRows * w, cnt, lane);
  __syncthreads();
  if (tid < kD) { atomicAdd(dbeta + tid, red[tid]); atomicAdd(dgamma + tid, red[kD + tid]); }
}

void launch_proj_bwd(const float* X, const float* dY, const float* dQ, const float* dK, const float* dV, const int* perm,
                     const int* ctl, const int* tile_bucket, const int* tile_begin, const int* tile_count, int max_tiles,
                     const float* Wq, const float* Wk, const float* Wv, const float* ln_beta, const float* ln_gamma,
                     float* dX, float* dWq, float* dWk, float* dWv, float* dbeta, float* dgamma, cudaStream_t st) {
  PAMREC_PROF("proj_bwd", 1, st);
  k_proj_bwd<<<max_tiles, kTokThreads, kProjBwdSmem, st>>>(X, dY, dQ, dK, dV, perm, ctl, tile_bucket, tile_begin, tile_count, Wq,
                                                        Wk, Wv, ln_beta, ln_gamma, dX, dWq, dWk, dWv, dbeta, dgamma);
}

int init_encoder_kernels(int max_T) {
  cudaError_t e = cudaSuccess;
  auto set = [&](const void* fn, size_t bytes) {
    if (e == cudaSuccess) e = cudaFuncSetAttribute(fn, cudaFuncAttributeMaxDynamicSharedMemorySize, (int)bytes);
  };
  set((const void*)k_proj_fwd, kProjFwdSmem);
  set((const void*)k_ffn_fwd, kFfnFwdSmem);
  set((const void*)k_ffn_bwd, kFfnBwdSmem);
  set((const void*)k_proj_bwd, kProjBwdSmem);
  size_t af = 0, ab = 0;
  for (int T = 1; T <= max_T; ++T) { af = af > attn_fwd_smem(T) ? af : attn_fwd_smem(T); ab = ab > attn_bwd_smem(T) ? ab : attn_bwd_smem(T); }
  set((const void*)k_attn_fwd, af);
  set((const void*)k_attn_bwd, ab);
  return e == cudaSuccess ? 0 : -1;
}

}
```

pamrec_b200/csrc/layout.h:

```cpp
#pragma once
#include <cstdio>
#include <cstring>
#include <map>
#include <string>
#include <vector>

#include "common.cuh"

namespace pamrec {

struct TensorDesc {
  std::string name;
  int pool = 0, dtype = PAMREC_F32, flags = 0;
  int64_t offset = 0, numel = 0;
  int ndim = 0;
  int64_t shape[4] = {0, 0, 0, 0};
};

struct BlockOff { int64_t ln_a_beta, ln_a_gamma, wq, wk, wv, w1, b1, w2, b2, ln_b_beta, ln_b_gamma; };
struct MlpOff { int64_t w0, b0, g0, be0, w1, b1, g1, be1, wout, bout; };
struct BnOff { int C; int64_t gamma, beta, mm, mv; };

enum BnId { BN_S0 = 0, BN_S1, BN_E0, BN_G0, BN_E1, BN_G1, BN_T0, BN_T1, BN_COUNT };

// ... 27 lines not shown
    TensorDesc t;
    t.name = name; t.pool = PAMREC_POOL_DENSE; t.flags = flags; t.offset = dense_numel;
    t.numel = 1; t.ndim = 0;
    for (int64_t s : shape) { t.shape[t.ndim++] = s; t.numel *= s; }
    dense_numel += t.numel;
    dense.push_back(t);
    return t.offset;
  }
  int64_t add_bn(const std::string& name, int64_t n) {
    TensorDesc t;
    t.name = name; t.pool = PAMREC_POOL_BN; t.offset = bn_numel; t.numel = n; t.ndim = 1; t.shape[0] = n;
    bn_numel += n;
    bn.push_back(t);
    return t.offset;
  }
  void add_ws(const std::string& name, int dtype, std::initializer_list<int64_t> shape) {
    TensorDesc t;
    t.name = name; t.pool = PAMREC_POOL_WORKSPACE; t.dtype = dtype; t.offset = (int64_t)ws_bytes;
    t.numel = 1; t.ndim = 0;
    for (int64_t s : shape) { t.shape[t.ndim++] = s; t.numel *= s; }
    size_t esz = (dtype == PAMREC_F64) ? 8 : (dtype == PAMREC_U8 ? 1 : 4);
    size_t bytes = (size_t)t.numel * esz;
    ws_bytes += (bytes + 255) / 256 * 256;
    ws_index[name] = ws.size();
    ws.push_back(t);
  }
  size_t ws_off(const std::string& name) const {
    auto it = ws_index.find(name);
    if (it == ws_index.end()) { fprintf(stderr, "pamrec: unknown workspace tensor %s\n", name.c_str()); abort(); }
    return (size_t)ws[it->second].offset;
  }

  MlpOff add_mlp(const std::vector<std::string>& scopes, const std::vector<int>& flags, int in, int h0, int h1, bool out,
                 BnOff* bn0, BnOff* bn1, bool live = true) {
    MlpOff o{};
    auto role = [&](const char* leaf, std::initializer_list<int64_t> shape) {
      int64_t first = -1;
      for (size_t g = 0; g < scopes.size(); ++g) {
        int64_t off = add_dense(scopes[g] + "/nn_part/" + leaf, shape, flags[g]);
        if (g == 0) first = off;
      }
      return first;
    };
    o.w0 = role("w_nn_layer0", {in, h0});
    o.b0 = role("b_nn_layer0", {h0});
    o.g0 = role("batch_normalization/gamma", {h0});
    o.be0 = role("batch_normalization/beta", {h0});
    o.w1 = role("w_nn_layer1", {h0, h1});
    o.b1 = role("b_nn_layer1", {h1});
    o.g1 = role("batch_normalization_1/gamma", {h1});
    o.be1 = role("batch_normalization_1/beta", {h1});
    o.wout = o.bout = -1;
    if (out) {
      o.wout = role("w_nn_output", {h1, 1});
      o.bout = role("b_nn_output", {1});
    }
    int G = (int)scopes.size();
    int64_t mm0 = -1, mv0 = -1, mm1 = -1, mv1 = -1;
    for (int g = 0; g < G; ++g) { int64_t x = add_bn(scopes[g] + "/nn_part/batch_normalization/moving_mean", h0); if (!g) mm0 = x; }
    for (int g = 0; g < G; ++g) { int64_t x = add_bn(scopes[g] + "/nn_part/batch_normalization/moving_variance", h0); if (!g) mv0 = x; }
    for (int g = 0; g < G; ++g) { int64_t x = add_bn(scopes[g] + "/nn_part/batch_normalization_1/moving_mean", h1); if (!g) mm1 = x; }
    for (int g = 0; g < G; ++g) { int64_t x = add_bn(scopes[g] + "/nn_part/batch_normalization_1/moving_variance", h1); if (!g) mv1 = x; }
    if (bn0) *bn0 = BnOff{G * h0, o.g0, o.be0, mm0, mv0};
    if (bn1) *bn1 = BnOff{G * h1, o.g1, o.be1, mm1, mv1};
    (void)live;
    return o;
  }

  void add_optim_ws() {
    add_ws("seg_id", PAMREC_I32, {dense_numel});
    add_ws("seg_tab", PAMREC_I32, {(int64_t)dense.size(), 4});
    add_ws("seg_normsq", PAMREC_F64, {(int64_t)dense.size()});
    add_ws("sp_normsq", PAMREC_F64, {8});
    add_ws("adam.step", PAMREC_F64, {2});
    add_ws("adam.lr", PAMREC_F32, {4});
  }
  void add_bn_ws() {
    const char* bn_names[BN_COUNT] = {"s0", "s1", "e0", "g0", "e1", "g1", "t0", "t1"};
    int64_t bn_c = 0;
    for (int i = 0; i < BN_COUNT; ++i) {
      std::string p = std::string("bn.") + bn_names[i];
      add_ws(p + ".sums", PAMREC_F64, {bnoff[i].C, 2});
      add_ws(p + ".stat", PAMREC_F32, {bnoff[i].C, 2});
      bn_bsums_off[i] = 2 * bn_c;
      bn_c += bnoff[i].C;
    }
    add_ws("bn.bsums", PAMREC_F64, {bn_c, 2});
    add_ws("bn.gsums", PAMREC_F64, {8, bn_c, 2});
    add_ws("bn.gbsums", PAMREC_F64, {8, bn_c, 2});
  }

  void build_sibling(const PamrecConfig& c) {
    const int L2 = PAMREC_SEG_L2;
    const int64_t B = Bcap, N = (int64_t)Bcap * T;
    const int E = emb_dim;
    const std::string clsr = "sequential/clsr/";
    att_mat = add_dense(clsr + "long_term/attention_fcn/attention_mat", {E, E}, L2);
    add_dense(clsr + "short_term/attention_fcn/attention_mat", {E, E}, L2);
    att = add_mlp({clsr + "long_term/attention_fcn/att_fcn", clsr + "short_term/attention_fcn/att_fcn"}, {L2, L2}, 4 * E, 80, 40, true,
                  &bnoff[BN_S0], &bnoff[BN_S1]);
    const int x_dim = 3 * E;
    std::vector<std::string> ex;
    if (model_kind == PAMREC_MODEL_MMOE) {
      for (int j = 0; j < 5; ++j) ex.push_back(clsr + "expert_" + std::to_string(j));
    } else if (model_kind == PAMREC_MODEL_PLE) {
      for (int j = 0; j < 3; ++j) ex.push_back(clsr + "share_expert_" + std::to_string(j));
      for (int j = 0; j < 2; ++j) ex.push_back(clsr + "main_expert_" + std::to_string(j));
      for (int j = 0; j < 2; ++j) ex.push_back(clsr + "sub_expert_" + std::to_string(j));
      const int ms[5] = {0, 1, 2, 3, 4}, ss[5] = {0, 1, 2, 5, 6};
      for (int j = 0; j < 5; ++j) { gate_sel[0][j] = ms[j]; gate_sel[1][j] = ss[j]; }
    }
    n_expert = (int)ex.size();
    if (n_expert) {
      expert = add_mlp(ex, std::vector<int>(ex.size(), L2), x_dim, 100, 64, false, &bnoff[BN_E0], &bnoff[BN_E1]);
      gate = add_mlp({clsr + "gate_main", clsr + "gate_sub"}, {L2, L2}, x_dim, 64, 5, false, &bnoff[BN_G0], &bnoff[BN_G1]);
      tower_in = 64 + E;
    } else {
      bnoff[BN_E0] = bnoff[BN_E1] = bnoff[BN_G0] = bnoff[BN_G1] = BnOff{0, 0, 0, 0, 0};
      tower_in = x_dim;
    }
    tower = add_mlp({"sequential/logit_fcn", "sequential/valid_logit_fcn"}, {L2, L2}, tower_in, 100, 64, true, &bnoff[BN_T0], &bnoff[BN_T1]);
    add_ws("sib.ids_item", PAMREC_I32, {2, N});
    add_ws("sib.ids_cate", PAMREC_I32, {2, N});
    add_ws("sib.h", PAMREC_F32, {2, N, E});
    add_ws("tgt", PAMREC_F32, {B, E});
    add_ws("sib.feat", PAMREC_F32, {N, 8 * E});
    add_ws("z1", PAMREC_F32, {N, 160});
    add_ws("z2", PAMREC_F32, {N, 80});
    add_ws("sib.score", PAMREC_F32, {N, 2});
    add_ws("sib.aw", PAMREC_F32, {2, N});
    add_ws("x", PAMREC_F32, {B, x_dim});
    add_ws("ze0", PAMREC_F32, {B, (int64_t)n_expert * 100});
    add_ws("zg0", PAMREC_F32, {B, n_expert ? 128 : 0});
    add_ws("ze1", PAMREC_F32, {B, (int64_t)n_expert * 64});
    add_ws("zg1", PAMREC_F32, {B, n_expert ? 10 : 0});
    add_ws("u", PAMREC_F32, {B, 2 * (64 + E)});
    add_ws("zt0", PAMREC_F32, {B, 200});
    add_ws("zt1", PAMREC_F32, {B, 128});
    add_ws("logits", PAMREC_F32, {B, 2});
    add_ws("losses", PAMREC_F32, {8});
    add_ws("loss_acc", PAMREC_F64, {8});
    add_ws("d_logits", PAMREC_F32, {B, 2});
    add_ws("d_t1", PAMREC_F32, {B, 128});
    add_ws("d_t0", PAMREC_F32, {B, 200});
    add_ws("d_u", PAMREC_F32, {B, 2 * (64 + E)});
    add_ws("d_e1", PAMREC_F32, {B, (int64_t)n_expert * 64});
    add_ws("d_g1", PAMREC_F32, {B, n_expert ? 10 : 0});
    add_ws("d_e0", PAMREC_F32, {B, (int64_t)n_expert * 100});
    add_ws("d_g0", PAMREC_F32, {B, n_expert ? 128 : 0});
    add_ws("d_x", PAMREC_F32, {B, x_dim});
    add_ws("d_tgt", PAMREC_F32, {B, E});
    add_ws("d_tgt_total", PAMREC_F32, {B, E});
    add_ws("sib.d_score", PAMREC_F32, {N, 2});
    add_ws("sib.d_a1", PAMREC_F32, {N, 80});
    add_ws("sib.d_a0", PAMREC_F32, {N, 160});
    add_ws("sib.d_feat", PAMREC_F32, {N, 8 * E});
    add_ws("sib.d_att", PAMREC_F32, {2, N, E});
    add_ws("sib.dq", PAMREC_F32, {B, 2, E});
    add_ws("sib.dh", PAMREC_F32, {2, N, E});
    add_ws("sib.zero", PAMREC_F32, {256});
    add_ws("sib.dummy", PAMREC_F32, {256});
    add_ws("sib.has0", PAMREC_I32, {4});
    add_bn_ws();
    add_optim_ws();
    const int64_t NK = 2 * N + B;
    cub_keys_table = NK;
    for (const char* t : {"item", "cate"}) {
      std::string p = std::string("sp.") + t + ".";
      for (const char* n : {"keys", "idx", "skeys", "sidx", "uidx", "ukeys"}) add_ws(p + n, PAMREC_I32, {NK});
      add_ws(p + "slot", PAMREC_I32, {t[0] == 'i' ? n_items : n_cates});
      add_ws(p + "accum", PAMREC_F32, {NK, t[0] == 'i' ? item_dim : cate_dim});
    }
    for (const char* n : {"keys", "idx", "skeys", "sidx", "uidx", "ukeys"}) add_ws(std::string("sp.user.") + n, PAMREC_I32, {B});
    add_ws("sp.user.slot", PAMREC_I32, {n_users});
    add_ws("sp.nuniq", PAMREC_I32, {8});
    add_ws("dp.scalars", PAMREC_F64, {8});
    cub_keys = NK;
    add_ws("cub_temp", PAMREC_U8, {(int64_t)(16u << 20) + 16 * cub_keys});
    (void)c;
  }

  struct SasBlock { int64_t ln_a_beta, ln_a_gamma, wqkv, bqkv, ln_b_beta, ln_b_gamma, w1, b1, w2, b2; };
  SasBlock sas[2];
  void build_sasrec(const PamrecConfig& c) {
    const int L2 = PAMREC_SEG_L2;
    const int64_t B = Bcap, N = (int64_t)Bcap * T;
    const int E = emb_dim;
    pos = add_dense("sequential/embedding/position_embedding", {T, E}, PAMREC_SEG_POS);
    for (int b = 0; b < 2; ++b) {
      const std::string p = "sequential/sasrec/num_blocks_" + std::to_string(b) + "/";
      SasBlock& o = sas[b];
      o.wqkv = add_dense(p + "self_attention/dense/kernel", {E, E}, L2);
      add_dense(p + "self_attention/dense_1/kernel", {E, E}, L2);
      add_dense(p + "self_attention/dense_2/kernel", {E, E}, L2);
      o.bqkv = add_dense(p + "self_attention/dense/bias", {E}, L2);
      add_dense(p + "self_attention/dense_1/bias", {E}, L2);
      add_dense(p + "self_attention/dense_2/bias", {E}, L2);
      o.ln_a_beta = add_dense(p + "ln/Variable", {E}, L2);
      o.ln_a_gamma = add_dense(p + "ln/Variable_1", {E}, L2);
      o.w1 = add_dense(p + "multihead_attention/conv1d/kernel", {1, E, E}, L2);
      o.w2 = add_dense(p + "multihead_attention/conv1d_1/kernel", {1, E, E}, L2);
      o.b1 = add_dense(p + "multihead_attention/conv1d/bias", {E}, L2);
      o.b2 = add_dense(p + "multihead_attention/conv1d_1/bias", {E}, L2);
      o.ln_b_beta = add_dense(p + "ln_1/Variable", {E}, L2);
      o.ln_b_gamma = add_dense(p + "ln_1/Variable_1", {E}, L2);
    }
    for (int i = 0; i < BN_COUNT; ++i) bnoff[i] = BnOff{0, 0, 0, 0, 0};
    tower_in = 2 * E;
    tower = add_mlp({"sequential/logit_fcn"}, {L2}, tower_in, 100, 64, true, &bnoff[BN_T0], &bnoff[BN_T1]);
    add_ws("sib.ids_item", PAMREC_I32, {2, N});
    add_ws("sib.ids_cate", PAMREC_I32, {2, N});
    add_ws("sib.h", PAMREC_F32, {2, N, E});
    add_ws("tgt", PAMREC_F32, {B, E});
    add_ws("x0", PAMREC_F32, {N, E});
    for (int b = 0; b < 2; ++b) {
      const std::string p = "blk" + std::to_string(b) + ".";
      add_ws(p + "xq", PAMREC_F32, {N, 2 * E});
      add_ws(p + "qkv", PAMREC_F32, {N, 3 * E});
      add_ws(p + "ml", PAMREC_F32, {N, 2});
      add_ws(p + "y", PAMREC_F32, {N, E});
      add_ws(p + "f", PAMREC_F32, {N, E});
      add_ws(p + "hpre", PAMREC_F32, {N, E});
      add_ws(p + "out", PAMREC_F32, {N, E});
    }
    add_ws("u", PAMREC_F32, {B, 2 * E});
    add_ws("zt0", PAMREC_F32, {B, 100});
    add_ws("zt1", PAMREC_F32, {B, 64});
    add_ws("logits", PAMREC_F32, {B, 1});
    add_ws("losses", PAMREC_F32, {8});
    add_ws("loss_acc", PAMREC_F64, {8});
    add_ws("d_logits", PAMREC_F32, {B, 1});
    add_ws("d_t1", PAMREC_F32, {B, 64});
    add_ws("d_t0", PAMREC_F32, {B, 100});
    add_ws("d_u", PAMREC_F32, {B, 2 * E});
    add_ws("d_tgt_total", PAMREC_F32, {B, E});
    add_ws("sas.g_a", PAMREC_F32, {N, E});
    add_ws("sas.g_b", PAMREC_F32, {N, E});
    add_ws("sas.hid", PAMREC_F32, {N, E});
    add_ws("sas.d_hpre", PAMREC_F32, {N, E});
    add_ws("sas.d_y", PAMREC_F32, {N, E});
    add_ws("sas.d_qkv", PAMREC_F32, {N, 3 * E});
    add_ws("sas.dq", PAMREC_F32, {N});
    add_ws("sib.dh", PAMREC_F32, {2, N, E});
    add_ws("sib.has0", PAMREC_I32, {4});
    add_bn_ws();
    add_optim_ws();
    const int64_t NK = 2 * N + B;
    cub_keys_table = NK;
    for (const char* t : {"item", "cate"}) {
      std::string p = std::string("sp.") + t + ".";
      for (const char* n : {"keys", "idx", "skeys", "sidx", "uidx", "ukeys"}) add_ws(p + n, PAMREC_I32, {NK});
      add_ws(p + "slot", PAMREC_I32, {t[0] == 'i' ? n_items : n_cates});
      add_ws(p + "accum", PAMREC_F32, {NK, t[0] == 'i' ? item_dim : cate_dim});
    }
    add_ws("sp.nuniq", PAMREC_I32, {8});
    add_ws("dp.scalars", PAMREC_F64, {8});
    cub_keys = NK;
    add_ws("cub_temp", PAMREC_U8, {(int64_t)(16u << 20) + 16 * cub_keys});
    (void)c;
  }

  void build(const PamrecConfig& c) {
    n_users = c.n_users; n_items = c.n_items; n_cates = c.n_cates; T = c.max_seq_len; Bcap = c.max_batch;
    world = c.world_size < 1 ? 1 : c.world_size; table_mode = c.table_mode;
    model_kind = c.model_kind;
    item_dim = c.item_dim ? c.item_dim : kI; cate_dim = c.cate_dim ? c.cate_dim : kC; user_dim = c.user_dim ? c.user_dim : PAMREC_USER_DIM;
    emb_dim = item_dim + cate_dim;
    if (model_kind == PAMREC_MODEL_SASREC) { build_sasrec(c); return; }
    if (model_kind != PAMREC_MODEL_PAMREC) { build_sibling(c); return; }
    const int L2 = PAMREC_SEG_L2;
    pos = add_dense("sequential/embedding/position_embedding", {T, kD}, PAMREC_SEG_POS);
    for (int b = 0; b < 2; ++b) {
      std::string p = "sequential/pamrec/num_blocks_" + std::to_string(b) + "/";
      BlockOff& o = blk[b];
      o.ln_a_beta = add_dense(p + "ln/Variable", {kD}, L2);
      o.ln_a_gamma = add_dense(p + "ln/Variable_1", {kD}, L2);
      o.wq = add_dense(p + "self_attention/Q_timeaware_embedding", {kNB, kDD}, L2);
      o.wk = add_dense(p + "self_attention/K_timeaware_embedding", {kNB, kDD}, L2);
      o.wv = add_dense(p + "self_attention/V_timeaware_embedding", {kNB, kDD}, L2);
      o.w1 = add_dense(p + "multihead_attention/conv1d/kernel", {1, kD, kD}, L2);
      o.b1 = add_dense(p + "multihead_attention/conv1d/bias", {kD}, L2);
      o.w2 = add_dense(p + "multihead_attention/conv1d_1/kernel", {1, kD, kD}, L2);
      o.b2 = add_dense(p + "multihead_attention/conv1d_1/bias", {kD}, L2);
      o.ln_b_beta = add_dense(p + "ln_1/Variable", {kD}, L2);
      o.ln_b_gamma = add_dense(p + "ln_1/Variable_1", {kD}, L2);
    }
    score = add_mlp({"sequential/pamrec/new_long/score_1"}, {L2}, kD, 20, 1, false, &bnoff[BN_S0], &bnoff[BN_S1]);
    std::vector<std::string> ex;
    for (int j = 0; j < 5; ++j) ex.push_back("sequential/pamrec/expert_" + std::to_string(j));
    expert = add_mlp(ex, {L2, L2, L2, L2, L2}, kD, 100, 64, false, &bnoff[BN_E0], &bnoff[BN_E1]);
    gate = add_mlp({"sequential/pamrec/gate_main", "sequential/pamrec/gate_sub"}, {L2, L2}, kD, 64, 5, false,
                   &bnoff[BN_G0], &bnoff[BN_G1]);
    tower = add_mlp({"sequential/logit_fcn", "sequential/valid_logit_fcn", "xilidu_logit_fcn"}, {L2, L2, 0}, 64 + kE, 100, 64,
                    true, &bnoff[BN_T0], &bnoff[BN_T1]);
    const char* dead[3] = {"new_distill", "long_term", "short_term"};
    const int dq[3] = {40, 20, 20};
    for (int i = 0; i < 3; ++i) {
      std::string p = std::string("sequential/pamrec/") + dead[i] + "/attention_fcn";
      add_dense(p + "/attention_mat", {kD, dq[i]}, L2 | PAMREC_SEG_DEAD);
      add_mlp({p + "/att_fcn"}, {L2 | PAMREC_SEG_DEAD}, 4 * dq[i], 80, 40, true, nullptr, nullptr, false);
    }

    const int64_t B = Bcap, N = (int64_t)Bcap * T;
    const int64_t NT = N / kTokTile + kNB + 2;
    add_ws("bucket", PAMREC_I32, {N});
    add_ws("perm", PAMREC_I32, {N});
    add_ws("bucket_ctl", PAMREC_I32, {64});
    add_ws("tile_bucket", PAMREC_I32, {NT});
    add_ws("tile_begin", PAMREC_I32, {NT});
    add_ws("tile_count", PAMREC_I32, {NT});
    add_ws("x0", PAMREC_F32, {B, T, kD});
    add_ws("tgt", PAMREC_F32, {B, kE});
    for (int b = 0; b < 2; ++b) {
      std::string p = "blk" + std::to_string(b) + ".";
      for (const char* n : {"qin", "Q", "K", "V", "y", "out"}) add_ws(p + n, PAMREC_F32, {B, T, kD});
      add_ws(p + "ml", PAMREC_F32, {B, T, 2});
    }
    add_ws("z1", PAMREC_F32, {B, T, 20});
    add_ws("z2", PAMREC_F32, {B, T});
    add_ws("pool.aw", PAMREC_F32, {B, T});
    add_ws("head.wT", PAMREC_F32, {3 * 6400 + 3 * 8400 + 5 * 6400 + 2 * 320 + 628 * 40});
    add_ws("new_long", PAMREC_F32, {B, kD});
    add_ws("ze0", PAMREC_F32, {B, 500});
    add_ws("zg0", PAMREC_F32, {B, 128});
    add_ws("ze1", PAMREC_F32, {B, 320});
    add_ws("zg1", PAMREC_F32, {B, 10});
    add_ws("u", PAMREC_F32, {B, 168});
    add_ws("zt0", PAMREC_F32, {B, 300});
    add_ws("zt1", PAMREC_F32, {B, 192});
    add_ws("logits", PAMREC_F32, {B, 3});
    add_ws("losses", PAMREC_F32, {8});
    add_ws("loss_acc", PAMREC_F64, {8});
    add_ws("d_logits", PAMREC_F32, {B, 3});
    add_ws("d_t1", PAMREC_F32, {B, 192});
    add_ws("d_t0", PAMREC_F32, {B, 300});
    add_ws("d_u", PAMREC_F32, {B, 168});
    add_ws("d_e1", PAMREC_F32, {B, 320});
    add_ws("d_g1", PAMREC_F32, {B, 10});
    add_ws("d_e0", PAMREC_F32, {B, 500});
    add_ws("d_g0", PAMREC_F32, {B, 128});
    add_ws("d_new_long", PAMREC_F32, {B, kD});
    add_ws("d_tgt", PAMREC_F32, {B, kE});
    add_ws("d_tgt_total", PAMREC_F32, {B, kE});
    add_ws("d_z2", PAMREC_F32, {B, T});
    add_ws("d_a1", PAMREC_F32, {B, T, 20});
    add_ws("g_a", PAMREC_F32, {B, T, kD});
    add_ws("g_b", PAMREC_F32, {B, T, kD});
    add_ws("d_y", PAMREC_F32, {B, T, kD});
    add_ws("d_Q", PAMREC_F32, {B, T, kD});
    add_ws("d_K", PAMREC_F32, {B, T, kD});
    add_ws("d_V", PAMREC_F32, {B, T, kD});
    add_bn_ws();
    add_optim_ws();
    const int64_t NK = N + B;
    const bool sharded = table_mode == PAMREC_TABLES_SHARDED;
    cub_keys_table = NK;
    for (const char* t : {"item", "cate"}) {
      std::string p = std::string("sp.") + t + ".";
      if (sharded) {
        add_ws(p + "keys", PAMREC_I32, {NK});
        add_ws(p + "idx", PAMREC_I32, {NK});
        add_ws(p + "skeys", PAMREC_I32, {NK});
        add_ws(p + "sidx", PAMREC_I32, {NK});
        add_ws(p + "uidx", PAMREC_I32, {NK});
        add_ws(p + "slot", PAMREC_I32, {rows_of(t[0] == 'i' ? n_items : n_cates)});
      }
      add_ws(p + "ukeys", PAMREC_I32, {NK});
      add_ws(p + "accum", PAMREC_F32, {NK, t[0] == 'i' ? kI : kC});
    }
    if (sharded) {
      add_ws("sp.user.keys", PAMREC_I32, {B});
      add_ws("sp.user.idx", PAMREC_I32, {B});
      add_ws("sp.user.skeys", PAMREC_I32, {B});
      add_ws("sp.user.sidx", PAMREC_I32, {B});
      add_ws("sp.user.uidx", PAMREC_I32, {B});
      add_ws("sp.user.slot", PAMREC_I32, {rows_of(n_users)});
    }
    add_ws("sp.user.ukeys", PAMREC_I32, {B});
    add_ws("sp.nuniq", PAMREC_I32, {8});
    add_ws("dp.scalars", PAMREC_F64, {8});
    cub_keys = NK;
    if (!sharded) {
      const int64_t NKA = 2 * NK + B;
      for (const char* n : {"keys", "idx", "skeys", "sidx", "uidx"}) add_ws(std::string("sp2.") + n, PAMREC_I32, {NKA});
      add_ws("sp2.meta", PAMREC_I32, {16});
      add_ws("sp2.slot", PAMREC_I32, {(int64_t)n_items + n_cates + n_users});
      add_ws("sp2.dflag", PAMREC_I32, {2 * NK});
      add_ws("sp2.l2sq", PAMREC_F64, {4});
      if (table_mode == PAMREC_TABLES_REPLICATED && world > 1)
        add_ws("rep.grad", PAMREC_F32, {(int64_t)n_items * 17 + (int64_t)n_cates * 5 + n_users});
      cub_keys = NKA;
    }
    if (table_mode == PAMREC_TABLES_SHARDED) {
      auto dim = [&](int64_t vocab, int64_t nk, int width) {
        ShardDim d;
        d.vocab = vocab; d.rps = rows_of(vocab); d.nk = nk; d.width = width;
        d.cap_recv = (int64_t)world * (nk < d.rps ? nk : d.rps);
        return d;
      };
      sh_item = dim(n_items, NK, kI); sh_cate = dim(n_cates, NK, kC); sh_user = dim(n_users, B, 0);
      const ShardDim* dims[3] = {&sh_item, &sh_cate, &sh_user};
      const char* names[3] = {"item", "cate", "user"};
      for (int i = 0; i < 3; ++i) {
        const ShardDim& d = *dims[i];
        std::string p = std::string("sh.") + names[i] + ".", q = std::string("so.") + names[i] + ".";
        add_ws(p + "inv", PAMREC_I32, {d.nk});
        add_ws(p + "send_ids", PAMREC_I32, {d.nk});
        add_ws(p + "off", PAMREC_I32, {128});
        add_ws(p + "recv_ids", PAMREC_I32, {d.cap_recv});
        if (d.width) {
          add_ws(p + "rows", PAMREC_F32, {d.nk, d.width});
          add_ws(p + "xrows", PAMREC_F32, {d.cap_recv, d.width});
          add_ws(q + "accum", PAMREC_F32, {d.cap_recv, d.width});
        }
        for (const char* n : {"keys", "idx", "skeys", "sidx", "uidx", "ukeys"}) add_ws(q + n, PAMREC_I32, {d.cap_recv});
        if (d.cap_recv > cub_keys) cub_keys = d.cap_recv;
      }
      add_ws("sh.counts_send", PAMREC_I32, {(int64_t)world * 4});
      add_ws("sh.counts_recv", PAMREC_I32, {(int64_t)world * 4});
      add_ws("sh.scratch", PAMREC_F64, {8});
    }
    add_ws("cub_temp", PAMREC_U8, {(int64_t)(16u << 20) + 16 * cub_keys});
  }
};

}
```

Measured before the change: 1.348 million.

## Port QKV projection forward to tcgen05 UMMA with 128-token tiles

Rewrites the forward QKV projection kernel to use Blackwell tcgen05 tf32 MMAs accumulating in tensor memory, with split hi/lo operands to keep near-fp32 accuracy. Bucket tiles grow to 128 tokens, and the backward projection kernel launches two half-tiles per bucket tile so it keeps its 64-token tiling. Shared tcgen05 helpers move into a common header, and an error flag buffer is added for mbarrier timeouts. This aims to remove the warp-level mma.sync GEMM cost and the per-tile weight reloads, at the cost of larger shared memory use, TMEM allocation, and fewer blocks when buckets are small.

```diff
diff --git a/pamrec_b200/csrc/api.cu b/pamrec_b200/csrc/api.cu
--- a/pamrec_b200/csrc/api.cu
+++ b/pamrec_b200/csrc/api.cu
@@ -627,14 +627,14 @@
   else launch_bucket_plan(b->item_loop_times_history, N, h->wi("bucket"), h->wi("perm"), ctl, h->wi("tile_bucket"),
                           h->wi("tile_begin"), h->wi("tile_count"), st);
   nl += 3;
-  const int max_tiles = N / kTokTile + kNB + 1;
+  const int max_tiles = N / kProjTile + kNB + 1;
   const float* xin = x0;
   for (int k = 0; k < 2; ++k) {
     const BlockOff& o = L.blk[k];
     std::string p = "blk" + std::to_string(k) + ".";
     launch_proj_fwd(xin, h->wi("perm"), ctl, h->wi("tile_bucket"), h->wi("tile_begin"), h->wi("tile_count"), max_tiles,
                     h->P(o.wq), h->P(o.wk), h->P(o.wv), h->P(o.ln_a_beta), h->P(o.ln_a_gamma), h->wf(p + "qin"), h->wf(p + "Q"),
-                    h->wf(p + "K"), h->wf(p + "V"), st);
+                    h->wf(p + "K"), h->wf(p + "V"), h->wi("tc_err"), st);
     if (h->attn_mma)
       launch_attn_fwd_mma(h->wf(p + "Q"), h->wf(p + "K"), h->wf(p + "V"), h->wf(p + "qin"), b->mask, h->wf(p + "y"), h->wf(p + "ml"), B, T, st);
     else if (h->attn_tc && attn_tc_supported(T))
@@ -978,7 +978,7 @@
     launch_dense_dx(x0, st);
     nl += 2;
   }
-  const int max_tiles = N / kTokTile + kNB + 1;
+  const int max_tiles = N / kProjTile + kNB + 1;
   int* ctl = h->wi("bucket_ctl");
   for (int k = 1; k >= 0; --k) {
     const BlockOff& o = L.blk[k];
diff --git a/pamrec_b200/csrc/common.cuh b/pamrec_b200/csrc/common.cuh
--- a/pamrec_b200/csrc/common.cuh
+++ b/pamrec_b200/csrc/common.cuh
@@ -16,6 +16,7 @@
 constexpr int kWarpRows = 16 * kMT;
 constexpr int kTokThreads = 128;
 constexpr int kTokTile = 4 * kWarpRows;
+constexpr int kProjTile = 128;
 constexpr int kRowPad = 41;
 constexpr int kAttnStride = 44;
 constexpr float kMaskNeg = -4294967295.0f;
diff --git a/pamrec_b200/csrc/kernels.h b/pamrec_b200/csrc/kernels.h
--- a/pamrec_b200/csrc/kernels.h
+++ b/pamrec_b200/csrc/kernels.h
@@ -36,7 +36,7 @@
                         int* tile_count, cudaStream_t st);
 void launch_proj_fwd(const float* X, const int* perm, const int* ctl, const int* tile_bucket, const int* tile_begin,
                      const int* tile_count, int max_tiles, const float* Wq, const float* Wk, const float* Wv,
-                     const float* ln_beta, const float* ln_gamma, float* QIN, float* Q, float* K, float* V, cudaStream_t st);
+                     const float* ln_beta, const float* ln_gamma, float* QIN, float* Q, float* K, float* V, int* err, cudaStream_t st);
 void launch_attn_fwd(const float* Q, const float* K, const float* V, const float* QIN, const int* mask, float* Y, float* ML,
                      int B, int T, cudaStream_t st);
 void launch_ffn_fwd(const float* Y, const float* W1, const float* b1, const float* W2, const float* b2,
diff --git a/pamrec_b200/csrc/kernels_attn_tc.cu b/pamrec_b200/csrc/kernels_attn_tc.cu
--- a/pamrec_b200/csrc/kernels_attn_tc.cu
+++ b/pamrec_b200/csrc/kernels_attn_tc.cu
@@ -1,5 +1,6 @@
 #include "kernels.h"
 #include "mma.cuh"
+#include "tcgen05.cuh"
 
 namespace pamrec {
 
@@ -11,63 +12,6 @@
 constexpr int kNV = 48;
 constexpr int kMaxNK = 208;
 constexpr uint32_t kColPlo = 256, kColO = 464, kTmemCols = 512;
-
-__device__ __forceinline__ uint32_t smem_u32(const void* p) { return (uint32_t)__cvta_generic_to_shared(p); }
-__device__ __forceinline__ void mbar_init(uint64_t* bar, uint32_t count) {
-  asm volatile("mbarrier.init.shared::cta.b64 [%0], %1;" ::"r"(smem_u32(bar)), "r"(count) : "memory");
-}
-__device__ __forceinline__ bool mbar_try_wait(uint64_t* bar, uint32_t parity) {
-  uint32_t ok;
-  asm volatile("{\n\t.reg .pred p;\n\tmbarrier.try_wait.parity.shared::cta.b64 p, [%1], %2;\n\tselp.u32 %0, 1, 0, p;\n\t}"
-               : "=r"(ok) : "r"(smem_u32(bar)), "r"(parity) : "memory");
-  return ok != 0;
-}
-__device__ __forceinline__ void mbar_wait(uint64_t* bar, uint32_t parity, int* err) {
-  uint32_t spins = 0;
-  while (!mbar_try_wait(bar, parity)) {
-    if (++spins > (1u << 22)) { if (err) atomicExch(err, 1); break; }
-  }
-}
-__device__ __forceinline__ void fence_proxy_async_smem() { asm volatile("fence.proxy.async.shared::cta;" ::: "memory"); }
-__device__ __forceinline__ void tc_fence_before() { asm volatile("tcgen05.fence::before_thread_sync;" ::: "memory"); }
-__device__ __forceinline__ void tc_fence_after() { asm volatile("tcgen05.fence::after_thread_sync;" ::: "memory"); }
-__device__ __forceinline__ void tc_commit(uint64_t* bar) {
-  asm volatile("tcgen05.commit.cta_group::1.mbarrier::arrive::one.shared::cluster.b64 [%0];" ::"r"(smem_u32(bar)) : "memory");
-}
-__device__ __forceinline__ void umma_ss(uint32_t tmem_d, uint64_t da, uint64_t db, uint32_t idesc, uint32_t accumulate) {
-  asm volatile("{\n\t.reg .pred p;\n\tsetp.ne.b32 p, %4, 0;\n\ttcgen05.mma.cta_group::1.kind::tf32 [%0], %1, %2, %3, p;\n\t}"
-               ::"r"(tmem_d), "l"(da), "l"(db), "r"(idesc), "r"(accumulate) : "memory");
-}
-__device__ __forceinline__ void umma_ts(uint32_t tmem_d, uint32_t tmem_a, uint64_t db, uint32_t idesc, uint32_t accumulate) {
-  asm volatile("{\n\t.reg .pred p;\n\tsetp.ne.b32 p, %4, 0;\n\ttcgen05.mma.cta_group::1.kind::tf32 [%0], [%1], %2, %3, p;\n\t}"
-               ::"r"(tmem_d), "r"(tmem_a), "l"(db), "r"(idesc), "r"(accumulate) : "memory");
-}
-__device__ __forceinline__ uint64_t make_desc(uint32_t smem_addr, uint32_t lbo_bytes, uint32_t sbo_bytes) {
-  uint64_t d = 0;
-  d |= (uint64_t)((smem_addr >> 4) & 0x3FFF);
-  d |= (uint64_t)((lbo_bytes >> 4) & 0x3FFF) << 16;
-  d |= (uint64_t)((sbo_bytes >> 4) & 0x3FFF) << 32;
-  d |= (uint64_t)1 << 46;
-  return d;
-}
-__device__ __forceinline__ uint32_t make_idesc(int M, int N) {
-  return (1u << 4) | (2u << 7) | (2u << 10) | ((uint32_t)(N >> 3) << 17) | ((uint32_t)(M >> 4) << 24);
-}
-__device__ __forceinline__ void tmem_ld16(uint32_t addr, float (&v)[16]) {
-  uint32_t r[16];
-  asm volatile("tcgen05.ld.sync.aligned.32x32b.x16.b32 {%0, %1, %2, %3, %4, %5, %6, %7, %8, %9, %10, %11, %12, %13, %14, %15}, [%16];"
-               : "=r"(r[0]), "=r"(r[1]), "=r"(r[2]), "=r"(r[3]), "=r"(r[4]), "=r"(r[5]), "=r"(r[6]), "=r"(r[7]), "=r"(r[8]), "=r"(r[9]),
-                 "=r"(r[10]), "=r"(r[11]), "=r"(r[12]), "=r"(r[13]), "=r"(r[14]), "=r"(r[15])
-               : "r"(addr) : "memory");
-  asm volatile("tcgen05.wait::ld.sync.aligned;" ::: "memory");
-#pragma unroll
-  for (int i = 0; i < 16; ++i) v[i] = __uint_as_float(r[i]);
-}
-__device__ __forceinline__ void tmem_st16(uint32_t addr, const uint32_t (&r)[16]) {
-  asm volatile("tcgen05.st.sync.aligned.32x32b.x16.b32 [%0], {%1, %2, %3, %4, %5, %6, %7, %8, %9, %10, %11, %12, %13, %14, %15, %16};"
-               ::"r"(addr), "r"(r[0]), "r"(r[1]), "r"(r[2]), "r"(r[3]), "r"(r[4]), "r"(r[5]), "r"(r[6]), "r"(r[7]), "r"(r[8]), "r"(r[9]),
-                 "r"(r[10]), "r"(r[11]), "r"(r[12]), "r"(r[13]), "r"(r[14]), "r"(r[15]) : "memory");
-}
 
 struct Geometry {
   int spt;
@@ -109,10 +53,7 @@
     mbar_init(bar, 1);
     asm volatile("fence.mbarrier_init.release.cluster;" ::: "memory");
   }
-  if (warp == 0) {
-    asm volatile("tcgen05.alloc.cta_group::1.sync.aligned.shared::cta.b32 [%0], %1;" ::"r"(smem_u32(tmem_slot)), "r"(kTmemCols) : "memory");
-    asm volatile("tcgen05.relinquish_alloc_permit.cta_group::1.sync.aligned;" ::: "memory");
-  }
+  if (warp == 0) tmem_alloc(tmem_slot, kTmemCols);
   tc_fence_before();
   __syncthreads();
   tc_fence_after();
@@ -222,7 +163,7 @@
         tmem_st16(lane_base + (uint32_t)c0, ph);
         tmem_st16(lane_base + kColPlo + (uint32_t)c0, pl);
       }
-      asm volatile("tcgen05.wait::st.sync.aligned;" ::: "memory");
+      tmem_wait_st();
       tc_fence_before();
       __syncthreads();
       tc_fence_after();
@@ -266,7 +207,7 @@
       tc_fence_after();
     }
   }
-  if (warp == 0) asm volatile("tcgen05.dealloc.cta_group::1.sync.aligned.b32 %0, %1;" ::"r"(tmem), "r"(kTmemCols) : "memory");
+  if (warp == 0) tmem_dealloc(tmem, kTmemCols);
 }
 
 bool attn_tc_supported(int T) { return T >= 1 && tc::geometry(T).nk <= tc::kMaxNK; }
diff --git a/pamrec_b200/csrc/kernels_encoder.cu b/pamrec_b200/csrc/kernels_encoder.cu
--- a/pamrec_b200/csrc/kernels_encoder.cu
+++ b/pamrec_b200/csrc/kernels_encoder.cu
@@ -1,5 +1,6 @@
 #include "kernels.h"
 #include "mma.cuh"
+#include "tcgen05.cuh"
 
 namespace pamrec {
 
@@ -86,10 +87,10 @@
   for (int k = 0; k < kNB; ++k) {
     int cnt = ctl[k];
     ctl[16 + k] = start;
-    for (int o = 0; o < cnt; o += kTokTile) {
+    for (int o = 0; o < cnt; o += kProjTile) {
       tile_bucket[nt] = k;
       tile_begin[nt] = start + o;
-      tile_count[nt] = min(kTokTile, cnt - o);
+      tile_count[nt] = min(kProjTile, cnt - o);
       ++nt;
     }
     start += cnt;
@@ -126,76 +127,218 @@
 constexpr int kTS = 44;
 __device__ __forceinline__ void load_split_mat(uint32_t* __restrict__ hi, uint32_t* __restrict__ lo, const float* __restrict__ W, int tid);
 __device__ __forceinline__ void load_tile44(float* __restrict__ dst, const float* __restrict__ src, const int* toks, int cnt, int tid);
-constexpr int kLnWriteF = 1, kLnWriteXhat = 2;
-__device__ __forceinline__ void ln_row44(float* __restrict__ row, const float* __restrict__ beta, const float* __restrict__ gamma,
-                                         float& mean, float& rstd, int write);
 __device__ __forceinline__ void store_frag_rows(float* __restrict__ dst, const float (&c)[kMT][5][4], int64_t tok0, const int* toks,
                                                 int row_base, int cnt, int lane);
 
-constexpr int kProjFwdSmem = (6 * kDD + 2 * kTokTile * kTS + 2 * kD) * 4;
-__global__ void __launch_bounds__(kTokThreads)
+__device__ __forceinline__ void ln_stats(const float4 (&x)[10], float& mean, float& rstd) {
+  float sacc = 0.f;
+#pragma unroll
+  for (int i = 0; i < 10; ++i) sacc += (x[i].x + x[i].y) + (x[i].z + x[i].w);
+  mean = sacc * (1.0f / kD);
+  float v = 0.f;
+#pragma unroll
+  for (int i = 0; i < 10; ++i) {
+    float a = x[i].x - mean, b = x[i].y - mean, c = x[i].z - mean, d = x[i].w - mean;
+    v = fmaf(a, a, v); v = fmaf(b, b, v); v = fmaf(c, c, v); v = fmaf(d, d, v);
+  }
+  rstd = 1.0f / sqrtf(v * (1.0f / kD) + kLnEps);
+}
+
+namespace pt {
+constexpr int kThreads = kProjTile;
+constexpr int kChunks = kD / 4;
+constexpr int kNQ = 48, kNKV = 2 * kD;
+constexpr uint32_t kColKV = 0, kColQ = 96, kColXh = 160, kColXl = 208, kTmemCols = 256;
+constexpr int kA = kChunks * kProjTile * 4, kBQ = kChunks * kNQ * 4, kBKV = kChunks * kNKV * 4;
+constexpr int kRowTile = kProjTile * kTS;
+constexpr int kIoIt = kProjTile * kChunks / kThreads;
+static_assert(3 * kRowTile <= 2 * kA + 2 * kBQ + 2 * kBKV, "Q, K, V row tiles reuse the operand buffers");
+constexpr int kFwdSmem = (2 * kA + 2 * kBQ + 2 * kBKV + kRowTile + kProjTile) * 4 + 16;
+}
+
+__device__ __forceinline__ void store_rows_through(float* __restrict__ dst, const float* __restrict__ tile, const int* toks, int cnt, int tid) {
+#pragma unroll
+  for (int it = 0; it < pt::kIoIt; ++it) {
+    const int i = tid + it * pt::kThreads, r = i / pt::kChunks, c = i % pt::kChunks;
+    if (r < cnt) st4(dst + (int64_t)toks[r] * kD + 4 * c, ld4(tile + r * kTS + 4 * c));
+  }
+}
+
+__global__ void __launch_bounds__(pt::kThreads, 2)
 k_proj_fwd(const float* __restrict__ X, const int* __restrict__ perm, const int* __restrict__ ctl,
            const int* __restrict__ tile_bucket, const int* __restrict__ tile_begin, const int* __restrict__ tile_count,
            const float* __restrict__ Wq, const float* __restrict__ Wk, const float* __restrict__ Wv,
            const float* __restrict__ ln_beta, const float* __restrict__ ln_gamma, float* __restrict__ QIN,
-           float* __restrict__ Q, float* __restrict__ K, float* __restrict__ V) {
-  int tile = blockIdx.x;
+           float* __restrict__ Q, float* __restrict__ K, float* __restrict__ V, int* __restrict__ err) {
+  using namespace tc;
+  using namespace pt;
+  const int tile = blockIdx.x;
   if (tile >= ctl[32]) return;
   extern __shared__ __align__(16) float sm[];
-  uint32_t* Whi = reinterpret_cast<uint32_t*>(sm);
-  uint32_t* Wlo = Whi + 3 * kDD;
-  float* xs = sm + 6 * kDD;
-  float* qs = xs + kTokTile * kTS;
-  float* lnp = qs + kTokTile * kTS;
-  __shared__ int toks[kTokTile];
-  const int tid = threadIdx.x, lane = tid & 31, w = tid >> 5;
-  const int k = tile_bucket[tile], begin = tile_begin[tile], cnt = tile_count[tile];
-  load_split_mat(Whi, Wlo, Wq + (int64_t)k * kDD, tid);
-  load_split_mat(Whi + kDD, Wlo + kDD, Wk + (int64_t)k * kDD, tid);
-  load_split_mat(Whi + 2 * kDD, Wlo + 2 * kDD, Wv + (int64_t)k * kDD, tid);
-  if (tid < kD) { lnp[tid] = ln_beta[tid]; lnp[kD + tid] = ln_gamma[tid]; }
+  float* Ah = sm;
+  float* Al = Ah + kA;
+  float* Bqh = Al + kA;
+  float* Bql = Bqh + kBQ;
+  float* Bkvh = Bql + kBQ;
+  float* Bkvl = Bkvh + kBKV;
+  float* Xs = Bkvl + kBKV;
+  int* toks = reinterpret_cast<int*>(Xs + kRowTile);
+  uint32_t* tmem_slot = reinterpret_cast<uint32_t*>(toks + kProjTile);
+  uint64_t* bar = reinterpret_cast<uint64_t*>(tmem_slot + 2);
+  float* Qs = sm;
+  float* Ks = Qs + kRowTile;
+  float* Vs = Ks + kRowTile;
+  const int tid = threadIdx.x, warp = tid >> 5;
+  if (tid == 0) {
+    mbar_init(bar, 1);
+    asm volatile("fence.mbarrier_init.release.cluster;" ::: "memory");
+  }
+  if (warp == 0) tmem_alloc(tmem_slot, kTmemCols);
+  const int bk = tile_bucket[tile], begin = tile_begin[tile], cnt = tile_count[tile];
   if (tid < cnt) toks[tid] = perm[begin + tid];
-  __syncthreads();
-  load_tile44(xs, X, toks, cnt, tid);
-  __syncthreads();
-  if (tid < kTokTile) {
-    float* xr = xs + tid * kTS;
-    float* qr = qs + tid * kTS;
-#pragma unroll
-    for (int i = 0; i < 10; ++i) st4(qr + 4 * i, ld4(xr + 4 * i));
+  constexpr int kW4 = kDD / 4, kWIt = (3 * kW4 + kThreads - 1) / kThreads;
+  float4 wv[kWIt];
+#pragma unroll
+  for (int it = 0; it < kWIt; ++it) {
+    const int i = tid + it * kThreads;
+    const float* w = i < kW4 ? Wq : (i < 2 * kW4 ? Wk : Wv);
+    if (i < 3 * kW4) wv[it] = ld4(w + (int64_t)bk * kDD + 4 * (i % kW4));
+  }
+  tc_fence_before();
+  __syncthreads();
+  tc_fence_after();
+  const uint32_t tmem = *tmem_slot;
+  const uint32_t lane_base = tmem + ((uint32_t)(warp * 32) << 16);
+  {
+    float4 xv[kIoIt];
+#pragma unroll
+    for (int it = 0; it < kIoIt; ++it) {
+      const int i = tid + it * kThreads, r = i / kChunks, c = i % kChunks;
+      xv[it] = r < cnt ? ld4(X + (int64_t)toks[r] * kD + 4 * c) : f4_zero();
+    }
+    uint32_t* bqh = reinterpret_cast<uint32_t*>(Bqh);
+    uint32_t* bql = reinterpret_cast<uint32_t*>(Bql);
+    for (int i = tid; i < (kNQ - kD) * kD; i += kThreads) {
+      const int n = kD + i % (kNQ - kD), k = i / (kNQ - kD);
+      const int o = ((k >> 2) * kNQ + n) * 4 + (k & 3);
+      bqh[o] = 0u; bql[o] = 0u;
+    }
+#pragma unroll
+    for (int it = 0; it < kWIt; ++it) {
+      const int i = tid + it * kThreads;
+      if (i < 3 * kW4) {
+        const int m = i / kW4, e = 4 * (i % kW4), k = e / kD, n0 = e % kD + (m == 2 ? kD : 0);
+        const int N = m == 0 ? kNQ : kNKV;
+        uint32_t* hi = reinterpret_cast<uint32_t*>(m == 0 ? Bqh : Bkvh);
+        uint32_t* lo = reinterpret_cast<uint32_t*>(m == 0 ? Bql : Bkvl);
+        const float f[4] = {wv[it].x, wv[it].y, wv[it].z, wv[it].w};
+#pragma unroll
+        for (int j = 0; j < 4; ++j) {
+          const int o = ((k >> 2) * N + n0 + j) * 4 + (k & 3);
+          split_tf32(f[j], hi[o], lo[o]);
+        }
+      }
+    }
+#pragma unroll
+    for (int it = 0; it < kIoIt; ++it) {
+      const int i = tid + it * kThreads;
+      st4(Xs + (i / kChunks) * kTS + 4 * (i % kChunks), xv[it]);
+    }
+  }
+  __syncthreads();
+  {
+    float4 x[10];
+    float* row = Xs + tid * kTS;
+#pragma unroll
+    for (int i = 0; i < 10; ++i) x[i] = ld4(row + 4 * i);
     float mean, rstd;
-    ln_row44(qr, lnp, lnp + kD, mean, rstd, kLnWriteF);
-    if (tid < cnt) {
-      float* o = QIN + (int64_t)toks[tid] * kD;
-#pragma unroll
-      for (int i = 0; i < 10; ++i) st4(o + 4 * i, ld4(qr + 4 * i));
-    }
-  }
-  __syncthreads();
-  const float* xw = xs + kWarpRows * w * kTS;
-  const float* qw = qs + kWarpRows * w * kTS;
-#pragma unroll 1
-  for (int m = 0; m < 3; ++m) {
-    float c[kMT][5][4];
-#pragma unroll
-    for (int mt = 0; mt < kMT; ++mt)
-#pragma unroll
-      for (int nt = 0; nt < 5; ++nt)
-#pragma unroll
-        for (int q = 0; q < 4; ++q) c[mt][nt][q] = 0.f;
-    const float* aw = m == 0 ? qw : xw;
-    warp_gemm_rows_x40x40<kMT, false>(c, [&](int r, int kk) { return aw[r * kTS + kk]; }, Whi + m * kDD, Wlo + m * kDD, lane);
-    store_frag_rows(m == 0 ? Q : (m == 1 ? K : V), c, 0, toks, kWarpRows * w, cnt, lane);
-  }
+    ln_stats(x, mean, rstd);
+#pragma unroll
+    for (int i = 0; i < kChunks; ++i) {
+      const float4 g = ld4(ln_gamma + 4 * i), b = ld4(ln_beta + 4 * i);
+      const float4 q = make_float4(fmaf(g.x, (x[i].x - mean) * rstd, b.x), fmaf(g.y, (x[i].y - mean) * rstd, b.y),
+                                   fmaf(g.z, (x[i].z - mean) * rstd, b.z), fmaf(g.w, (x[i].w - mean) * rstd, b.w));
+      st4(row + 4 * i, q);
+      uint4 h, l;
+      split_tf32(q.x, h.x, l.x); split_tf32(q.y, h.y, l.y); split_tf32(q.z, h.z, l.z); split_tf32(q.w, h.w, l.w);
+      *reinterpret_cast<uint4*>(Ah + (i * kProjTile + tid) * 4) = h;
+      *reinterpret_cast<uint4*>(Al + (i * kProjTile + tid) * 4) = l;
+    }
+    const float* xf = reinterpret_cast<const float*>(x);
+#pragma unroll
+    for (int c0 = 0; c0 < kNQ; c0 += 16) {
+      uint32_t h[16], l[16];
+#pragma unroll
+      for (int j = 0; j < 16; ++j) {
+        h[j] = 0u; l[j] = 0u;
+        if (c0 + j < kD) split_tf32(xf[c0 + j], h[j], l[j]);
+      }
+      tmem_st16(lane_base + kColXh + (uint32_t)c0, h);
+      tmem_st16(lane_base + kColXl + (uint32_t)c0, l);
+    }
+  }
+  fence_proxy_async_smem();
+  tmem_wait_st();
+  tc_fence_before();
+  __syncthreads();
+  tc_fence_after();
+  if (tid == 0) {
+    const uint32_t sbo = 128, lbo_a = kProjTile * 16, lbo_q = kNQ * 16, lbo_kv = kNKV * 16;
+    const uint32_t idesc_q = make_idesc(kProjTile, kNQ), idesc_kv = make_idesc(kProjTile, kNKV);
+#pragma unroll
+    for (int ks = 0; ks < kD / 8; ++ks) {
+      const uint32_t acc = ks > 0 ? 1u : 0u;
+      const uint64_t dah = make_desc(smem_u32(Ah) + 2 * ks * lbo_a, lbo_a, sbo), dal = make_desc(smem_u32(Al) + 2 * ks * lbo_a, lbo_a, sbo);
+      const uint64_t dqh = make_desc(smem_u32(Bqh) + 2 * ks * lbo_q, lbo_q, sbo), dql = make_desc(smem_u32(Bql) + 2 * ks * lbo_q, lbo_q, sbo);
+      const uint64_t dkvh = make_desc(smem_u32(Bkvh) + 2 * ks * lbo_kv, lbo_kv, sbo);
+      const uint64_t dkvl = make_desc(smem_u32(Bkvl) + 2 * ks * lbo_kv, lbo_kv, sbo);
+      umma_ss(tmem + kColQ, dal, dqh, idesc_q, acc);
+      umma_ss(tmem + kColQ, dah, dql, idesc_q, 1);
+      umma_ss(tmem + kColQ, dah, dqh, idesc_q, 1);
+      umma_ts(tmem + kColKV, tmem + kColXl + 8 * ks, dkvh, idesc_kv, acc);
+      umma_ts(tmem + kColKV, tmem + kColXh + 8 * ks, dkvl, idesc_kv, 1);
+      umma_ts(tmem + kColKV, tmem + kColXh + 8 * ks, dkvh, idesc_kv, 1);
+    }
+    tc_commit(bar);
+  }
+  store_rows_through(QIN, Xs, toks, cnt, tid);
+  mbar_wait(bar, 0, err);
+  tc_fence_after();
+  float* qr = Qs + tid * kTS;
+#pragma unroll
+  for (int c0 = 0; c0 < kNQ; c0 += 16) {
+    float v[16];
+    tmem_ld16(lane_base + kColQ + (uint32_t)c0, v);
+#pragma unroll
+    for (int j = 0; j < 16 && c0 + j < kD; j += 4) st4(qr + c0 + j, make_float4(v[j], v[j + 1], v[j + 2], v[j + 3]));
+  }
+#pragma unroll
+  for (int c0 = 0; c0 < kNKV; c0 += 16) {
+    float v[16];
+    tmem_ld16(lane_base + kColKV + (uint32_t)c0, v);
+#pragma unroll
+    for (int j = 0; j < 16; j += 4) {
+      const int col = c0 + j;
+      float* dst = col < kD ? Ks + tid * kTS + col : Vs + tid * kTS + col - kD;
+      st4(dst, make_float4(v[j], v[j + 1], v[j + 2], v[j + 3]));
+    }
+  }
+  tc_fence_before();
+  __syncthreads();
+  tc_fence_after();
+  if (warp == 0) tmem_dealloc(tmem, kTmemCols);
+  store_rows_through(Q, Qs, toks, cnt, tid);
+  store_rows_through(K, Ks, toks, cnt, tid);
+  store_rows_through(V, Vs, toks, cnt, tid);
 }
 
 void launch_proj_fwd(const float* X, const int* perm, const int* ctl, const int* tile_bucket, const int* tile_begin,
                      const int* tile_count, int max_tiles, const float* Wq, const float* Wk, const float* Wv,
-                     const float* ln_beta, const float* ln_gamma, float* QIN, float* Q, float* K, float* V,
+                     const float* ln_beta, const float* ln_gamma, float* QIN, float* Q, float* K, float* V, int* err,
                      cudaStream_t st) {
   PAMREC_PROF("proj_fwd", 1, st);
-  k_proj_fwd<<<max_tiles, kTokThreads, kProjFwdSmem, st>>>(X, perm, ctl, tile_bucket, tile_begin, tile_count, Wq, Wk, Wv,
-                                                        ln_beta, ln_gamma, QIN, Q, K, V);
+  k_proj_fwd<<<max_tiles, pt::kThreads, pt::kFwdSmem, st>>>(X, perm, ctl, tile_bucket, tile_begin, tile_count, Wq, Wk, Wv,
+                                                           ln_beta, ln_gamma, QIN, Q, K, V, err);
 }
 
 constexpr int kAttnCh = 8;
@@ -356,20 +499,13 @@
     st4(dst + (i / 10) * kTS + 4 * (i % 10), v[it]);
   }
 }
+constexpr int kLnWriteF = 1, kLnWriteXhat = 2;
 __device__ __forceinline__ void ln_row44(float* __restrict__ row, const float* __restrict__ beta, const float* __restrict__ gamma,
                                          float& mean, float& rstd, int write) {
   float4 x[10];
-  float sacc = 0.f;
-#pragma unroll
-  for (int i = 0; i < 10; ++i) { x[i] = ld4(row + 4 * i); sacc += (x[i].x + x[i].y) + (x[i].z + x[i].w); }
-  mean = sacc * (1.0f / kD);
-  float v = 0.f;
-#pragma unroll
-  for (int i = 0; i < 10; ++i) {
-    float a = x[i].x - mean, b = x[i].y - mean, c = x[i].z - mean, d = x[i].w - mean;
-    v = fmaf(a, a, v); v = fmaf(b, b, v); v = fmaf(c, c, v); v = fmaf(d, d, v);
-  }
-  rstd = 1.0f / sqrtf(v * (1.0f / kD) + kLnEps);
+#pragma unroll
+  for (int i = 0; i < 10; ++i) x[i] = ld4(row + 4 * i);
+  ln_stats(x, mean, rstd);
   if (write == kLnWriteXhat) {
 #pragma unroll
     for (int i = 0; i < 10; ++i)
@@ -791,8 +927,10 @@
            const float* __restrict__ Wv, const float* __restrict__ ln_beta, const float* __restrict__ ln_gamma,
            float* __restrict__ dX, float* __restrict__ dWq, float* __restrict__ dWk, float* __restrict__ dWv,
            float* __restrict__ dbeta, float* __restrict__ dgamma) {
-  int tile = blockIdx.x;
+  const int tile = blockIdx.x >> 1, half = blockIdx.x & 1;
   if (tile >= ctl[32]) return;
+  const int k = tile_bucket[tile], begin = tile_begin[tile] + half * kTokTile, cnt = min(kTokTile, tile_count[tile] - half * kTokTile);
+  if (cnt <= 0) return;
   extern __shared__ __align__(16) float sm[];
   uint32_t* Whi = reinterpret_cast<uint32_t*>(sm);
   uint32_t* Wlo = Whi + 3 * kDD;
@@ -806,7 +944,6 @@
   __shared__ int toks[kTokTile];
   const int tid = threadIdx.x, lane = tid & 31, w = tid >> 5;
   const int g = lane >> 2, t = lane & 3;
-  const int k = tile_bucket[tile], begin = tile_begin[tile], cnt = tile_count[tile];
   load_split_mat(Whi, Wlo, Wq + (int64_t)k * kDD, tid);
   load_split_mat(Whi + kDD, Wlo + kDD, Wk + (int64_t)k * kDD, tid);
   load_split_mat(Whi + 2 * kDD, Wlo + 2 * kDD, Wv + (int64_t)k * kDD, tid);
@@ -903,7 +1040,7 @@
                      const float* Wq, const float* Wk, const float* Wv, const float* ln_beta, const float* ln_gamma,
                      float* dX, float* dWq, float* dWk, float* dWv, float* dbeta, float* dgamma, cudaStream_t st) {
   PAMREC_PROF("proj_bwd", 1, st);
-  k_proj_bwd<<<max_tiles, kTokThreads, kProjBwdSmem, st>>>(X, dY, dQ, dK, dV, perm, ctl, tile_bucket, tile_begin, tile_count, Wq,
+  k_proj_bwd<<<2 * max_tiles, kTokThreads, kProjBwdSmem, st>>>(X, dY, dQ, dK, dV, perm, ctl, tile_bucket, tile_begin, tile_count, Wq,
                                                         Wk, Wv, ln_beta, ln_gamma, dX, dWq, dWk, dWv, dbeta, dgamma);
 }
 
@@ -912,7 +1049,7 @@
   auto set = [&](const void* fn, size_t bytes) {
     if (e == cudaSuccess) e = cudaFuncSetAttribute(fn, cudaFuncAttributeMaxDynamicSharedMemorySize, (int)bytes);
   };
-  set((const void*)k_proj_fwd, kProjFwdSmem);
+  set((const void*)k_proj_fwd, pt::kFwdSmem);
   set((const void*)k_ffn_fwd, kFfnFwdSmem);
   set((const void*)k_ffn_bwd, kFfnBwdSmem);
   set((const void*)k_proj_bwd, kProjBwdSmem);
diff --git a/pamrec_b200/csrc/layout.h b/pamrec_b200/csrc/layout.h
--- a/pamrec_b200/csrc/layout.h
+++ b/pamrec_b200/csrc/layout.h
@@ -353,13 +353,14 @@
     }
 
     const int64_t B = Bcap, N = (int64_t)Bcap * T;
-    const int64_t NT = N / kTokTile + kNB + 2;
+    const int64_t NT = N / kProjTile + kNB + 2;
     add_ws("bucket", PAMREC_I32, {N});
     add_ws("perm", PAMREC_I32, {N});
     add_ws("bucket_ctl", PAMREC_I32, {64});
     add_ws("tile_bucket", PAMREC_I32, {NT});
     add_ws("tile_begin", PAMREC_I32, {NT});
     add_ws("tile_count", PAMREC_I32, {NT});
+    add_ws("tc_err", PAMREC_I32, {4});
     add_ws("x0", PAMREC_F32, {B, T, kD});
     add_ws("tgt", PAMREC_F32, {B, kE});
     for (int b = 0; b < 2; ++b) {
diff --git a/pamrec_b200/csrc/tcgen05.cuh b/pamrec_b200/csrc/tcgen05.cuh
--- /dev/null
+++ b/pamrec_b200/csrc/tcgen05.cuh
@@ -0,0 +1,74 @@
+#pragma once
+#include <cuda_runtime.h>
+#include <stdint.h>
+
+namespace pamrec {
+namespace tc {
+
+__device__ __forceinline__ uint32_t smem_u32(const void* p) { return (uint32_t)__cvta_generic_to_shared(p); }
+__device__ __forceinline__ void mbar_init(uint64_t* bar, uint32_t count) {
+  asm volatile("mbarrier.init.shared::cta.b64 [%0], %1;" ::"r"(smem_u32(bar)), "r"(count) : "memory");
+}
+__device__ __forceinline__ bool mbar_try_wait(uint64_t* bar, uint32_t parity) {
+  uint32_t ok;
+  asm volatile("{\n\t.reg .pred p;\n\tmbarrier.try_wait.parity.shared::cta.b64 p, [%1], %2;\n\tselp.u32 %0, 1, 0, p;\n\t}"
+               : "=r"(ok) : "r"(smem_u32(bar)), "r"(parity) : "memory");
+  return ok != 0;
+}
+__device__ __forceinline__ void mbar_wait(uint64_t* bar, uint32_t parity, int* err) {
+  uint32_t spins = 0;
+  while (!mbar_try_wait(bar, parity)) {
+    if (++spins > (1u << 22)) { if (err) atomicExch(err, 1); break; }
+  }
+}
+__device__ __forceinline__ void fence_proxy_async_smem() { asm volatile("fence.proxy.async.shared::cta;" ::: "memory"); }
+__device__ __forceinline__ void tc_fence_before() { asm volatile("tcgen05.fence::before_thread_sync;" ::: "memory"); }
+__device__ __forceinline__ void tc_fence_after() { asm volatile("tcgen05.fence::after_thread_sync;" ::: "memory"); }
+__device__ __forceinline__ void tc_commit(uint64_t* bar) {
+  asm volatile("tcgen05.commit.cta_group::1.mbarrier::arrive::one.shared::cluster.b64 [%0];" ::"r"(smem_u32(bar)) : "memory");
+}
+__device__ __forceinline__ void tmem_alloc(uint32_t* slot, uint32_t cols) {
+  asm volatile("tcgen05.alloc.cta_group::1.sync.aligned.shared::cta.b32 [%0], %1;" ::"r"(smem_u32(slot)), "r"(cols) : "memory");
+  asm volatile("tcgen05.relinquish_alloc_permit.cta_group::1.sync.aligned;" ::: "memory");
+}
+__device__ __forceinline__ void tmem_dealloc(uint32_t tmem, uint32_t cols) {
+  asm volatile("tcgen05.dealloc.cta_group::1.sync.aligned.b32 %0, %1;" ::"r"(tmem), "r"(cols) : "memory");
+}
+__device__ __forceinline__ void umma_ss(uint32_t tmem_d, uint64_t da, uint64_t db, uint32_t idesc, uint32_t accumulate) {
+  asm volatile("{\n\t.reg .pred p;\n\tsetp.ne.b32 p, %4, 0;\n\ttcgen05.mma.cta_group::1.kind::tf32 [%0], %1, %2, %3, p;\n\t}"
+               ::"r"(tmem_d), "l"(da), "l"(db), "r"(idesc), "r"(accumulate) : "memory");
+}
+__device__ __forceinline__ void umma_ts(uint32_t tmem_d, uint32_t tmem_a, uint64_t db, uint32_t idesc, uint32_t accumulate) {
+  asm volatile("{\n\t.reg .pred p;\n\tsetp.ne.b32 p, %4, 0;\n\ttcgen05.mma.cta_group::1.kind::tf32 [%0], [%1], %2, %3, p;\n\t}"
+               ::"r"(tmem_d), "r"(tmem_a), "l"(db), "r"(idesc), "r"(accumulate) : "memory");
+}
+__device__ __forceinline__ uint64_t make_desc(uint32_t smem_addr, uint32_t lbo_bytes, uint32_t sbo_bytes) {
+  uint64_t d = 0;
+  d |= (uint64_t)((smem_addr >> 4) & 0x3FFF);
+  d |= (uint64_t)((lbo_bytes >> 4) & 0x3FFF) << 16;
+  d |= (uint64_t)((sbo_bytes >> 4) & 0x3FFF) << 32;
+  d |= (uint64_t)1 << 46;
+  return d;
+}
+__device__ __forceinline__ uint32_t make_idesc(int M, int N) {
+  return (1u << 4) | (2u << 7) | (2u << 10) | ((uint32_t)(N >> 3) << 17) | ((uint32_t)(M >> 4) << 24);
+}
+__device__ __forceinline__ void tmem_ld16(uint32_t addr, float (&v)[16]) {
+  uint32_t r[16];
+  asm volatile("tcgen05.ld.sync.aligned.32x32b.x16.b32 {%0, %1, %2, %3, %4, %5, %6, %7, %8, %9, %10, %11, %12, %13, %14, %15}, [%16];"
+               : "=r"(r[0]), "=r"(r[1]), "=r"(r[2]), "=r"(r[3]), "=r"(r[4]), "=r"(r[5]), "=r"(r[6]), "=r"(r[7]), "=r"(r[8]), "=r"(r[9]),
+                 "=r"(r[10]), "=r"(r[11]), "=r"(r[12]), "=r"(r[13]), "=r"(r[14]), "=r"(r[15])
+               : "r"(addr) : "memory");
+  asm volatile("tcgen05.wait::ld.sync.aligned;" ::: "memory");
+#pragma unroll
+  for (int i = 0; i < 16; ++i) v[i] = __uint_as_float(r[i]);
+}
+__device__ __forceinline__ void tmem_st16(uint32_t addr, const uint32_t (&r)[16]) {
+  asm volatile("tcgen05.st.sync.aligned.32x32b.x16.b32 [%0], {%1, %2, %3, %4, %5, %6, %7, %8, %9, %10, %11, %12, %13, %14, %15, %16};"
+               ::"r"(addr), "r"(r[0]), "r"(r[1]), "r"(r[2]), "r"(r[3]), "r"(r[4]), "r"(r[5]), "r"(r[6]), "r"(r[7]), "r"(r[8]), "r"(r[9]),
+                 "r"(r[10]), "r"(r[11]), "r"(r[12]), "r"(r[13]), "r"(r[14]), "r"(r[15]) : "memory");
+}
+__device__ __forceinline__ void tmem_wait_st() { asm volatile("tcgen05.wait::st.sync.aligned;" ::: "memory"); }
+
+}
+}
```

Measured after the change: 1.350 million, median of 6. About the same (+0.2%).
